# cipherflow-fhe/lattisense

Measured on AMD Instinct MI355X. Metric: ckks_hmult_relin_rescale_throughput, higher is better.
Workload: dtype u64

## Files before the change

include/lattisense_amd.h:

```cpp
#ifndef LATTISENSE_AMD_H
#define LATTISENSE_AMD_H
#include <stddef.h>
#include <stdint.h>

#ifdef __cplusplus
extern "C" {
#endif

typedef struct lsa_context_st* lsa_context;
typedef struct lsa_key_st* lsa_key;

enum { LSA_OK = 0, LSA_ERR_ARG = 1, LSA_ERR_NO_DEVICE = 2, LSA_ERR_HIP = 3, LSA_ERR_INTERNAL = 4 };
enum { LSA_ALGO_BFV = 0, LSA_ALGO_CKKS = 1 };

const char* lsa_last_error(void);
const char* lsa_version(void);
const char* lsa_build_flags(void);

int lsa_context_create(int algo, int n, const uint64_t* q, int nq, const uint64_t* p, int np, uint64_t t,
                       int device, lsa_context* out);
int lsa_context_destroy(lsa_context ctx);
int lsa_context_moduli(lsa_context ctx, uint64_t* out, int capacity, int* count);

int lsa_malloc(lsa_context ctx, void** dptr, size_t bytes);
int lsa_free(lsa_context ctx, void* dptr);
int lsa_memcpy_h2d(lsa_context ctx, void* dst, const void* src, size_t bytes, void* stream);
int lsa_memcpy_d2h(lsa_context ctx, void* dst, const void* src, size_t bytes, void* stream);
int lsa_memcpy_d2d(lsa_context ctx, void* dst, const void* src, size_t bytes, void* stream);
int lsa_stream_create(lsa_context ctx, void** stream);
int lsa_stream_destroy(lsa_context ctx, void* stream);
int lsa_stream_synchronize(lsa_context ctx, void* stream);
int lsa_event_create(lsa_context ctx, void** ev);
int lsa_event_record(lsa_context ctx, void* ev, void* stream);
int lsa_event_elapsed_ms(lsa_context ctx, void* ev_start, void* ev_stop, float* ms);
int lsa_event_destroy(lsa_context ctx, void* ev);

int lsa_key_upload(lsa_context ctx, const uint64_t* compact_host, int key_level, void* stream, lsa_key* out);
int lsa_key_adopt_device(lsa_context ctx, uint64_t* compact_dev, int key_level, void* stream, lsa_key* out);
int lsa_key_destroy(lsa_context ctx, lsa_key key);
size_t lsa_key_bytes(lsa_context ctx, int key_level);

int lsa_ntt(lsa_context ctx, uint64_t* data, int batch, long long batch_stride, int rows, const int* mod_of,
            int period, int inverse, void* stream);

int lsa_poly_addsub(lsa_context ctx, int op, int level, int polys, const uint64_t* a, const uint64_t* b,
                    uint64_t* out, int batch, long long stride_a, long long stride_b, long long stride_out,
                    void* stream);

int lsa_ckks_mult(lsa_context ctx, int level, const uint64_t* a, const uint64_t* b, uint64_t* d3, int batch,
                  long long stride_a, long long stride_b, long long stride_d, void* stream);
int lsa_ckks_relin(lsa_context ctx, int level, const uint64_t* d3, lsa_key rlk, uint64_t* out, int batch,
                   long long stride_d, long long stride_out, void* stream);
int lsa_ckks_rescale(lsa_context ctx, int level, int polys, const uint64_t* in, uint64_t* out, int batch,
                     long long stride_in, long long stride_out, void* stream);
int lsa_ckks_rotate(lsa_context ctx, int level, const uint64_t* in, uint64_t galois_element, lsa_key glk,
                    uint64_t* out, int batch, long long stride_in, long long stride_out, void* stream);
int lsa_drop_level(lsa_context ctx, int level, int polys, const uint64_t* in, uint64_t* out, int batch,
                   long long stride_in, long long stride_out, void* stream);
int lsa_ckks_mult_relin_rescale(lsa_context ctx, int level, const uint64_t* a, const uint64_t* b, lsa_key rlk,
                                uint64_t* out, int batch, long long stride_a, long long stride_b,
                                long long stride_out, void* stream);
int lsa_ckks_mult_sum(lsa_context ctx, int level, int n, const uint64_t* const* as, const long long* sas, const int* a_rpp,
                      const uint64_t* const* bs, const long long* sbs, const int* b_rpp, const uint64_t* addend,
                      long long s_addend, uint64_t* d3, int batch, long long sd, void* stream);
int lsa_ckks_dot(lsa_context ctx, int level, int n, const uint64_t* const* as, const long long* sas, const int* a_rpp,
                 const uint64_t* const* bs, const long long* sbs, const int* b_rpp, const uint64_t* addend,
                 long long s_addend, lsa_key rlk, uint64_t* out, int batch, long long sout, int rescale, void* stream);

int lsa_ckks_encode(lsa_context ctx, int level, int log_slots, const double* values, double scale, uint64_t* out_dev, long long sout,
                    int batch, void* stream);
int lsa_ckks_mult_plain(lsa_context ctx, int level, const uint64_t* ct, long long sct, const uint64_t* pt, long long spt, uint64_t* out,
                        long long sout, int batch, int rescale, void* stream);
int lsa_ckks_addsub_plain(lsa_context ctx, int op, int level, const uint64_t* ct, long long sct, const uint64_t* pt, long long spt,
                          uint64_t* out, long long sout, int batch, void* stream);
int lsa_ckks_mac_plain(lsa_context ctx, int level, int n, const uint64_t* const* cts, const long long* scts, const uint64_t* const* pts,
                       const long long* spts, const uint64_t* addend, long long s_addend, uint64_t* out, long long sout, int batch,
                       int rescale, void* stream);
int lsa_ckks_mult_const(lsa_context ctx, int level, const uint64_t* ct, long long sct, double re, double im, double const_scale,
                        uint64_t* out, long long sout, int batch, int rescale, void* stream);
int lsa_ckks_add_const(lsa_context ctx, int level, const uint64_t* ct, long long sct, double re, double im, double ct_scale,
                       uint64_t* out, long long sout, int batch, void* stream);
int lsa_ckks_affine_const(lsa_context ctx, int level, const uint64_t* ct, long long sct, double re, double im, double const_scale,
                          double add_re, double add_im, double ct_scale, uint64_t* out, long long sout, int batch, int rescale,
                          void* stream);

int lsa_bfv_mult(lsa_context ctx, int level, const uint64_t* a, const uint64_t* b, uint64_t* d3, int batch,
                 long long stride_a, long long stride_b, long long stride_d, void* stream);
int lsa_bfv_relin(lsa_context ctx, int level, const uint64_t* d3, lsa_key rlk, uint64_t* out, int batch,
                  long long stride_d, long long stride_out, void* stream);
int lsa_bfv_rotate(lsa_context ctx, int level, const uint64_t* in, uint64_t galois_element, lsa_key glk,
                   uint64_t* out, int batch, long long stride_in, long long stride_out, void* stream);
int lsa_bfv_mult_plain_mul(lsa_context ctx, int level, const uint64_t* ct, const uint64_t* pt, uint64_t* out, int batch,
                           long long sct, long long spt, long long sout, void* stream);
int lsa_bfv_mac_plain_mul(lsa_context ctx, int level, int n, const uint64_t* const* cts, const long long* scts,
                          const uint64_t* const* pts, const long long* spts, const uint64_t* partial, long long spartial,
                          uint64_t* out, int batch, long long sout, void* stream);
int lsa_bfv_rotate_mac_plain_mul(lsa_context ctx, int level, const uint64_t* in, int n, const uint64_t* galois_elements,
                                 const lsa_key* glk, const uint64_t* const* pts, const long long* spts, const uint64_t* partial,
                                 long long spartial, uint64_t* out, int batch, long long sin, long long sout, void* stream);
int lsa_bfv_rescale(lsa_context ctx, int level, int polys, const uint64_t* in, uint64_t* out, int batch,
                    long long stride_in, long long stride_out, void* stream);
int lsa_bfv_mult_relin(lsa_context ctx, int level, const uint64_t* a, const uint64_t* b, lsa_key rlk,
                       uint64_t* out, int batch, long long stride_a, long long stride_b, long long stride_out,
                       void* stream);
int lsa_bfv_mult_sum(lsa_context ctx, int level, int n, const uint64_t* const* as, const long long* sas, const uint64_t* const* bs,
                     const long long* sbs, const uint64_t* addend, long long s_addend, uint64_t* d3, int batch, long long sd,
                     void* stream);
int lsa_bfv_dot(lsa_context ctx, int level, int n, const uint64_t* const* as, const long long* sas, const uint64_t* const* bs,
                const long long* sbs, const uint64_t* addend, long long s_addend, lsa_key rlk, uint64_t* out, int batch,
                long long sout, void* stream);
int lsa_bfv_dot_plan(int n_ring, const uint64_t* q, int nq, int level, int terms, int* max_terms, int* n_groups, int* aux_limbs);

int lsa_set_bfv_dot_chunk(lsa_context ctx, int pairs);
int lsa_set_tile_batch(lsa_context ctx, int tile_batch);
int lsa_set_fp64_ntt(lsa_context ctx, int enable);
int lsa_set_dual_stream(lsa_context ctx, int enable);
int lsa_set_fuse_tails(lsa_context ctx, int enable);
int lsa_set_modup_lift(lsa_context ctx, int enable);
int lsa_set_ks_tail_in_mac(lsa_context ctx, int mode);
int lsa_set_ntt_chunk_mib(lsa_context ctx, int mib);
int lsa_ckks_rotate_many(lsa_context ctx, int level, const uint64_t* in, int n_rot, const uint64_t* galois_elements,
                         const lsa_key* glk, uint64_t* const* outs, int batch, long long sin, long long sout, void* stream);
int lsa_bfv_rotate_many(lsa_context ctx, int level, const uint64_t* in, int n_rot, const uint64_t* galois_elements,
                        const lsa_key* glk, uint64_t* const* outs, int batch, long long sin, long long sout, void* stream);

typedef struct lsa_bootstrap_st* lsa_bootstrap;
int lsa_bootstrap_create(lsa_context ctx, int cts_depth, int stc_depth, int k, int double_angle, double message_ratio,
                         double in_scale, double out_scale, int log_slots, void* stream, lsa_bootstrap* out);
int lsa_bootstrap_create_ex(lsa_context ctx, int cts_depth, int stc_depth, int k, int double_angle, double message_ratio,
                            double in_scale, double out_scale, int log_slots, int sine_deg, int arcsine_deg, void* stream,
                            lsa_bootstrap* out);
int lsa_bootstrap_evalmod_constants(lsa_bootstrap b, int* n_cheb, double* cheb, int* n_asin, double* asin_coef);
void lsa_bootstrap_destroy(lsa_bootstrap b);
int lsa_bootstrap_info(lsa_bootstrap b, int* out_level, double* out_scale, int* n_galois, int* n_matrices, int* n_cts,
                       int* sparse);
int lsa_bootstrap_galois_elements(lsa_bootstrap b, uint64_t* out, int capacity);
int lsa_bootstrap_chebyshev(lsa_bootstrap b, double* out32);
int lsa_bootstrap_matrix_info(lsa_bootstrap b, int index, int* level, int* n1, int* n_diagonals, int* diagonals, int capacity);
int lsa_bootstrap_plaintext(lsa_bootstrap b, int matrix, int diag_pos, uint64_t* host_out);
int lsa_bootstrap_plaintext_rows(lsa_bootstrap b, int matrix, int* rows);
int lsa_bootstrap_plaintext_ext(lsa_bootstrap b, int matrix, int diag_pos, uint64_t* host_out, long long capacity_words);
int lsa_ckks_bootstrap(lsa_context ctx, lsa_bootstrap b, const uint64_t* in, uint64_t* out, int batch, long long sin, long long sout,
                       lsa_key rlk, int n_glk, const uint64_t* glk_elements, const lsa_key* glk, lsa_key swk_dts, lsa_key swk_std,
                       void* stream);

typedef struct lsa_linear_transform_st* lsa_linear_transform;
int lsa_lt_create(lsa_context ctx, int level, int log_slots, int n_diag, const int* diag_index, const double* values,
                  double pt_scale, double bsgs_ratio, int double_hoist, void* stream, lsa_linear_transform* out);
void lsa_lt_destroy(lsa_linear_transform lt);
int lsa_lt_info(lsa_linear_transform lt, int* level, int* period, int* n_diag, int* n1, int* rows, int* n_galois,
                int* double_hoist, double* pt_scale);
int lsa_lt_diagonals(lsa_linear_transform lt, int* index_out, int capacity);
int lsa_lt_galois_elements(lsa_linear_transform lt, uint64_t* out, int capacity);
int lsa_lt_plaintext(lsa_linear_transform lt, int diag_pos, uint64_t* host_out, long long capacity_words);
int lsa_ckks_linear_transform(lsa_context ctx, lsa_linear_transform lt, const uint64_t* in, uint64_t* out, int batch,
                              long long sin, long long sout, int rescale, int n_glk, const uint64_t* glk_elements,
                              const lsa_key* glk, void* stream);
int lsa_lt_plan_rotations(int period, int n_diag, const int* diag_index, double bsgs_ratio, int* n1, int* rotations,
                          int capacity, int* count);

typedef struct lsa_slot_sum_st* lsa_slot_sum;
int lsa_slot_sum_plan(int n_ring, long long step, int count, int radix, int* n_steps, int* n_keyswitch, int* n_moddown,
                      int* rotations, int capacity, int* n_rot);
int lsa_slot_sum_create(lsa_context ctx, int level, long long step, int count, int radix, lsa_slot_sum* out);
void lsa_slot_sum_destroy(lsa_slot_sum plan);
int lsa_slot_sum_info(lsa_slot_sum plan, int* level, int* count, int* radix, int* n_steps, int* n_keyswitch, int* n_moddown,
                      int* n_galois);
int lsa_slot_sum_galois_elements(lsa_slot_sum plan, uint64_t* out, int capacity);
int lsa_slot_sum_set_multi_mac(lsa_slot_sum plan, int enable);
int lsa_ckks_slot_sum(lsa_context ctx, lsa_slot_sum plan, const uint64_t* in, uint64_t* out, int batch, long long sin,
                      long long sout, int n_keys, const uint64_t* galois_elements, const lsa_key* keys, void* stream);

typedef struct lsa_bfv_slot_sum_st* lsa_bfv_slot_sum_handle;
int lsa_bfv_slot_sum_plan(int n_ring, long long step, int count, int radix, int rows, int* n_steps, int* n_keyswitch, int* n_moddown,
                          uint64_t* galois_elements, int capacity, int* n_galois);
int lsa_bfv_slot_sum_create(lsa_context ctx, int level, long long step, int count, int radix, int rows, lsa_bfv_slot_sum_handle* out);
void lsa_bfv_slot_sum_destroy(lsa_bfv_slot_sum_handle plan);
int lsa_bfv_slot_sum_info(lsa_bfv_slot_sum_handle plan, int* level, int* count, int* radix, int* rows, int* n_steps, int* n_keyswitch,
                          int* n_moddown, int* n_galois, int* gather);
int lsa_bfv_slot_sum_galois_elements(lsa_bfv_slot_sum_handle plan, uint64_t* out, int capacity);
int lsa_bfv_slot_sum_set_gather(lsa_bfv_slot_sum_handle plan, int enable);
int lsa_bfv_slot_sum(lsa_context ctx, lsa_bfv_slot_sum_handle plan, const uint64_t* in, uint64_t* out, int batch, long long sin,
                     long long sout, int n_keys, const uint64_t* galois_elements, const lsa_key* keys, void* stream);

int lsa_bfv_encode(lsa_context ctx, int level, int form, const uint64_t* values, uint64_t* out_dev, long long sout, int batch,
                   void* stream);

int lsa_bfv_addsub_plain(lsa_context ctx, int op, int level, const uint64_t* ct, long long sct, const uint64_t* pt, long long spt,
                         uint64_t* out, long long sout, int batch, void* stream);
int lsa_bfv_plain_lift(lsa_context ctx, int level, int form, const uint64_t* pt, long long spt, uint64_t* out, long long sout,
                       int batch, void* stream);
int lsa_bfv_mult_plain(lsa_context ctx, int level, const uint64_t* ct, long long sct, const uint64_t* pt, long long spt,
                       uint64_t* out, long long sout, int batch, void* stream);

typedef struct lsa_bfv_lt_st* lsa_bfv_lt;
int lsa_bfv_lt_create(lsa_context ctx, int level, int period, int n_diag, const int* diag_index, const uint64_t* values,
                      double bsgs_ratio, void* stream, lsa_bfv_lt* out);
void lsa_bfv_lt_destroy(lsa_bfv_lt lt);
int lsa_bfv_lt_info(lsa_bfv_lt lt, int* level, int* period, int* n_diag, int* n1, int* n_baby, int* n_giant, int* rows,
                    int* n_galois, int* n_moddown);
int lsa_bfv_lt_diagonals(lsa_bfv_lt lt, int* index_out, int capacity);
int lsa_bfv_lt_galois_elements(lsa_bfv_lt lt, uint64_t* out, int capacity);
int lsa_bfv_lt_plaintext(lsa_bfv_lt lt, int diag_pos, uint64_t* host_out, long long capacity_words);
int lsa_bfv_linear_transform(lsa_context ctx, lsa_bfv_lt lt, const uint64_t* in, uint64_t* out, int batch, long long sin,
                             long long sout, int n_keys, const uint64_t* galois_elements, const lsa_key* keys, void* stream);

typedef struct lsa_polynomial_st* lsa_polynomial;
int lsa_poly_plan(int basis, int n_coef, const double* coef, int log_baby, int level_in, int with_interval, int* depth,
                  int* log_baby_out, int* n_mult, int* n_leaves, int* n_leaf_launches);
int lsa_poly_create(lsa_context ctx, int basis, int n_coef, const double* coef, double a, double b, int level_in, double scale_in,
                    double scale_out, int log_baby, lsa_polynomial* out);
void lsa_poly_destroy(lsa_polynomial p);
int lsa_poly_info(lsa_polynomial p, int* level_in, int* level_out, double* scale_out, int* depth, int* log_baby, int* n_mult,
                  int* n_leaves, int* n_leaf_launches, int* n_constants);
int lsa_poly_constants(lsa_polynomial p, long long* out, int capacity);
int lsa_ckks_poly_eval(lsa_context ctx, lsa_polynomial p, const uint64_t* in, uint64_t* out, int batch, long long sin,
                       long long sout, lsa_key rlk, void* stream);

typedef struct lsa_bfv_polynomial_st* lsa_bfv_polynomial;
int lsa_bfv_poly_plan(uint64_t t, int n_coef, const uint64_t* coef, int log_baby, int* log_baby_out, int* depth, int* n_mult,
                      int* n_leaves, int* n_leaf_launches, int* n_pairs);
int lsa_bfv_poly_create(lsa_context ctx, int level, int n_coef, const uint64_t* coef, int log_baby, void* stream,
                        lsa_bfv_polynomial* out);
void lsa_bfv_poly_destroy(lsa_bfv_polynomial p);
int lsa_bfv_poly_info(lsa_bfv_polynomial p, int* level, int* n_coef, int* log_baby, int* depth, int* n_mult, int* n_leaves,
                      int* n_leaf_launches, int* n_pairs);
int lsa_bfv_poly_eval(lsa_context ctx, lsa_bfv_polynomial p, const uint64_t* in, uint64_t* out, int batch, long long sin,
                      long long sout, lsa_key rlk, void* stream);
int lsa_bfv_affine_const(lsa_context ctx, int level, const uint64_t* ct, long long sct, uint64_t k, uint64_t c, uint64_t* out,
                         long long sout, int batch, void* stream);

int lsa_debug_set_ntt_stamps(lsa_context ctx, void* device_buffer);
int lsa_debug_baseconv_plans(lsa_context ctx, int capacity, int* count, int* ns, int* nd, int* split);
int lsa_debug_key_switch_fused(lsa_context ctx, int level, lsa_key key, int* fused);
int lsa_profile_begin(lsa_context ctx, int stride);
int lsa_profile_end(lsa_context ctx);
int lsa_profile_read(lsa_context ctx, int kind, double* total_ms, double* total_bytes, long long* sampled,
                     long long* launched);
int lsa_profile_read_primary(lsa_context ctx, int kind, double* total_bytes_primary);
int lsa_probe_copy(lsa_context ctx, uint64_t* dst, const uint64_t* src, size_t n_u64, void* stream);
int lsa_probe_mulhi(lsa_context ctx, uint64_t* buf, size_t n_u64, int iters, void* stream);

#ifdef __cplusplus
}
#endif
#endif
```

lattisense_amd/_native.py:

```python
import ctypes
import importlib.util
import os

_HERE = os.path.dirname(os.path.abspath(__file__))
LIB_PATH = os.environ.get("LSA_NATIVE_LIB") or os.path.join(_HERE, "liblattisense_amd.so")

_lib = None

c_u64p = ctypes.POINTER(ctypes.c_uint64)
c_ll = ctypes.c_longlong
c_vp = ctypes.c_void_p
c_int = ctypes.c_int


class LsaError(RuntimeError):
    def __init__(self, code, msg):
        super().__init__("lattisense_amd error %d: %s" % (code, msg))
        self.code = code


def _preload_hip_runtime():
    spec = importlib.util.find_spec("torch")
    if spec is not None and spec.origin:
        p = os.path.join(os.path.dirname(spec.origin), "lib", "libamdhip64.so")
        if os.path.exists(p):
            ctypes.CDLL(p, mode=ctypes.RTLD_GLOBAL)


SIGNATURES = {
    "lsa_last_error": (ctypes.c_char_p, []),
    "lsa_version": (ctypes.c_char_p, []),
    "lsa_build_flags": (ctypes.c_char_p, []),
    "lsa_context_create": (c_int, [c_int, c_int, c_u64p, c_int, c_u64p, c_int, ctypes.c_uint64, c_int,
                                   ctypes.POINTER(c_vp)]),
    "lsa_context_destroy": (c_int, [c_vp]),
    "lsa_context_moduli": (c_int, [c_vp, c_u64p, c_int, ctypes.POINTER(c_int)]),
    "lsa_malloc": (c_int, [c_vp, ctypes.POINTER(c_vp), ctypes.c_size_t]),
    "lsa_free": (c_int, [c_vp, c_vp]),
    "lsa_memcpy_h2d": (c_int, [c_vp, c_vp, c_vp, ctypes.c_size_t, c_vp]),
    "lsa_memcpy_d2h": (c_int, [c_vp, c_vp, c_vp, ctypes.c_size_t, c_vp]),
    "lsa_memcpy_d2d": (c_int, [c_vp, c_vp, c_vp, ctypes.c_size_t, c_vp]),
    "lsa_stream_create": (c_int, [c_vp, ctypes.POINTER(c_vp)]),
    "lsa_stream_destroy": (c_int, [c_vp, c_vp]),
    "lsa_stream_synchronize": (c_int, [c_vp, c_vp]),
    "lsa_event_create": (c_int, [c_vp, ctypes.POINTER(c_vp)]),
    "lsa_event_record": (c_int, [c_vp, c_vp, c_vp]),
    "lsa_event_elapsed_ms": (c_int, [c_vp, c_vp, c_vp, ctypes.POINTER(ctypes.c_float)]),
    "lsa_event_destroy": (c_int, [c_vp, c_vp]),
    "lsa_key_upload": (c_int, [c_vp, c_vp, c_int, c_vp, ctypes.POINTER(c_vp)]),
    "lsa_key_adopt_device": (c_int, [c_vp, c_vp, c_int, c_vp, ctypes.POINTER(c_vp)]),
    "lsa_key_destroy": (c_int, [c_vp, c_vp]),
    "lsa_key_bytes": (ctypes.c_size_t, [c_vp, c_int]),
    "lsa_ntt": (c_int, [c_vp, c_vp, c_int, c_ll, c_int, ctypes.POINTER(c_int), c_int, c_int, c_vp]),
    "lsa_poly_addsub": (c_int, [c_vp, c_int, c_int, c_int, c_vp, c_vp, c_vp, c_int, c_ll, c_ll, c_ll, c_vp]),
    "lsa_ckks_mult": (c_int, [c_vp, c_int, c_vp, c_vp, c_vp, c_int, c_ll, c_ll, c_ll, c_vp]),
    "lsa_ckks_relin": (c_int, [c_vp, c_int, c_vp, c_vp, c_vp, c_int, c_ll, c_ll, c_vp]),
    "lsa_ckks_rescale": (c_int, [c_vp, c_int, c_int, c_vp, c_vp, c_int, c_ll, c_ll, c_vp]),
    "lsa_ckks_rotate": (c_int, [c_vp, c_int, c_vp, ctypes.c_uint64, c_vp, c_vp, c_int, c_ll, c_ll, c_vp]),
    "lsa_drop_level": (c_int, [c_vp, c_int, c_int, c_vp, c_vp, c_int, c_ll, c_ll, c_vp]),
    "lsa_ckks_mult_relin_rescale": (c_int, [c_vp, c_int, c_vp, c_vp, c_vp, c_vp, c_int, c_ll, c_ll, c_ll, c_vp]),
    "lsa_ckks_mult_sum": (c_int, [c_vp, c_int, c_int, ctypes.POINTER(c_vp), ctypes.POINTER(c_ll), ctypes.POINTER(c_int),
                                  ctypes.POINTER(c_vp), ctypes.POINTER(c_ll), ctypes.POINTER(c_int), c_vp, c_ll, c_vp, c_int, c_ll, c_vp]),
    "lsa_ckks_dot": (c_int, [c_vp, c_int, c_int, ctypes.POINTER(c_vp), ctypes.POINTER(c_ll), ctypes.POINTER(c_int),
                             ctypes.POINTER(c_vp), ctypes.POINTER(c_ll), ctypes.POINTER(c_int), c_vp, c_ll, c_vp, c_vp, c_int, c_ll, c_int,
                             c_vp]),
    "lsa_ckks_encode": (c_int, [c_vp, c_int, c_int, ctypes.POINTER(ctypes.c_double), ctypes.c_double, c_vp, c_ll, c_int, c_vp]),
    "lsa_ckks_mult_plain": (c_int, [c_vp, c_int, c_vp, c_ll, c_vp, c_ll, c_vp, c_ll, c_int, c_int, c_vp]),
    "lsa_ckks_addsub_plain": (c_int, [c_vp, c_int, c_int, c_vp, c_ll, c_vp, c_ll, c_vp, c_ll, c_int, c_vp]),
    "lsa_ckks_mac_plain": (c_int, [c_vp, c_int, c_int, ctypes.POINTER(c_vp), ctypes.POINTER(c_ll), ctypes.POINTER(c_vp),
                                   ctypes.POINTER(c_ll), c_vp, c_ll, c_vp, c_ll, c_int, c_int, c_vp]),
    "lsa_ckks_mult_const": (c_int, [c_vp, c_int, c_vp, c_ll, ctypes.c_double, ctypes.c_double, ctypes.c_double, c_vp, c_ll, c_int,
                                    c_int, c_vp]),
    "lsa_ckks_add_const": (c_int, [c_vp, c_int, c_vp, c_ll, ctypes.c_double, ctypes.c_double, ctypes.c_double, c_vp, c_ll, c_int,
                                   c_vp]),
    "lsa_ckks_affine_const": (c_int, [c_vp, c_int, c_vp, c_ll, ctypes.c_double, ctypes.c_double, ctypes.c_double, ctypes.c_double,
                                      ctypes.c_double, ctypes.c_double, c_vp, c_ll, c_int, c_int, c_vp]),
    "lsa_bfv_mult": (c_int, [c_vp, c_int, c_vp, c_vp, c_vp, c_int, c_ll, c_ll, c_ll, c_vp]),
    "lsa_bfv_relin": (c_int, [c_vp, c_int, c_vp, c_vp, c_vp, c_int, c_ll, c_ll, c_vp]),
    "lsa_bfv_rotate": (c_int, [c_vp, c_int, c_vp, ctypes.c_uint64, c_vp, c_vp, c_int, c_ll, c_ll, c_vp]),
    "lsa_bfv_rescale": (c_int, [c_vp, c_int, c_int, c_vp, c_vp, c_int, c_ll, c_ll, c_vp]),
    "lsa_bfv_mult_relin": (c_int, [c_vp, c_int, c_vp, c_vp, c_vp, c_vp, c_int, c_ll, c_ll, c_ll, c_vp]),
    "lsa_bfv_mult_sum": (c_int, [c_vp, c_int, c_int, ctypes.POINTER(c_vp), ctypes.POINTER(c_ll), ctypes.POINTER(c_vp),
                                 ctypes.POINTER(c_ll), c_vp, c_ll, c_vp, c_int, c_ll, c_vp]),
    "lsa_bfv_dot": (c_int, [c_vp, c_int, c_int, ctypes.POINTER(c_vp), ctypes.POINTER(c_ll), ctypes.POINTER(c_vp), ctypes.POINTER(c_ll),
                            c_vp, c_ll, c_vp, c_vp, c_int, c_ll, c_vp]),
    "lsa_bfv_dot_plan": (c_int, [c_int, c_u64p, c_int, c_int, c_int, ctypes.POINTER(c_int), ctypes.POINTER(c_int),
                                 ctypes.POINTER(c_int)]),
    "lsa_set_bfv_dot_chunk": (c_int, [c_vp, c_int]),
    "lsa_set_tile_batch": (c_int, [c_vp, c_int]),
    "lsa_set_fp64_ntt": (c_int, [c_vp, c_int]),
    "lsa_set_dual_stream": (c_int, [c_vp, c_int]),
    "lsa_set_fuse_tails": (c_int, [c_vp, c_int]),
    "lsa_set_modup_lift": (c_int, [c_vp, c_int]),
    "lsa_set_ks_tail_in_mac": (c_int, [c_vp, c_int]),
    "lsa_set_ntt_chunk_mib": (c_int, [c_vp, c_int]),
    "lsa_debug_set_ntt_stamps": (c_int, [c_vp, c_vp]),
    "lsa_debug_baseconv_plans": (c_int, [c_vp, c_int, ctypes.POINTER(c_int), ctypes.POINTER(c_int), ctypes.POINTER(c_int),
                                         ctypes.POINTER(c_int)]),
    "lsa_debug_key_switch_fused": (c_int, [c_vp, c_int, c_vp, ctypes.POINTER(c_int)]),
    "lsa_ckks_rotate_many": (c_int, [c_vp, c_int, c_vp, c_int, c_u64p, ctypes.POINTER(c_vp), ctypes.POINTER(c_vp), c_int,
                                     ctypes.c_longlong, ctypes.c_longlong, c_vp]),
    "lsa_bfv_rotate_many": (c_int, [c_vp, c_int, c_vp, c_int, c_u64p, ctypes.POINTER(c_vp), ctypes.POINTER(c_vp), c_int,
                                    ctypes.c_longlong, ctypes.c_longlong, c_vp]),
    "lsa_bfv_mult_plain_mul": (c_int, [c_vp, c_int, c_vp, c_vp, c_vp, c_int, c_ll, c_ll, c_ll, c_vp]),
    "lsa_bfv_mac_plain_mul": (c_int, [c_vp, c_int, c_int, ctypes.POINTER(c_vp), ctypes.POINTER(c_ll), ctypes.POINTER(c_vp),
                                      ctypes.POINTER(c_ll), c_vp, c_ll, c_vp, c_int, c_ll, c_vp]),
    "lsa_bfv_rotate_mac_plain_mul": (c_int, [c_vp, c_int, c_vp, c_int, c_u64p, ctypes.POINTER(c_vp), ctypes.POINTER(c_vp),
                                             ctypes.POINTER(c_ll), c_vp, c_ll, c_vp, c_int, c_ll, c_ll, c_vp]),
    "lsa_bootstrap_create": (c_int, [c_vp, c_int, c_int, c_int, c_int, ctypes.c_double, ctypes.c_double, ctypes.c_double, c_int,
                                     c_vp, ctypes.POINTER(c_vp)]),
    "lsa_bootstrap_create_ex": (c_int, [c_vp, c_int, c_int, c_int, c_int, ctypes.c_double, ctypes.c_double, ctypes.c_double, c_int,
                                        c_int, c_int, c_vp, ctypes.POINTER(c_vp)]),
    "lsa_bootstrap_evalmod_constants": (c_int, [c_vp, ctypes.POINTER(c_int), ctypes.POINTER(ctypes.c_double), ctypes.POINTER(c_int),
                                                ctypes.POINTER(ctypes.c_double)]),
    "lsa_bootstrap_destroy": (None, [c_vp]),
    "lsa_bootstrap_info": (c_int, [c_vp, ctypes.POINTER(c_int), ctypes.POINTER(ctypes.c_double), ctypes.POINTER(c_int),
                                   ctypes.POINTER(c_int), ctypes.POINTER(c_int), ctypes.POINTER(c_int)]),
    "lsa_bootstrap_galois_elements": (c_int, [c_vp, c_u64p, c_int]),
    "lsa_bootstrap_chebyshev": (c_int, [c_vp, ctypes.POINTER(ctypes.c_double)]),
    "lsa_bootstrap_matrix_info": (c_int, [c_vp, c_int, ctypes.POINTER(c_int), ctypes.POINTER(c_int), ctypes.POINTER(c_int),
                                          ctypes.POINTER(c_int), c_int]),
    "lsa_bootstrap_plaintext": (c_int, [c_vp, c_int, c_int, c_u64p]),
    "lsa_bootstrap_plaintext_rows": (c_int, [c_vp, c_int, ctypes.POINTER(c_int)]),
    "lsa_bootstrap_plaintext_ext": (c_int, [c_vp, c_int, c_int, c_u64p, ctypes.c_longlong]),
    "lsa_ckks_bootstrap": (c_int, [c_vp, c_vp, c_vp, c_vp, c_int, ctypes.c_longlong, ctypes.c_longlong, c_vp, c_int, c_u64p,
                                   ctypes.POINTER(c_vp), c_vp, c_vp, c_vp]),
    "lsa_lt_create": (c_int, [c_vp, c_int, c_int, c_int, ctypes.POINTER(c_int), ctypes.POINTER(ctypes.c_double), ctypes.c_double,
                              ctypes.c_double, c_int, c_vp, ctypes.POINTER(c_vp)]),
    "lsa_lt_destroy": (None, [c_vp]),
    "lsa_lt_info": (c_int, [c_vp, ctypes.POINTER(c_int), ctypes.POINTER(c_int), ctypes.POINTER(c_int), ctypes.POINTER(c_int),
                            ctypes.POINTER(c_int), ctypes.POINTER(c_int), ctypes.POINTER(c_int), ctypes.POINTER(ctypes.c_double)]),
    "lsa_lt_diagonals": (c_int, [c_vp, ctypes.POINTER(c_int), c_int]),
    "lsa_lt_galois_elements": (c_int, [c_vp, c_u64p, c_int]),
    "lsa_lt_plaintext": (c_int, [c_vp, c_int, c_u64p, c_ll]),
    "lsa_ckks_linear_transform": (c_int, [c_vp, c_vp, c_vp, c_vp, c_int, c_ll, c_ll, c_int, c_int, c_u64p, ctypes.POINTER(c_vp),
                                          c_vp]),
    "lsa_slot_sum_plan": (c_int, [c_int, c_ll, c_int, c_int, ctypes.POINTER(c_int), ctypes.POINTER(c_int), ctypes.POINTER(c_int),
                                  ctypes.POINTER(c_int), c_int, ctypes.POINTER(c_int)]),
    "lsa_slot_sum_create": (c_int, [c_vp, c_int, c_ll, c_int, c_int, ctypes.POINTER(c_vp)]),
    "lsa_slot_sum_destroy": (None, [c_vp]),
    "lsa_slot_sum_info": (c_int, [c_vp] + [ctypes.POINTER(c_int)] * 7),
    "lsa_slot_sum_galois_elements": (c_int, [c_vp, c_u64p, c_int]),
    "lsa_slot_sum_set_multi_mac": (c_int, [c_vp, c_int]),
    "lsa_ckks_slot_sum": (c_int, [c_vp, c_vp, c_vp, c_vp, c_int, c_ll, c_ll, c_int, c_u64p, ctypes.POINTER(c_vp), c_vp]),
    "lsa_bfv_slot_sum_plan": (c_int, [c_int, c_ll, c_int, c_int, c_int, ctypes.POINTER(c_int), ctypes.POINTER(c_int), ctypes.POINTER(c_int),
                                      c_u64p, c_int, ctypes.POINTER(c_int)]),
    "lsa_bfv_slot_sum_create": (c_int, [c_vp, c_int, c_ll, c_int, c_int, c_int, ctypes.POINTER(c_vp)]),
    "lsa_bfv_slot_sum_destroy": (None, [c_vp]),
    "lsa_bfv_slot_sum_info": (c_int, [c_vp] + [ctypes.POINTER(c_int)] * 9),
    "lsa_bfv_slot_sum_galois_elements": (c_int, [c_vp, c_u64p, c_int]),
    "lsa_bfv_slot_sum_set_gather": (c_int, [c_vp, c_int]),
    "lsa_bfv_slot_sum": (c_int, [c_vp, c_vp, c_vp, c_vp, c_int, c_ll, c_ll, c_int, c_u64p, ctypes.POINTER(c_vp), c_vp]),
    "lsa_bfv_encode": (c_int, [c_vp, c_int, c_int, c_u64p, c_vp, c_ll, c_int, c_vp]),
    "lsa_bfv_addsub_plain": (c_int, [c_vp, c_int, c_int, c_vp, c_ll, c_vp, c_ll, c_vp, c_ll, c_int, c_vp]),
    "lsa_bfv_plain_lift": (c_int, [c_vp, c_int, c_int, c_vp, c_ll, c_vp, c_ll, c_int, c_vp]),
    "lsa_bfv_mult_plain": (c_int, [c_vp, c_int, c_vp, c_ll, c_vp, c_ll, c_vp, c_ll, c_int, c_vp]),
    "lsa_bfv_lt_create": (c_int, [c_vp, c_int, c_int, c_int, ctypes.POINTER(c_int), c_u64p, ctypes.c_double, c_vp, ctypes.POINTER(c_vp)]),
    "lsa_bfv_lt_destroy": (None, [c_vp]),
    "lsa_bfv_lt_info": (c_int, [c_vp] + [ctypes.POINTER(c_int)] * 9),
    "lsa_bfv_lt_diagonals": (c_int, [c_vp, ctypes.POINTER(c_int), c_int]),
    "lsa_bfv_lt_galois_elements": (c_int, [c_vp, c_u64p, c_int]),
    "lsa_bfv_lt_plaintext": (c_int, [c_vp, c_int, c_u64p, c_ll]),
    "lsa_bfv_linear_transform": (c_int, [c_vp, c_vp, c_vp, c_vp, c_int, c_ll, c_ll, c_int, c_u64p, ctypes.POINTER(c_vp), c_vp]),
    "lsa_lt_plan_rotations": (c_int, [c_int, c_int, ctypes.POINTER(c_int), ctypes.c_double, ctypes.POINTER(c_int),
                                      ctypes.POINTER(c_int), c_int, ctypes.POINTER(c_int)]),
    "lsa_poly_plan": (c_int, [c_int, c_int, ctypes.POINTER(ctypes.c_double), c_int, c_int, c_int, ctypes.POINTER(c_int),
                              ctypes.POINTER(c_int), ctypes.POINTER(c_int), ctypes.POINTER(c_int), ctypes.POINTER(c_int)]),
    "lsa_poly_create": (c_int, [c_vp, c_int, c_int, ctypes.POINTER(ctypes.c_double), ctypes.c_double, ctypes.c_double, c_int,
                                ctypes.c_double, ctypes.c_double, c_int, ctypes.POINTER(c_vp)]),
    "lsa_poly_destroy": (None, [c_vp]),
    "lsa_poly_info": (c_int, [c_vp, ctypes.POINTER(c_int), ctypes.POINTER(c_int), ctypes.POINTER(ctypes.c_double),
                              ctypes.POINTER(c_int), ctypes.POINTER(c_int), ctypes.POINTER(c_int), ctypes.POINTER(c_int),
                              ctypes.POINTER(c_int), ctypes.POINTER(c_int)]),
    "lsa_poly_constants": (c_int, [c_vp, ctypes.POINTER(c_ll), c_int]),
    "lsa_ckks_poly_eval": (c_int, [c_vp, c_vp, c_vp, c_vp, c_int, c_ll, c_ll, c_vp, c_vp]),
    "lsa_bfv_poly_plan": (c_int, [ctypes.c_uint64, c_int, c_u64p, c_int] + [ctypes.POINTER(c_int)] * 6),
    "lsa_bfv_poly_create": (c_int, [c_vp, c_int, c_int, c_u64p, c_int, c_vp, ctypes.POINTER(c_vp)]),
    "lsa_bfv_poly_destroy": (None, [c_vp]),
    "lsa_bfv_poly_info": (c_int, [c_vp] + [ctypes.POINTER(c_int)] * 8),
    "lsa_bfv_poly_eval": (c_int, [c_vp, c_vp, c_vp, c_vp, c_int, c_ll, c_ll, c_vp, c_vp]),
    "lsa_bfv_affine_const": (c_int, [c_vp, c_int, c_vp, c_ll, ctypes.c_uint64, ctypes.c_uint64, c_vp, c_ll, c_int, c_vp]),
    "lsa_profile_begin": (c_int, [c_vp, c_int]),
    "lsa_profile_end": (c_int, [c_vp]),
    "lsa_profile_read": (c_int, [c_vp, c_int, ctypes.POINTER(ctypes.c_double), ctypes.POINTER(ctypes.c_double),
                                 ctypes.POINTER(c_ll), ctypes.POINTER(c_ll)]),
    "lsa_profile_read_primary": (c_int, [c_vp, c_int, ctypes.POINTER(ctypes.c_double)]),
    "lsa_probe_copy": (c_int, [c_vp, c_vp, c_vp, ctypes.c_size_t, c_vp]),
    "lsa_probe_mulhi": (c_int, [c_vp, c_vp, ctypes.c_size_t, c_int, c_vp]),
}


def lib():
    global _lib
    if _lib is None:
        if not os.path.exists(LIB_PATH):
            raise RuntimeError("liblattisense_amd.so is not built: run `python -m lattisense_amd.build` "
                               "(or __graft_entry__.build()); there is no fallback path")
        _preload_hip_runtime()
        L = ctypes.CDLL(LIB_PATH)
        for name, (res, args) in SIGNATURES.items():
            fn = getattr(L, name)
            fn.restype = res
            fn.argtypes = args
        flags = L.lsa_build_flags().decode()
        if flags and not os.environ.get("LSA_NATIVE_LIB"):
            raise RuntimeError("%s was built with switches [%s]: not the product build; rebuild with "
                               "`python -m lattisense_amd.build --force`" % (LIB_PATH, flags))
        _lib = L
    return _lib


def build_flags():
    return lib().lsa_build_flags().decode()


def check(rc):
    if rc != 0:
        raise LsaError(rc, lib().lsa_last_error().decode())
```

lattisense_amd/csrc/c_api.hip:

```cpp
#include "bfv_encode.h"
#include "bfv_poly.h"
#include "build_flags.h"
#include "linear_transform.h"
#include "poly_eval.h"
#include "lsa_internal.h"

namespace lsa {
const char* kernels_build_flags();
const char* context_build_flags();
}

using namespace lsa;

struct lsa_context_st {
    Context ctx;
    lsa_context_st(int algo, int n, const u64* q, int nq, const u64* p, int np, u64 t, int dev)
        : ctx(algo, n, q, nq, p, np, t, dev) {}
};
struct lsa_key_st {
    Key key;
    double* fp_owned = nullptr;
};

template <typename F>
// ... 291 lines not shown
    return guard([&] { ckks_encode(CP(ctx, "lsa_ckks_encode"), level, log_slots, values, scale, out_dev, sout, batch, S(stream)); });
}
int lsa_ckks_mult_plain(lsa_context ctx, int level, const uint64_t* ct, long long sct, const uint64_t* pt, long long spt, uint64_t* out,
                        long long sout, int batch, int rescale, void* stream) {
    return guard([&] { ckks_mult_plain(CP(ctx, "lsa_ckks_mult_plain"), level, ct, sct, pt, spt, out, sout, batch, rescale != 0, S(stream)); });
}
int lsa_ckks_addsub_plain(lsa_context ctx, int op, int level, const uint64_t* ct, long long sct, const uint64_t* pt, long long spt,
                          uint64_t* out, long long sout, int batch, void* stream) {
    return guard([&] { ckks_addsub_plain(CP(ctx, "lsa_ckks_addsub_plain"), op, level, ct, sct, pt, spt, out, sout, batch, S(stream)); });
}
int lsa_ckks_mac_plain(lsa_context ctx, int level, int n, const uint64_t* const* cts, const long long* scts, const uint64_t* const* pts,
                       const long long* spts, const uint64_t* addend, long long s_addend, uint64_t* out, long long sout, int batch,
                       int rescale, void* stream) {
    return guard([&] {
        ckks_mac_plain(CP(ctx, "lsa_ckks_mac_plain"), level, n, cts, scts, pts, spts, addend, s_addend, out, sout, batch, rescale != 0,
                       S(stream));
    });
}
int lsa_ckks_mult_const(lsa_context ctx, int level, const uint64_t* ct, long long sct, double re, double im, double const_scale,
                        uint64_t* out, long long sout, int batch, int rescale, void* stream) {
    return guard([&] {
        ckks_mult_const(CP(ctx, "lsa_ckks_mult_const"), level, ct, sct, re, im, const_scale, out, sout, batch, rescale != 0, S(stream));
    });
}
int lsa_ckks_add_const(lsa_context ctx, int level, const uint64_t* ct, long long sct, double re, double im, double ct_scale,
                       uint64_t* out, long long sout, int batch, void* stream) {
    return guard([&] { ckks_add_const(CP(ctx, "lsa_ckks_add_const"), level, ct, sct, re, im, ct_scale, out, sout, batch, S(stream)); });
}
int lsa_ckks_affine_const(lsa_context ctx, int level, const uint64_t* ct, long long sct, double re, double im, double const_scale,
                          double add_re, double add_im, double ct_scale, uint64_t* out, long long sout, int batch, int rescale,
                          void* stream) {
    return guard([&] {
        ckks_affine_const(CP(ctx, "lsa_ckks_affine_const"), level, ct, sct, re, im, const_scale, add_re, add_im, ct_scale, out, sout,
                          batch, rescale != 0, S(stream));
    });
}

int lsa_bfv_mult(lsa_context ctx, int level, const uint64_t* a, const uint64_t* b, uint64_t* d3, int batch, long long sa,
                 long long sb, long long sd, void* stream) {
    return guard([&] { bfv_mult(C(ctx), level, a, b, d3, batch, sa, sb, sd, S(stream)); });
}
int lsa_bfv_relin(lsa_context ctx, int level, const uint64_t* d3, lsa_key rlk, uint64_t* out, int batch, long long sd,
                  long long so, void* stream) {
    return guard([&] { bfv_relin(C(ctx), level, d3, K(rlk, "lsa_bfv_relin"), out, batch, sd, so, S(stream)); });
}
int lsa_bfv_rotate(lsa_context ctx, int level, const uint64_t* in, uint64_t g, lsa_key glk, uint64_t* out, int batch,
                   long long si, long long so, void* stream) {
    return guard([&] { bfv_rotate(C(ctx), level, in, g, K(glk, "lsa_bfv_rotate"), out, batch, si, so, S(stream)); });
}
int lsa_bfv_rescale(lsa_context ctx, int level, int polys, const uint64_t* in, uint64_t* out, int batch, long long si,
                    long long so, void* stream) {
    return guard([&] { bfv_rescale(C(ctx), level, polys, in, out, batch, si, so, S(stream)); });
}
int lsa_bfv_mult_relin(lsa_context ctx, int level, const uint64_t* a, const uint64_t* b, lsa_key rlk, uint64_t* out,
                       int batch, long long sa, long long sb, long long so, void* stream) {
    return guard([&] { bfv_mult_relin(C(ctx), level, a, b, K(rlk, "lsa_bfv_mult_relin"), out, batch, sa, sb, so, S(stream)); });
}

int lsa_bfv_mult_sum(lsa_context ctx, int level, int n, const uint64_t* const* as, const long long* sas, const uint64_t* const* bs,
                     const long long* sbs, const uint64_t* addend, long long s_addend, uint64_t* d3, int batch, long long sd,
                     void* stream) {
    return guard([&] {
        const DotTerms t{n, as, sas, nullptr, bs, sbs, nullptr, addend, s_addend};
        bfv_mult_sum(C(ctx), level, t, d3, batch, sd, S(stream));
    });
}
int lsa_bfv_dot(lsa_context ctx, int level, int n, const uint64_t* const* as, const long long* sas, const uint64_t* const* bs,
                const long long* sbs, const uint64_t* addend, long long s_addend, lsa_key rlk, uint64_t* out, int batch, long long sout,
                void* stream) {
    return guard([&] {
        const DotTerms t{n, as, sas, nullptr, bs, sbs, nullptr, addend, s_addend};
        bfv_dot(C(ctx), level, t, rlk ? &rlk->key : nullptr, out, batch, sout, S(stream));
    });
}
int lsa_bfv_dot_plan(int n_ring, const uint64_t* q, int nq, int level, int terms, int* max_terms, int* n_groups, int* aux_limbs) {
    return guard([&] {
        LSA_REQUIRE(n_ring >= 2 && n_ring <= (1 << 20) && (n_ring & (n_ring - 1)) == 0, "bfv_dot: the ring degree must be a power of two");
        LSA_REQUIRE(q != nullptr && nq >= 1, "bfv_dot: null argument");
        LSA_REQUIRE(level >= 0 && level < nq, "bfv_dot: level out of range");
        LSA_REQUIRE(terms >= 1, "bfv_dot: needs at least one term");
        for (int i = 0; i < nq; i++) LSA_REQUIRE(q[i] >= 2 && (q[i] >> 61) == 0, "bfv_dot: a modulus is out of range");
        int logn = 0;
        while ((1 << logn) < n_ring) logn++;
        const BfvDotPlan p = bfv_dot_plan(q, nq, level, logn, terms);
        if (max_terms) *max_terms = p.max_terms;
        if (n_groups) *n_groups = p.n_groups;
        if (aux_limbs) *aux_limbs = p.aux_limbs;
    });
}

int lsa_profile_begin(lsa_context ctx, int stride) {
    return guard([&] {
        Context& c = C(ctx);
        LSA_REQUIRE(stride >= 1, "stride must be >= 1");
        for (auto& sm : c.prof_samples) {
            c.prof_pool.push_back(sm.e0);
            c.prof_pool.push_back(sm.e1);
        }
        c.prof_samples.clear();
        for (auto& n : c.prof_launched) n = 0;
        c.prof_stride = stride;
        c.prof_on = true;
    });
}
int lsa_profile_end(lsa_context ctx) {
    return guard([&] { C(ctx).prof_on = false; });
}
int lsa_profile_read(lsa_context ctx, int kind, double* total_ms, double* total_bytes, long long* sampled,
                     long long* launched) {
    return guard([&] {
        Context& c = C(ctx);
        LSA_REQUIRE(kind >= 0 && kind < LSA_PROF_KINDS, "unknown kernel kind");
        double ms = 0, by = 0;
        long long n = 0;
        for (auto& sm : c.prof_samples) {
            if (sm.kid != kind) continue;
            LSA_HIP(hipEventSynchronize(sm.e1));
            float t = 0;
            LSA_HIP(hipEventElapsedTime(&t, sm.e0, sm.e1));
            ms += t;
            by += sm.bytes;
            n++;
        }
        if (total_ms) *total_ms = ms;
        if (total_bytes) *total_bytes = by;
        if (sampled) *sampled = n;
        if (launched) *launched = c.prof_launched[kind];
    });
}

int lsa_profile_read_primary(lsa_context ctx, int kind, double* total_bytes_primary) {
    return guard([&] {
        Context& c = C(ctx);
        LSA_REQUIRE(kind >= 0 && kind < LSA_PROF_KINDS && total_bytes_primary, "bad argument");
        double by = 0;
        for (auto& sm : c.prof_samples)
            if (sm.kid == kind) by += sm.bytes_primary;
        *total_bytes_primary = by;
    });
}

int lsa_set_fuse_tails(lsa_context ctx, int enable) {
    return guard([&] { C(ctx).fuse_tails = enable ? 1 : 0; });
}
int lsa_set_modup_lift(lsa_context ctx, int enable) {
    return guard([&] { C(ctx).modup_lift = enable ? 1 : 0; });
}
int lsa_set_ks_tail_in_mac(lsa_context ctx, int mode) {
    return guard([&] {
        LSA_REQUIRE(mode >= 0 && mode <= 2, "lsa_set_ks_tail_in_mac: mode is 0, 1 or 2");
        C(ctx).ks_tail_in_mac = mode;
    });
}
int lsa_set_dual_stream(lsa_context ctx, int enable) {
    return guard([&] { C(ctx).dual_stream = enable ? 1 : 0; });
}
int lsa_debug_set_ntt_stamps(lsa_context ctx, void* device_buffer) {
    return guard([&] { C(ctx).ntt_diag = static_cast<unsigned long long*>(device_buffer); });
}
int lsa_debug_baseconv_plans(lsa_context ctx, int capacity, int* count, int* ns, int* nd, int* split) {
    return guard([&] {
        Context& c = C(ctx);
        LSA_REQUIRE(count != nullptr && (capacity == 0 || (ns && nd && split)), "null argument");
        std::lock_guard<std::mutex> lk(c.mu);
        *count = (int)c.bconv.size();
        int i = 0;
        for (auto& kv : c.bconv) {
            if (i >= capacity) break;
            ns[i] = kv.second.ns;
            nd[i] = kv.second.nd;
            split[i] = kv.second.split29 ? 1 : 0;
            i++;
        }
    });
}
int lsa_debug_key_switch_fused(lsa_context ctx, int level, lsa_key key, int* fused) {
    return guard([&] {
        Context& c = C(ctx);
        LSA_REQUIRE(fused != nullptr && level >= 0 && level < c.nq, "bad argument");
        *fused = ks_fuse_mac(c, level, K(key)) ? 1 : 0;
    });
}

int lsa_ckks_rotate_many(lsa_context ctx, int level, const uint64_t* in, int n_rot, const uint64_t* galois_elements,
                         const lsa_key* glk, uint64_t* const* outs, int batch, long long sin, long long sout, void* stream) {
    return guard([&] {
        LSA_REQUIRE(in != nullptr && n_rot >= 0 && (n_rot == 0 || (galois_elements && glk && outs)), "lsa_ckks_rotate_many: null argument");
        std::vector<const Key*> keys(n_rot);
        for (int i = 0; i < n_rot; i++) {
            LSA_REQUIRE(glk[i] != nullptr && outs[i] != nullptr, "lsa_ckks_rotate_many: null key or output");
            keys[i] = &K(glk[i], "lsa_ckks_rotate_many");
        }
        ckks_rotate_many(C(ctx), level, in, n_rot, galois_elements, keys.data(), outs, batch, sin, sout, S(stream));
    });
}
int lsa_bfv_rotate_many(lsa_context ctx, int level, const uint64_t* in, int n_rot, const uint64_t* galois_elements,
                        const lsa_key* glk, uint64_t* const* outs, int batch, long long sin, long long sout, void* stream) {
    return guard([&] {
        LSA_REQUIRE(in != nullptr && n_rot >= 0 && (n_rot == 0 || (galois_elements && glk && outs)), "null argument");
        std::vector<const Key*> keys(n_rot);
        for (int i = 0; i < n_rot; i++) {
            LSA_REQUIRE(glk[i] != nullptr && outs[i] != nullptr, "null key or output");
            keys[i] = &K(glk[i]);
        }
        bfv_rotate_many(C(ctx), level, in, n_rot, galois_elements, keys.data(), outs, batch, sin, sout, S(stream));
    });
}

int lsa_bfv_mult_plain_mul(lsa_context ctx, int level, const uint64_t* ct, const uint64_t* pt, uint64_t* out, int batch,
                           long long sct, long long spt, long long sout, void* stream) {
    return guard([&] {
        LSA_REQUIRE(ct != nullptr && pt != nullptr && out != nullptr, "null argument");
        bfv_mult_plain_mul(C(ctx), level, ct, pt, out, batch, sct, spt, sout, S(stream));
    });
}
int lsa_bfv_mac_plain_mul(lsa_context ctx, int level, int n, const uint64_t* const* cts, const long long* scts,
                          const uint64_t* const* pts, const long long* spts, const uint64_t* partial, long long spartial,
                          uint64_t* out, int batch, long long sout, void* stream) {
    return guard([&] {
        LSA_REQUIRE(n >= 1 && cts && scts && pts && spts && out, "null argument");
        for (int i = 0; i < n; i++) LSA_REQUIRE(cts[i] != nullptr && pts[i] != nullptr, "null ciphertext or plaintext");
        bfv_mac_plain_mul(C(ctx), level, n, cts, scts, pts, spts, partial, spartial, out, batch, sout, S(stream));
    });
}
int lsa_bfv_rotate_mac_plain_mul(lsa_context ctx, int level, const uint64_t* in, int n, const uint64_t* galois_elements,
                                 const lsa_key* glk, const uint64_t* const* pts, const long long* spts, const uint64_t* partial,
                                 long long spartial, uint64_t* out, int batch, long long sin, long long sout, void* stream) {
    return guard([&] {
        LSA_REQUIRE(n >= 1, "bfv_rotate_mac_plain_mul: needs at least one term");
        LSA_REQUIRE(in && galois_elements && glk && pts && spts && out, "null argument");
        std::vector<const Key*> keys(n, nullptr);
        for (int i = 0; i < n; i++) keys[i] = glk[i] ? &K(glk[i]) : nullptr;
        bfv_rotate_mac_plain_mul(C(ctx), level, in, n, galois_elements, keys.data(), pts, spts, partial, spartial, out, batch, sin,
                                 sout, S(stream));
    });
}


struct lsa_bootstrap_st : PlanHandle<Bootstrap> {};
int lsa_bootstrap_create_ex(lsa_context ctx, int cts_depth, int stc_depth, int k, int double_angle, double message_ratio,
                            double in_scale, double out_scale, int log_slots, int sine_deg, int arcsine_deg, void* stream,
                            lsa_bootstrap* out) {
    return guard([&] {
        LSA_REQUIRE(out != nullptr, "null argument");
        LSA_REQUIRE(k >= 1 && double_angle >= 0 && double_angle <= 8 && message_ratio > 0 && in_scale > 0, "bad bootstrap parameters");
        Context& c = C(ctx);
        LSA_REQUIRE(log_slots >= 0 && (log_slots == 0 || (2 << log_slots) <= c.n), "bad slot count");
        make_plan(out, c, bootstrap_create(c, cts_depth, stc_depth, k, double_angle, message_ratio, in_scale, out_scale, log_slots, S(stream),
                                           sine_deg, arcsine_deg), bootstrap_destroy);
    });
}
int lsa_bootstrap_create(lsa_context ctx, int cts_depth, int stc_depth, int k, int double_angle, double message_ratio,
                         double in_scale, double out_scale, int log_slots, void* stream, lsa_bootstrap* out) {
    return lsa_bootstrap_create_ex(ctx, cts_depth, stc_depth, k, double_angle, message_ratio, in_scale, out_scale, log_slots, 30, 0, stream, out);
}
int lsa_bootstrap_evalmod_constants(lsa_bootstrap b, int* n_cheb, double* cheb, int* n_asin, double* asin_coef) {
    return guard([&] {
        const Bootstrap& bt = P(b, "null bootstrap handle");
        const auto& c = bootstrap_chebyshev(bt);
        const auto& a = bootstrap_arcsine(bt);
        if (n_cheb) *n_cheb = (int)c.size();
        if (n_asin) *n_asin = (int)a.size();
        if (cheb) std::copy(c.begin(), c.end(), cheb);
        if (asin_coef) std::copy(a.begin(), a.end(), asin_coef);
    });
}
void lsa_bootstrap_destroy(lsa_bootstrap b) { delete b; }
int lsa_bootstrap_info(lsa_bootstrap b, int* out_level, double* out_scale, int* n_galois, int* n_matrices, int* n_cts,
                       int* sparse) {
    return guard([&] {
        const Bootstrap& bt = P(b, "null bootstrap handle");
        if (out_level) *out_level = bootstrap_out_level(bt);
        if (out_scale) *out_scale = bootstrap_out_scale(bt);
        if (n_galois) *n_galois = (int)bootstrap_galois(bt).size();
        if (n_matrices) *n_matrices = bootstrap_matrices(bt);
        if (n_cts) *n_cts = bootstrap_cts_matrices(bt);
        if (sparse) *sparse = bootstrap_is_sparse(bt) ? 1 : 0;
    });
}
int lsa_bootstrap_galois_elements(lsa_bootstrap b, uint64_t* out, int capacity) {
    return guard([&] {
        LSA_REQUIRE(b != nullptr && out != nullptr, "null argument");
        copy_out(bootstrap_galois(*b->plan), out, capacity, "buffer too small");
    });
}
int lsa_bootstrap_chebyshev(lsa_bootstrap b, double* out32) {
    return guard([&] {
        LSA_REQUIRE(b != nullptr && out32 != nullptr, "null argument");
        const auto& cf = bootstrap_chebyshev(*b->plan);
        LSA_REQUIRE(cf.size() <= 32, "more than 32 Chebyshev coefficients: use lsa_bootstrap_evalmod_constants");
        for (size_t i = 0; i < 32; i++) out32[i] = i < cf.size() ? cf[i] : 0.0;
    });
}
int lsa_bootstrap_matrix_info(lsa_bootstrap b, int index, int* level, int* n1, int* n_diagonals, int* diagonals, int capacity) {
    return guard([&] {
        int lv, n1v;
        const std::vector<int>* ks;
        const std::vector<u64*>* pl;
        bootstrap_matrix(P(b, "null bootstrap handle"), index, &lv, &n1v, &ks, &pl);
        if (level) *level = lv;
        if (n1) *n1 = n1v;
        if (n_diagonals) *n_diagonals = (int)ks->size();
        if (diagonals) copy_out(*ks, diagonals, capacity, "buffer too small");
    });
}
int lsa_bootstrap_plaintext(lsa_bootstrap b, int matrix, int diag_pos, uint64_t* host_out) {
// ... 445 lines not shown
```

lattisense_amd/csrc/context.hip:

```cpp
#include "build_flags.h"
#include "lsa_internal.h"
#include <cstdlib>
#include <cstring>

namespace lsa {

const char* context_build_flags() { return LSA_BUILD_FLAGS_TEXT; }

static thread_local std::string g_last_error;
void set_last_error(const std::string& m) { g_last_error = m; }
const std::string& last_error() { return g_last_error; }

Context::Context(int algo_, int n_, const u64* q, int nq_, const u64* p, int np_, u64 t_, int device_)
    : algo(algo_), n(n_), nq(nq_), np(np_), device(device_), t(t_) {
    LSA_REQUIRE(algo == LSA_ALGO_BFV || algo == LSA_ALGO_CKKS, "unknown algorithm");
    LSA_REQUIRE(n >= 512 && n <= (1 << 17) && (n & (n - 1)) == 0, "ring degree must be a power of two in [2^9, 2^17]");
    LSA_REQUIRE(nq >= 1 && np >= 0 && np <= LSA_BC_NARROW_SRC, "bad modulus chain lengths");
    std::vector<u64> mods(q, q + nq);
    mods.insert(mods.end(), p, p + np);
    nmul = 0;
    int lg = 0;
    while ((1 << lg) < n) lg++;
    if (algo == LSA_ALGO_BFV) {
        LSA_REQUIRE(t > 1, "BFV needs a plaintext modulus");
        nmul = bfv_aux_count(q, nq, lg);
        std::vector<u64> aux = gen_aux_primes(n, nmul, mods);
        mods.insert(mods.end(), aux.begin(), aux.end());
    }
    nmod = (int)mods.size();
    LSA_REQUIRE(nmod < LSA_ROW_SKIP, "too many moduli");
    T.build(n, mods);
    logn = T.logn;
#ifndef LSA_NTT_TAU
#define LSA_NTT_TAU 12
#endif
    plan = make_ntt_plan(logn, LSA_NTT_TAU, sw::ntt_mu_a());
    plan_wide = make_ntt_plan(logn, (logn == 13 || logn == 14) ? logn : LSA_NTT_TAU);
    fp_raw = sw::ntt_fp_raw(fp_raw);
    wide_mode = sw::ntt_wide(wide_mode);
    LSA_REQUIRE(plan.npass == 1 || plan.pass[1].mu <= plan.pass[1].tau, "ring degree too large for the NTT tile size");

    int ndev = 0;
    hipError_t e = hipGetDeviceCount(&ndev);
    if (e != hipSuccess || ndev <= 0)
        throw Error(LSA_ERR_NO_DEVICE, "no HIP device available: this library has no CPU fallback");
    LSA_REQUIRE(device >= 0 && device < ndev, "device index out of range");
    use_device();
    LSA_HIP(hipMalloc((void**)&d_mods, nmod * sizeof(ModDev)));
    LSA_HIP(hipMalloc((void**)&d_scale, (size_t)nmod * 4 * sizeof(u64)));
    LSA_HIP(hipMalloc((void**)&d_scale_d, (size_t)nmod * 2 * sizeof(double)));
    LSA_HIP(hipMemcpy(d_mods, T.mods.data(), nmod * sizeof(ModDev), hipMemcpyHostToDevice));
    LSA_HIP(hipMemcpy(d_scale, T.scale.data(), (size_t)nmod * 4 * sizeof(u64), hipMemcpyHostToDevice));
    auto upload = [&](const NttPlan& pl, u64** psi, u64** psiinv, double** psi_d, double** psiinv_d) {
        const size_t tw_bytes = (size_t)nmod * n * sizeof(u64);
        std::vector<u64> pi(T.psi.size()), pii(T.psiinv.size());
        std::vector<double> pd(T.psi_d.size()), pdi(T.psiinv_d.size());
        for (int m = 0; m < nmod; m++) {
            const size_t o = (size_t)m * n;
            ntt_permute_twiddles(pl, logn, T.psi.data() + 2 * o, pi.data() + 2 * o, 2, false);
            ntt_permute_twiddles(pl, logn, T.psiinv.data() + 2 * o, pii.data() + 2 * o, 2, false);
            ntt_permute_twiddles(pl, logn, T.psi_d.data() + o, pd.data() + o, 1, true);
            ntt_permute_twiddles(pl, logn, T.psiinv_d.data() + o, pdi.data() + o, 1, true);
        }
        LSA_HIP(hipMalloc((void**)psi, 2 * tw_bytes));
        LSA_HIP(hipMalloc((void**)psiinv, 2 * tw_bytes));
        LSA_HIP(hipMalloc((void**)psi_d, tw_bytes));
        LSA_HIP(hipMalloc((void**)psiinv_d, tw_bytes));
        LSA_HIP(hipMemcpy(*psi, pi.data(), 2 * tw_bytes, hipMemcpyHostToDevice));
        LSA_HIP(hipMemcpy(*psiinv, pii.data(), 2 * tw_bytes, hipMemcpyHostToDevice));
        LSA_HIP(hipMemcpy(*psi_d, pd.data(), tw_bytes, hipMemcpyHostToDevice));
        LSA_HIP(hipMemcpy(*psiinv_d, pdi.data(), tw_bytes, hipMemcpyHostToDevice));
    };
    upload(plan, &d_psi, &d_psiinv, &d_psi_d, &d_psiinv_d);
    if (plan_wide.npass < plan.npass) upload(plan_wide, &d_psi_w, &d_psiinv_w, &d_psi_d_w, &d_psiinv_d_w);
    LSA_HIP(hipMemcpy(d_scale_d, T.scale_d.data(), (size_t)nmod * 2 * sizeof(double), hipMemcpyHostToDevice));
}

Context::~Context() {
    (void)hipSetDevice(device);
    (void)hipDeviceSynchronize();
    (void)hipFree(d_mods);
    (void)hipFree(d_psi);
    (void)hipFree(d_psiinv);
    (void)hipFree(d_scale);
    (void)hipFree(d_psi_d);
    (void)hipFree(d_psiinv_d);
    (void)hipFree(d_psi_w);
    (void)hipFree(d_psiinv_w);
    (void)hipFree(d_psi_d_w);
    (void)hipFree(d_psiinv_d_w);
    (void)hipFree(d_scale_d);
    (void)hipFree(ws);
    (void)hipFree(ws2);
    if (aux_stream) {
        (void)hipStreamDestroy(aux_stream);
        (void)hipEventDestroy(ev_fork);
        (void)hipEventDestroy(ev_join);
    }
    for (auto& sm : prof_samples) {
        (void)hipEventDestroy(sm.e0);
        (void)hipEventDestroy(sm.e1);
    }
    for (auto& e : prof_pool) (void)hipEventDestroy(e);
    for (auto& kv : bconv) (void)hipFree(kv.second.dev);
    for (auto& kv : perm_ntt) (void)hipFree(kv.second);
    for (auto& kv : perm_coeff) (void)hipFree(kv.second);
    for (auto& kv : consts) (void)hipFree(kv.second);
}

u64* Context::workspace(size_t words, hipStream_t s) {
    if (words > ws_words) {
        LSA_HIP(hipStreamSynchronize(s));
        if (ws) LSA_HIP(hipFree(ws));
        ws = nullptr;
        ws_words = 0;
        LSA_HIP(hipMalloc((void**)&ws, words * sizeof(u64)));
        ws_words = words;
    }
    return ws;
}

void Context::fork_aux(hipStream_t s) {
    if (!aux_stream) {
        LSA_HIP(hipStreamCreateWithFlags(&aux_stream, hipStreamNonBlocking));
        LSA_HIP(hipEventCreateWithFlags(&ev_fork, hipEventDisableTiming));
        LSA_HIP(hipEventCreateWithFlags(&ev_join, hipEventDisableTiming));
    }
    LSA_HIP(hipEventRecord(ev_fork, s));
    LSA_HIP(hipStreamWaitEvent(aux_stream, ev_fork, 0));
}

void Context::join_aux(hipStream_t s) {
    LSA_HIP(hipEventRecord(ev_join, aux_stream));
    LSA_HIP(hipStreamWaitEvent(s, ev_join, 0));
}

u64* Context::workspace2(size_t words, hipStream_t s) {
    if (words > ws2_words) {
        LSA_HIP(hipStreamSynchronize(s));
        if (ws2) LSA_HIP(hipFree(ws2));
        ws2 = nullptr;
        ws2_words = 0;
        LSA_HIP(hipMalloc((void**)&ws2, words * sizeof(u64)));
        ws2_words = words;
    }
    return ws2;
}

const BaseConvPlan* Context::baseconv(const std::vector<int>& src, const std::vector<int>& dst, bool centered,
                                      bool pinv_scaled, const BaseConvFold* fold) {
    std::string key = centered ? "c" : "u";
    if (pinv_scaled) key += "s";
    if (fold) {
        LSA_REQUIRE(!fold->tag.empty() && (fold->src_pre.empty() || fold->src_pre.size() == src.size()) &&
                        (fold->dst_scale.empty() || fold->dst_scale.size() == dst.size()),
                    "base conversion: folded factors do not match the limb lists");
        key += "f:" + fold->tag;
    }
    for (int x : src) key += "|" + std::to_string(x);
    key += "->";
    for (int x : dst) key += "|" + std::to_string(x);
    std::lock_guard<std::mutex> lk(mu);
    auto it = bconv.find(key);
    if (it != bconv.end()) return &it->second;
    const int ns = (int)src.size(), nd = (int)dst.size();
    LSA_REQUIRE(ns >= 1 && ns <= LSA_BC_MAX_SRC && nd >= 1 && nd <= LSA_BC_MAX_DST, "base conversion too wide");
    auto K = std::make_unique<BaseConvConsts>();
    K->ns = ns;
    K->nd = nd;
    K->centered = centered ? 1 : 0;
    for (int i = 0; i < ns; i++) {
        const u64 qi = T.mod[src[i]];
        K->src_mod[i] = src[i];
        u64 pr = 1 % qi;
        for (int l = 0; l < ns; l++)
            if (l != i) pr = mul_mod_host(pr, T.mod[src[l]] % qi, qi);
        K->shat_inv_m[i] = to_mont_host(inv_mod(pr, qi), qi);
        K->half_src[i] = mul_mod_host(qi - 1, (qi + 1) >> 1, qi);
        if (fold && !fold->src_pre.empty()) {
            const u64 f = fold->src_pre[i] % qi;
            LSA_REQUIRE(f != 0, "base conversion: folded source factor is zero");
            K->shat_inv_m[i] = to_mont_host(mul_mod_host(inv_mod(pr, qi), f, qi), qi);
            K->half_src[i] = mul_mod_host(K->half_src[i], inv_mod(f, qi), qi);
        }
        K->qf[i] = (double)qi;
        K->rf[i] = 1.0 / (double)qi;
    }
    for (int j = 0; j < nd; j++) {
        const u64 pj = T.mod[dst[j]];
        K->dst_mod[j] = dst[j];
        u64 all = 1 % pj;
        for (int l = 0; l < ns; l++) all = mul_mod_host(all, T.mod[src[l]] % pj, pj);
        u64 scale = 1 % pj;
        if (pinv_scaled && j + 1 < nd) {
            u64 pp = 1;
            for (int l = 0; l < np; l++) pp = mul_mod_host(pp, T.mod[p_mod(l)] % pj, pj);
            scale = inv_mod(pp, pj);
        }
        if (fold && !fold->dst_scale.empty()) scale = mul_mod_host(scale, fold->dst_scale[j] % pj, pj);
        for (int i = 0; i < ns; i++) {
            u64 pr = 1 % pj;
            for (int l = 0; l < ns; l++)
                if (l != i) pr = mul_mod_host(pr, T.mod[src[l]] % pj, pj);
            K->shat_m[j][i] = to_mont_host(mul_mod_host(pr, scale, pj), pj);
        }
        for (int v = 0; v <= ns; v++) K->vs[j][v] = mul_mod_host(mul_mod_host((u64)v % pj, all, pj), scale, pj);
        K->half_dst[j] = mul_mod_host(mul_mod_host((all + pj - 1 % pj) % pj, (pj + 1) >> 1, pj), scale, pj);
    }
    bool small = !sw::bc_no_split() && ns <= LSA_BC_NARROW_SRC;
    for (int i = 0; i < ns; i++) small = small && (T.mod[src[i]] >> 58) == 0;
    for (int j = 0; j < nd; j++) small = small && (T.mod[dst[j]] >> 58) == 0;
    K->split29 = small ? 1 : 0;
    for (int j = 0; j < nd; j++)
        for (int i = 0; i < ns; i++) {
            K->shat_lo[j][i] = (u32)(K->shat_m[j][i] & ((1u << 29) - 1));
            K->shat_hi[j][i] = (u32)(K->shat_m[j][i] >> 29);
            K->shat_sum[j][i] = K->shat_lo[j][i] + K->shat_hi[j][i];
        }
    for (int j = 0; j < nd; j++) {
        const u64 pj = T.mod[dst[j]];
        K->corr_a[j] = to_mont_host((pj - K->vs[j][1]) % pj, pj);
        K->corr_b[j] = centered ? to_mont_host((pj - K->half_dst[j]) % pj, pj) : 0;
    }
    use_device();
    BaseConvConsts* d = nullptr;
    LSA_HIP(hipMalloc((void**)&d, sizeof(BaseConvConsts)));
    LSA_HIP(hipMemcpy(d, K.get(), sizeof(BaseConvConsts), hipMemcpyHostToDevice));
    BaseConvPlan pl;
    pl.dev = d;
    pl.ns = ns;
    pl.nd = nd;
    pl.split29 = small;
    bconv[key] = pl;
    return &bconv[key];
}

static unsigned brv_bits(unsigned x, int bits) {
    unsigned r = 0;
    for (int i = 0; i < bits; i++) {
        r = (r << 1) | (x & 1);
        x >>= 1;
    }
    return r;
}

const u32* Context::ntt_perm(u64 g) {
    std::lock_guard<std::mutex> lk(mu);
    auto it = perm_ntt.find(g);
    if (it != perm_ntt.end()) return it->second;
    LSA_REQUIRE((g & 1) == 1 && g < 2 * (u64)n, "Galois element must be odd and < 2N");
    std::vector<u32> h(n);
    const u64 mask = 2 * (u64)n - 1;
    for (int i = 0; i < n; i++) {
        const u64 e = 2 * (u64)brv_bits((unsigned)i, logn) + 1;
        const u64 e2 = (g * e) & mask;
        h[i] = brv_bits((unsigned)((e2 - 1) >> 1), logn);
    }
    use_device();
    u32* d = nullptr;
    LSA_HIP(hipMalloc((void**)&d, n * sizeof(u32)));
    LSA_HIP(hipMemcpy(d, h.data(), n * sizeof(u32), hipMemcpyHostToDevice));
    perm_ntt[g] = d;
    return d;
}

const u32* Context::coeff_perm(u64 g) {
    std::lock_guard<std::mutex> lk(mu);
    auto it = perm_coeff.find(g);
    if (it != perm_coeff.end()) return it->second;
    LSA_REQUIRE((g & 1) == 1 && g < 2 * (u64)n, "Galois element must be odd and < 2N");
    std::vector<u32> h(n);
    const u64 mask = 2 * (u64)n - 1;
    for (int i = 0; i < n; i++) {
        u64 idx = ((u64)i * g) & mask;
        u32 sign = 0;
        if (idx >= (u64)n) {
            idx -= n;
            sign = 1u << 31;
        }
        h[idx] = (u32)i | sign;
    }
    use_device();
    u32* d = nullptr;
    LSA_HIP(hipMalloc((void**)&d, n * sizeof(u32)));
    LSA_HIP(hipMemcpy(d, h.data(), n * sizeof(u32), hipMemcpyHostToDevice));
    perm_coeff[g] = d;
    return d;
}

const u64* Context::pinv_vec(int level) {
    const int L = level + 1;
    std::vector<int> mods(L);
    std::vector<u64> pinv(L);
    for (int i = 0; i < L; i++) {
        mods[i] = i;
        u64 q = T.mod[i], pr = 1;
        for (int l = 0; l < np; l++) pr = mul_mod_host(pr, T.mod[p_mod(l)] % q, q);
        pinv[i] = inv_mod(pr, q);
    }
    return const_vec("pinv" + std::to_string(L), mods, pinv);
}

const u64* Context::pmodq_vec(int level) {
    const int L = level + 1;
    std::vector<int> mods(L);
    std::vector<u64> pm(L);
    for (int j = 0; j < L; j++) {
        mods[j] = j;
        const u64 q = T.mod[j];
        u64 pr = 1;
        for (int l = 0; l < np; l++) pr = mul_mod_host(pr, T.mod[p_mod(l)] % q, q);
        pm[j] = pr;
    }
    return const_vec("pmodq" + std::to_string(L), mods, pm);
}

const u64* Context::pfold_vec(int level) {
    const int L = level + 1;
    std::vector<u64> v(2 * (size_t)L);
    for (int j = 0; j < L; j++) {
        const u64 q = T.mod[j];
        u64 pr = 1;
        for (int l = 0; l < np; l++) pr = mul_mod_host(pr, T.mod[p_mod(l)] % q, q);
        v[j] = to_mont_host(to_mont_host(pr, q), q);
        v[L + j] = pr;
    }
    return raw_vec("pfold" + std::to_string(L), v);
}

const u64* Context::tail_fp_vec(int level) {
    const std::string name = "tailfp" + std::to_string(level);
    {
        std::lock_guard<std::mutex> lk(mu);
        auto it = consts.find(name);
        if (it != consts.end()) return it->second;
    }
    std::vector<u64> v(2 * (size_t)level);
    const u64 ql = T.mod[level];
    for (int j = 0; j < level; j++) {
        const u64 q = T.mod[j];
        u64 pr = 1;
        for (int l = 0; l < np; l++) pr = mul_mod_host(pr, T.mod[p_mod(l)] % q, q);
        const double kd = (double)inv_mod(pr, q), k2d = (double)inv_mod(ql % q, q);
        std::memcpy(&v[j], &kd, sizeof(double));
        std::memcpy(&v[level + j], &k2d, sizeof(double));
    }
    return raw_vec(name, v);
}

const u64* Context::qlinv_vec(int level) {
    std::vector<int> mods(level);
    std::vector<u64> v(level);
    const u64 ql = T.mod[level];
    for (int i = 0; i < level; i++) {
        mods[i] = i;
        v[i] = inv_mod(ql % T.mod[i], T.mod[i]);
    }
    return const_vec("qlinv" + std::to_string(level), mods, v);
}

// ... 28 lines not shown
```

lattisense_amd/csrc/kernels.hip:

```cpp
#include <atomic>
#include <cstdlib>

#include "build_flags.h"
#include "lsa_internal.h"
#include "ntt_r16.h"
#include "plain_ops.h"
#include "poly_lincomb.h"
#include "tensor_sum.h"

namespace lsa {

const char* kernels_build_flags() { return LSA_BUILD_FLAGS_TEXT; }

static constexpr int TPB = 256;

#ifndef LSA_NTT_WAVES
#define LSA_NTT_WAVES 4
#endif

#if defined(LSA_NTT_DIAG_STAMPS)
#define LSA_STAMP(k)                                                                               \
    do {                                                                                           \
        if (a.diag && threadIdx.x == 0 && blockIdx.x < 8192) a.diag[blockIdx.x * 8 + (k)] = __builtin_amdgcn_s_memtime(); \
    } while (0)
// ... 1025 lines not shown
    const int x = ((blockIdx.x % chunks) * TPB + threadIdx.x) * 2;
    const ModDev m = g.mods[g.mod_of[limb]];
    const long long b = blockIdx.y;
    const long long poly = (long long)g.limbs << g.logn;
    const long long off = ((long long)limb << g.logn) + x;
    const u64* pa = g.a + b * g.sa + off;
    const u64* pb = g.b + b * g.sb + off;
    u64* pd = g.d + b * g.sd + off;
    const ulonglong2 a0 = ld2(pa), a1 = ld2(pa + g.pa), b0 = ld2(pb), b1 = ld2(pb + g.pb);
    u64 r[3][2];
    const u64 a0v[2] = {a0.x, a0.y}, a1v[2] = {a1.x, a1.y}, b0v[2] = {b0.x, b0.y}, b1v[2] = {b1.x, b1.y};
#pragma unroll
    for (int e = 0; e < 2; e++) {
        const u64 b0m = mont_mul_lazy(b0v[e], m.r2, m.q, m.qinv);
        const u64 b1m = mont_mul_lazy(b1v[e], m.r2, m.q, m.qinv);
        r[0][e] = mont_mul(a0v[e], b0m, m.q, m.qinv);
        r[2][e] = mont_mul(a1v[e], b1m, m.q, m.qinv);
        r[1][e] = add_mod(mont_mul(a0v[e], b1m, m.q, m.qinv), mont_mul(a1v[e], b0m, m.q, m.qinv), m.q);
    }
    st2(pd, r[0][0], r[0][1]);
    st2(pd + poly, r[1][0], r[1][1]);
    st2(pd + 2 * poly, r[2][0], r[2][1]);
}

void launch_tensor(Context& c, const u64* a, const u64* b, u64* d, int batch, long long sa, long long sb, long long sd,
                   int limbs, const RowMap& rm, hipStream_t s, int a_rpp, int b_rpp) {
    if (batch <= 0) return;
    TensorArgs g{};
    LSA_REQUIRE((a_rpp == 0 || a_rpp >= limbs) && (b_rpp == 0 || b_rpp >= limbs), "tensor: rows per polynomial below the limb count");
    g.pa = (long long)(a_rpp ? a_rpp : limbs) << c.logn;
    g.pb = (long long)(b_rpp ? b_rpp : limbs) << c.logn;
    g.a = a;
    g.b = b;
    g.d = d;
    g.sa = sa;
    g.sb = sb;
    g.sd = sd;
    g.mods = c.d_mods;
    g.limbs = limbs;
    g.logn = c.logn;
    LSA_REQUIRE(rm.period == limbs && limbs <= LSA_MAX_PERIOD, "tensor: row map must cover the limbs");
    int period;
    fill_rowmap(g.mod_of, period, rm, c.nmod);
    ProfScope ps(c, PROF_TENSOR, 7.0 * 8 * c.n * limbs * batch, s);
    hipLaunchKernelGGL(k_tensor, ew_grid(c, limbs, batch), dim3(TPB), 0, s, g);
    LSA_HIP(hipGetLastError());
}

struct TensorSumArgs {
    const u64* a[LSA_DOT_MAX_TERMS];
    const u64* b[LSA_DOT_MAX_TERMS];
    long long sa[LSA_DOT_MAX_TERMS], sb[LSA_DOT_MAX_TERMS];
    long long pa[LSA_DOT_MAX_TERMS], pb[LSA_DOT_MAX_TERMS];
    const u64* addend;
    u64* d;
    long long s_addend, sd;
    const ModDev* mods;
    int terms, limbs, logn;
    unsigned char mod_of[LSA_MAX_PERIOD];
};

template <bool ACC>
__global__ __launch_bounds__(TPB) void k_tensor_sum(TensorSumArgs g) {
    const int chunks = (1 << g.logn) / (2 * TPB);
    const int limb = blockIdx.x / chunks;
    const int x = ((blockIdx.x % chunks) * TPB + threadIdx.x) * 2;
    const ModDev m = g.mods[g.mod_of[limb]];
    const long long b = blockIdx.y;
    const long long poly = (long long)g.limbs << g.logn;
    const long long off = ((long long)limb << g.logn) + x;
    u64* pd = g.d + b * g.sd + off;
    TsAcc t0, t1;
    ts_init(t0);
    ts_init(t1);
    if (ACC) {
        const ulonglong2 v0 = ld2(pd), v1 = ld2(pd + poly), v2 = ld2(pd + 2 * poly);
        ts_seed(t0.l0, v0.x);
        ts_seed(t1.l0, v0.y);
        ts_seed(t0.l1, v1.x);
        ts_seed(t1.l1, v1.y);
        ts_seed(t0.l2, v2.x);
        ts_seed(t1.l2, v2.y);
    }
    if (g.addend) {
        const u64* pe = g.addend + b * g.s_addend + off;
        const ulonglong2 v0 = ld2(pe), v1 = ld2(pe + poly);
        ts_seed(t0.l0, v0.x);
        ts_seed(t1.l0, v0.y);
        ts_seed(t0.l1, v1.x);
        ts_seed(t1.l1, v1.y);
    }
    for (int i = 0; i < g.terms; i++) {
        const u64* pa = g.a[i] + b * g.sa[i] + off;
        const u64* pb = g.b[i] + b * g.sb[i] + off;
        const ulonglong2 a0 = ld2(pa), a1 = ld2(pa + g.pa[i]), b0 = ld2(pb), b1 = ld2(pb + g.pb[i]);
        ts_term(t0, i, a0.x, a1.x, b0.x, b1.x, m);
        ts_term(t1, i, a0.y, a1.y, b0.y, b1.y, m);
    }
    st2(pd, ts_finish(t0.h0, t0.l0, m), ts_finish(t1.h0, t1.l0, m));
    st2(pd + poly, ts_finish(t0.h1, t0.l1, m), ts_finish(t1.h1, t1.l1, m));
    st2(pd + 2 * poly, ts_finish(t0.h2, t0.l2, m), ts_finish(t1.h2, t1.l2, m));
}

void launch_tensor_sum(Context& c, int terms, const u64* const* a, const long long* sa, const int* a_rpp, const u64* const* b,
                       const long long* sb, const int* b_rpp, const u64* addend, long long s_addend, bool accumulate, u64* d,
                       long long sd, int batch, int limbs, const RowMap& rm, hipStream_t s) {
    if (batch <= 0) return;
    LSA_REQUIRE(terms >= 1 && terms <= LSA_DOT_MAX_TERMS, "dot: too many terms for one launch");
    LSA_REQUIRE(rm.period == limbs && limbs <= LSA_MAX_PERIOD, "dot: row map must cover the limbs");
    LSA_REQUIRE(sd >= 3LL * limbs * c.n, "dot: output stride below three polynomials");
    TensorSumArgs g{};
    for (int i = 0; i < terms; i++) {
        const int ra = a_rpp && a_rpp[i] ? a_rpp[i] : limbs, rb = b_rpp && b_rpp[i] ? b_rpp[i] : limbs;
        LSA_REQUIRE(a[i] && b[i], "dot: null operand");
        LSA_REQUIRE(ra >= limbs && rb >= limbs, "dot: rows per polynomial below the limb count");
        LSA_REQUIRE((sa[i] == 0 || sa[i] >= 2LL * ra * c.n) && (sb[i] == 0 || sb[i] >= 2LL * rb * c.n), "dot: batch stride below one ciphertext");
        g.a[i] = a[i];
        g.b[i] = b[i];
        g.sa[i] = sa[i];
        g.sb[i] = sb[i];
        g.pa[i] = (long long)ra << c.logn;
        g.pb[i] = (long long)rb << c.logn;
    }
    LSA_REQUIRE(!addend || s_addend == 0 || s_addend >= 2LL * limbs * c.n, "dot: addend stride below one ciphertext");
    g.addend = addend;
    g.s_addend = s_addend;
    g.d = d;
    g.sd = sd;
    g.mods = c.d_mods;
    g.terms = terms;
    g.limbs = limbs;
    g.logn = c.logn;
    int period;
    fill_rowmap(g.mod_of, period, rm, c.nmod);
    for (int i = 0; i < limbs; i++) LSA_REQUIRE(g.mod_of[i] != LSA_ROW_SKIP, "dot: every limb needs a modulus");
    ProfScope ps(c, PROF_TENSOR, 8.0 * c.n * limbs * batch * (4 * terms + 3 + (addend ? 2 : 0) + (accumulate ? 3 : 0)), s);
    if (accumulate) hipLaunchKernelGGL((k_tensor_sum<true>), ew_grid(c, limbs, batch), dim3(TPB), 0, s, g);
    else hipLaunchKernelGGL((k_tensor_sum<false>), ew_grid(c, limbs, batch), dim3(TPB), 0, s, g);
    LSA_HIP(hipGetLastError());
}

struct BaseConvArgs {
    const BaseConvConsts* k;
    const ModDev* mods;
    const u64* src;
    u64* dst;
    long long ssrc, sdst;
    int logn;
    BaseConvRows rows;
    const u64* sub;
    long long ssub;
    int sub_row[LSA_BC_MAX_SRC];
};

#define LSA_CONST_AS __attribute__((address_space(4)))
__device__ __forceinline__ ModDev ld_mod(const LSA_CONST_AS ModDev* t, int i) {
    ModDev m;
    m.q = t[i].q;
    m.qinv = t[i].qinv;
    m.r2 = t[i].r2;
    m.r1 = t[i].r1;
    return m;
}
template <int NSMAX, bool EXACT, int TGT, bool SPLIT = false>
__global__ __launch_bounds__(TPB) void k_baseconv(BaseConvArgs g) {
    const LSA_CONST_AS BaseConvConsts& K = *(const LSA_CONST_AS BaseConvConsts*)g.k;
    const LSA_CONST_AS ModDev* const mods_c = (const LSA_CONST_AS ModDev*)g.mods;
    const int x = (blockIdx.x * TPB + threadIdx.x) * 2;
    const long long b = blockIdx.y;
    const u64* src = g.src + b * g.ssrc + x;
    u64* dst = g.dst + b * g.sdst + x;
    const int ns = EXACT ? NSMAX : K.ns, nd = K.nd;
    ulonglong2 xin[NSMAX];
#pragma unroll
    for (int i = 0; i < NSMAX; i++)
        if (EXACT || i < ns) xin[i] = ld2(src + ((long long)g.rows.src_row[i] << g.logn));
    if (g.sub) {
        const u64* sub = g.sub + b * g.ssub + x;
#pragma unroll
        for (int i = 0; i < NSMAX; i++)
            if (EXACT || i < ns) {
                const u64 q = mods_c[K.src_mod[i]].q;
                const ulonglong2 w = ld2(sub + ((long long)g.sub_row[i] << g.logn));
                xin[i].x = sub_mod(xin[i].x, w.x, q);
                xin[i].y = sub_mod(xin[i].y, w.y, q);
            }
    }
    u64 y[NSMAX][2];
    double vf0 = 0.0, vf1 = 0.0;
#pragma unroll
    for (int i = 0; i < NSMAX; i++) {
        if (EXACT || i < ns) {
            const ModDev m = ld_mod(mods_c, K.src_mod[i]);
            ulonglong2 v = xin[i];
            if (K.centered) {
                v.x = add_mod(v.x, K.half_src[i], m.q);
                v.y = add_mod(v.y, K.half_src[i], m.q);
            }
            y[i][0] = mont_mul(v.x, K.shat_inv_m[i], m.q, m.qinv);
            y[i][1] = mont_mul(v.y, K.shat_inv_m[i], m.q, m.qinv);
            const double qf = K.qf[i], rf = K.rf[i];
            const double a0 = (double)y[i][0], a1 = (double)y[i][1];
            const double e0 = a0 * rf, e1 = a1 * rf;
            vf0 += __builtin_fma(__builtin_fma(-e0, qf, a0), rf, e0);
            vf1 += __builtin_fma(__builtin_fma(-e1, qf, a1), rf, e1);
        }
    }
    const int v0 = (int)(u64)vf0, v1 = (int)(u64)vf1;
    const int j0 = blockIdx.z * TGT;
    u32 ylo[SPLIT ? NSMAX : 1][2], yhi[SPLIT ? NSMAX : 1][2], ysum[SPLIT ? NSMAX : 1][2];
    if (SPLIT) {
#pragma unroll
        for (int i = 0; i < NSMAX; i++)
#pragma unroll
            for (int e = 0; e < 2; e++) {
                ylo[i][e] = (u32)y[i][e] & ((1u << 29) - 1);
                yhi[i][e] = (u32)(y[i][e] >> 29);
                ysum[i][e] = ylo[i][e] + yhi[i][e];
            }
    }
#pragma unroll
    for (int jj = 0; jj < TGT; jj++) {
        const int j = min(j0 + jj, nd - 1);
        const ModDev m = ld_mod(mods_c, K.dst_mod[j]);
        u64 h0 = 0, l0 = 0, h1 = 0, l1 = 0, r0 = 0, r1 = 0;
#if defined(LSA_BC_DIAG_NO_MATH)
        if (SPLIT) {
            st2(dst + ((long long)g.rows.dst_row[j] << g.logn), xin[jj % NSMAX].x + v0, xin[jj % NSMAX].y + v1);
            continue;
        }
#endif
        if (SPLIT) {
            constexpr bool KARA = NSMAX <= 8;
            u64 c0[2] = {0, 0}, c1[2] = {0, 0}, c2[2] = {0, 0};
#pragma unroll
            for (int i = 0; i < NSMAX; i++) {
                if (EXACT || i < ns) {
                    const u32 w0 = K.shat_lo[j][i], w1 = K.shat_hi[j][i], ws = K.shat_sum[j][i];
#pragma unroll
                    for (int e = 0; e < 2; e++) {
                        c0[e] += (u64)ylo[i][e] * w0;
                        c2[e] += (u64)yhi[i][e] * w1;
                        if (KARA) {
                            c1[e] += (u64)ysum[i][e] * ws;
                        } else {
                            c1[e] += (u64)ylo[i][e] * w1;
                            c1[e] += (u64)yhi[i][e] * w0;
                        }
                    }
                }
            }
            u64 hs[2], ls[2];
            const u64 cr[2] = {(u64)(u32)v0 * K.corr_a[j] + K.corr_b[j], (u64)(u32)v1 * K.corr_a[j] + K.corr_b[j]};
#pragma unroll
            for (int e = 0; e < 2; e++) {
                const u64 mid = KARA ? c1[e] - c0[e] - c2[e] : c1[e];
#if defined(LSA_BC_CARRY_COMPARES)
                const u64 a = c0[e] + (mid << 29);
                const u64 b = a + (c2[e] << 58);
                const u64 d = b + cr[e];
                ls[e] = d;
                hs[e] = (mid >> 35) + (c2[e] >> 6) + (a < c0[e] ? 1 : 0) + (b < a ? 1 : 0) + (d < b ? 1 : 0);
#else
                const unsigned __int128 sum = (unsigned __int128)c0[e] + ((unsigned __int128)mid << 29) + ((unsigned __int128)c2[e] << 58) + cr[e];
                ls[e] = (u64)sum;
                hs[e] = (u64)(sum >> 64);
#endif
            }
            r0 = csub(mont_redc_lazy(hs[0], ls[0], m.q, m.qinv), m.q);
            r1 = csub(mont_redc_lazy(hs[1], ls[1], m.q, m.qinv), m.q);
#if defined(LSA_BC_DIAG_NO_STORE)
            if (r0 == 0x123456789abcdefull) st2(dst + ((long long)g.rows.dst_row[j] << g.logn), r0, r1);
#else
            st2(dst + ((long long)g.rows.dst_row[j] << g.logn), r0, r1);
#endif
            continue;
        } else {
#pragma unroll
        for (int i = 0; i < NSMAX; i++) {
            if (EXACT || i < ns) {
                const u64 w = K.shat_m[j][i];
                mac128(h0, l0, y[i][0], w);
                mac128(h1, l1, y[i][1], w);
                if ((i & 7) == 7) {
                    r0 = add_mod(r0, csub(mont_redc_lazy(h0, l0, m.q, m.qinv), m.q), m.q);
                    r1 = add_mod(r1, csub(mont_redc_lazy(h1, l1, m.q, m.qinv), m.q), m.q);
                    h0 = l0 = h1 = l1 = 0;
                }
            }
        }
        r0 = add_mod(r0, csub(mont_redc_lazy(h0, l0, m.q, m.qinv), m.q), m.q);
        r1 = add_mod(r1, csub(mont_redc_lazy(h1, l1, m.q, m.qinv), m.q), m.q);
        }
        r0 = sub_mod(r0, K.vs[j][v0], m.q);
        r1 = sub_mod(r1, K.vs[j][v1], m.q);
        if (K.centered) {
            r0 = sub_mod(r0, K.half_dst[j], m.q);
            r1 = sub_mod(r1, K.half_dst[j], m.q);
        }
        st2(dst + ((long long)g.rows.dst_row[j] << g.logn), r0, r1);
    }
}

template <int NSMAX, int TGT>
static void launch_baseconv_nt(int ns, int nd, bool split, dim3 grid, hipStream_t s, const BaseConvArgs& g) {
    grid.z = (unsigned)((nd + TGT - 1) / TGT);
    if (split) {
        if (ns == NSMAX) hipLaunchKernelGGL((k_baseconv<NSMAX, true, TGT, true>), grid, dim3(TPB), 0, s, g);
        else hipLaunchKernelGGL((k_baseconv<NSMAX, false, TGT, true>), grid, dim3(TPB), 0, s, g);
        return;
    }
    if (ns == NSMAX) hipLaunchKernelGGL((k_baseconv<NSMAX, true, TGT>), grid, dim3(TPB), 0, s, g);
    else hipLaunchKernelGGL((k_baseconv<NSMAX, false, TGT>), grid, dim3(TPB), 0, s, g);
}
static int baseconv_targets_per_block(int nd) {
    const int cand[3] = {4, 7, 13};
    int best = 4;
    double best_cost = 1e30;
    for (int T : cand) {
        const double cost = (double)((nd + T - 1) / T) * (2.5 + T);
        if (cost < best_cost) {
            best_cost = cost;
            best = T;
        }
    }
    return best;
}
template <int NSMAX>
static void launch_baseconv_ns(int ns, int nd, bool split, dim3 grid, hipStream_t s, const BaseConvArgs& g) {
    const int best = baseconv_targets_per_block(nd);
    if (best == 4) launch_baseconv_nt<NSMAX, 4>(ns, nd, split, grid, s, g);
    else if (best == 7) launch_baseconv_nt<NSMAX, 7>(ns, nd, split, grid, s, g);
    else launch_baseconv_nt<NSMAX, 13>(ns, nd, split, grid, s, g);
}

template <int NSMAX, bool EXACT, int TGT>
__global__ __launch_bounds__(TPB) void k_baseconv_wide(BaseConvArgs g) {
    const LSA_CONST_AS BaseConvConsts& K = *(const LSA_CONST_AS BaseConvConsts*)g.k;
    const LSA_CONST_AS ModDev* const mods_c = (const LSA_CONST_AS ModDev*)g.mods;
    const int x = blockIdx.x * TPB + threadIdx.x;
    const long long b = blockIdx.y;
    const u64* src = g.src + b * g.ssrc + x;
    u64* dst = g.dst + b * g.sdst + x;
    const int ns = EXACT ? NSMAX : K.ns, nd = K.nd;
    u64 y[NSMAX];
#pragma unroll
    for (int i = 0; i < NSMAX; i++)
        if (EXACT || i < ns) y[i] = src[(long long)g.rows.src_row[i] << g.logn];
    if (g.sub) {
        const u64* sub = g.sub + b * g.ssub + x;
#pragma unroll
        for (int i = 0; i < NSMAX; i++)
            if (EXACT || i < ns) y[i] = sub_mod(y[i], sub[(long long)g.sub_row[i] << g.logn], mods_c[K.src_mod[i]].q);
    }
    double vf = 0.0;
#pragma unroll
    for (int i = 0; i < NSMAX; i++) {
        if (EXACT || i < ns) {
            const ModDev m = ld_mod(mods_c, K.src_mod[i]);
            u64 v = y[i];
            if (K.centered) v = add_mod(v, K.half_src[i], m.q);
            y[i] = mont_mul(v, K.shat_inv_m[i], m.q, m.qinv);
            const double qf = K.qf[i], rf = K.rf[i];
            const double a = (double)y[i];
            const double e = a * rf;
            vf += __builtin_fma(__builtin_fma(-e, qf, a), rf, e);
        }
    }
    const int v = (int)(u64)vf;
    const int j0 = blockIdx.z * TGT;
#pragma unroll
    for (int jj = 0; jj < TGT; jj++) {
        const int j = min(j0 + jj, nd - 1);
        const ModDev m = ld_mod(mods_c, K.dst_mod[j]);
        u64 h = 0, l = 0, r = 0;
#pragma unroll
        for (int i = 0; i < NSMAX; i++) {
            if (EXACT || i < ns) {
                mac128(h, l, y[i], K.shat_m[j][i]);
                if ((i & 7) == 7) {
                    r = add_mod(r, csub(mont_redc_lazy(h, l, m.q, m.qinv), m.q), m.q);
                    h = l = 0;
                }
            }
        }
        r = add_mod(r, csub(mont_redc_lazy(h, l, m.q, m.qinv), m.q), m.q);
        r = sub_mod(r, K.vs[j][v], m.q);
        if (K.centered) r = sub_mod(r, K.half_dst[j], m.q);
        dst[(long long)g.rows.dst_row[j] << g.logn] = r;
    }
}

template <int NSMAX, int TGT>
static void launch_baseconv_wide_nt(int ns, int nd, dim3 grid, hipStream_t s, const BaseConvArgs& g) {
    grid.z = (unsigned)((nd + TGT - 1) / TGT);
    if (ns == NSMAX) hipLaunchKernelGGL((k_baseconv_wide<NSMAX, true, TGT>), grid, dim3(TPB), 0, s, g);
    else hipLaunchKernelGGL((k_baseconv_wide<NSMAX, false, TGT>), grid, dim3(TPB), 0, s, g);
}
template <int NSMAX>
static void launch_baseconv_wide_ns(int ns, int nd, dim3 grid, hipStream_t s, const BaseConvArgs& g) {
    const int best = baseconv_targets_per_block(nd);
    if (best == 4) launch_baseconv_wide_nt<NSMAX, 4>(ns, nd, grid, s, g);
    else if (best == 7) launch_baseconv_wide_nt<NSMAX, 7>(ns, nd, grid, s, g);
    else launch_baseconv_wide_nt<NSMAX, 13>(ns, nd, grid, s, g);
}

void launch_baseconv(Context& c, const BaseConvPlan* k, const BaseConvRows& rows, const u64* src, u64* dst, int batch,
                     long long ssrc, long long sdst, hipStream_t s, const u64* sub, long long ssub, const int* sub_row) {
    if (batch <= 0) return;
    BaseConvArgs g{};
    g.sub = sub;
    g.ssub = ssub;
    LSA_REQUIRE(!sub || sub_row, "base conversion: subtrahend rows missing");
    if (sub)
        for (int i = 0; i < k->ns; i++) g.sub_row[i] = sub_row[i];
    g.k = k->dev;
    g.mods = c.d_mods;
    g.src = src;
    g.dst = dst;
    g.ssrc = ssrc;
    g.sdst = sdst;
    g.logn = c.logn;
    g.rows = rows;
    ProfScope ps(c, PROF_BASECONV, 8.0 * c.n * batch * (double)(k->ns * (sub ? 2 : 1) + k->nd), s);
    const int ns = k->ns, nd = k->nd;
    if (ns > LSA_BC_NARROW_SRC) {
        const dim3 grid((unsigned)(c.n / TPB), (unsigned)batch, 1);
        if (ns <= 24) launch_baseconv_wide_ns<24>(ns, nd, grid, s, g);
        else launch_baseconv_wide_ns<LSA_BC_MAX_SRC>(ns, nd, grid, s, g);
        LSA_HIP(hipGetLastError());
        return;
    }
    const dim3 grid((unsigned)(c.n / (2 * TPB)), (unsigned)batch, 1);
    if (ns <= 1) launch_baseconv_ns<1>(ns, nd, k->split29, grid, s, g);
    else if (ns <= 2) launch_baseconv_ns<2>(ns, nd, k->split29, grid, s, g);
    else if (ns <= 3) launch_baseconv_ns<3>(ns, nd, k->split29, grid, s, g);
    else if (ns <= 4) launch_baseconv_ns<4>(ns, nd, k->split29, grid, s, g);
    else if (ns <= 5) launch_baseconv_ns<5>(ns, nd, k->split29, grid, s, g);
    else if (ns <= 8) launch_baseconv_ns<8>(ns, nd, k->split29, grid, s, g);
    else if (ns <= 12) launch_baseconv_ns<12>(ns, nd, k->split29, grid, s, g);
    else launch_baseconv_ns<LSA_BC_NARROW_SRC>(ns, nd, k->split29, grid, s, g);
    LSA_HIP(hipGetLastError());
}

struct KsMacArgs {
    const u64* cx;
    const u64* ext;
    const u64* key;
    u64* acc;
    long long scx, sext, sacc;
    const ModDev* mods;
    int logn, L, np, nq, beta, kcomp, klvl, batch, bpt;
    int n_tl;
    unsigned char tl_list[64];
    const unsigned* scatter;
    const u64* base;
    const u64* pm;
    long long sbase;
    const u64* fa;
    const u64* fb;
    long long sfa, sfb, pfa, pfb;
    const u64* pf;
};

template <int KB, bool EXT = false, bool FOLD = false, bool EXT_ACC = false>
__global__ __launch_bounds__(TPB) void k_ks_mac(KsMacArgs g) {
    const int chunks = (1 << g.logn) / (2 * TPB);
    const int tl = g.n_tl ? g.tl_list[blockIdx.x / chunks] : blockIdx.x / chunks;
    const int x = ((blockIdx.x % chunks) * TPB + threadIdx.x) * 2;
    const int T = g.L + g.np;
    const int mi = tl < g.L ? tl : g.nq + (tl - g.L);
    const int kj = tl < g.L ? tl : g.klvl + 1 + (tl - g.L);
    const ModDev m = g.mods[mi];
    const long long N = 1LL << g.logn;
    const int own_d = tl < g.L ? tl / g.np : -1;
    ulonglong2 k0[KB > 0 ? KB : 1], k1[KB > 0 ? KB : 1];
    constexpr bool in_regs = KB > 0;
    if constexpr (in_regs) {
#pragma unroll
        for (int d = 0; d < KB; d++) {
            if (d < g.beta) {
                const u64* pk = g.key + ((long long)(d * 2) * g.kcomp + kj) * N + x;
                k0[d] = ld2(pk);
                k1[d] = ld2(pk + (long long)g.kcomp * N);
            }
        }
    }
    const int b_begin = blockIdx.y * g.bpt;
    const int b_end = min(g.batch, b_begin + g.bpt);
    ulonglong2 en[KB > 0 ? KB : 1];
    ulonglong2 fn[FOLD ? 4 : 1];
    auto fetch = [&](long long b) {
        if constexpr (in_regs) {
#pragma unroll
            for (int d = 0; d < KB; d++)
                if (d < g.beta && !(FOLD && d == own_d))
                    en[d] = ld2(d == own_d ? g.cx + b * g.scx + tl * N + x : g.ext + b * g.sext + ((long long)d * T + tl) * N + x);
        }
        if constexpr (FOLD) {
            if (own_d >= 0) {
                const u64* pa = g.fa + b * g.sfa + tl * N + x;
                const u64* pb = g.fb + b * g.sfb + tl * N + x;
                fn[0] = ld2(pa);
                fn[1] = ld2(pa + g.pfa);
                fn[2] = ld2(pb);
                fn[3] = ld2(pb + g.pfb);
            }
        }
    };
    auto own_d2 = [&](const ulonglong2& a1, const ulonglong2& b1) {
        return ulonglong2{mont_mul(a1.x, mont_mul_lazy(b1.x, m.r2, m.q, m.qinv), m.q, m.qinv),
                          mont_mul(a1.y, mont_mul_lazy(b1.y, m.r2, m.q, m.qinv), m.q, m.qinv)};
    };
    if (b_begin < b_end) fetch(b_begin);
    for (long long b = b_begin; b < b_end; b++) {
        u64 h00 = 0, l00 = 0, h01 = 0, l01 = 0, h10 = 0, l10 = 0, h11 = 0, l11 = 0;
        u64 r00 = 0, r01 = 0, r10 = 0, r11 = 0;
        ulonglong2 fc[FOLD ? 4 : 1];
        if constexpr (FOLD) {
            if constexpr (in_regs) {
#pragma unroll
                for (int i = 0; i < 4; i++) fc[i] = fn[i];
            } else if (own_d >= 0) {
                const u64* pa = g.fa + b * g.sfa + tl * N + x;
                const u64* pb = g.fb + b * g.sfb + tl * N + x;
                fc[0] = ld2(pa);
                fc[1] = ld2(pa + g.pfa);
                fc[2] = ld2(pb);
                fc[3] = ld2(pb + g.pfb);
            }
        }
        if constexpr (in_regs) {
            ulonglong2 ec[KB > 0 ? KB : 1];
#pragma unroll
            for (int d = 0; d < KB; d++) ec[d] = en[d];
            if (b + 1 < b_end) fetch(b + 1);
            if constexpr (FOLD) {
                if (own_d >= 0) {
#pragma unroll
                    for (int d = 0; d < KB; d++)
                        if (d == own_d) ec[d] = own_d2(fc[1], fc[3]);
                }
            }
#pragma unroll
            for (int d = 0; d < KB; d++) {
                if (d < g.beta) {
                    const ulonglong2 e = ec[d];
#if defined(LSA_KS_DIAG_NO_MATH)
                    l00 += e.x ^ k0[d].x; l01 += e.y ^ k0[d].y; l10 += e.x ^ k1[d].x; l11 += e.y ^ k1[d].y;
#else
                    mac128(h00, l00, e.x, k0[d].x);
                    mac128(h01, l01, e.y, k0[d].y);
                    mac128(h10, l10, e.x, k1[d].x);
                    mac128(h11, l11, e.y, k1[d].y);
#endif
                }
            }
        } else {
            for (int d = 0; d < g.beta; d++) {
                const u64* pe = d == own_d ? g.cx + b * g.scx + tl * N + x : g.ext + b * g.sext + ((long long)d * T + tl) * N + x;
                const ulonglong2 e = FOLD && d == own_d ? own_d2(fc[1], fc[3]) : ld2(pe);
                const u64* pk = g.key + ((long long)(d * 2) * g.kcomp + kj) * N + x;
                const ulonglong2 kk0 = ld2(pk), kk1 = ld2(pk + (long long)g.kcomp * N);
                mac128(h00, l00, e.x, kk0.x);
                mac128(h01, l01, e.y, kk0.y);
                mac128(h10, l10, e.x, kk1.x);
                mac128(h11, l11, e.y, kk1.y);
                if ((d & 7) == 7) {
                    r00 = add_mod(r00, csub(mont_redc_lazy(h00, l00, m.q, m.qinv), m.q), m.q);
                    r01 = add_mod(r01, csub(mont_redc_lazy(h01, l01, m.q, m.qinv), m.q), m.q);
                    r10 = add_mod(r10, csub(mont_redc_lazy(h10, l10, m.q, m.qinv), m.q), m.q);
                    r11 = add_mod(r11, csub(mont_redc_lazy(h11, l11, m.q, m.qinv), m.q), m.q);
                    h00 = l00 = h01 = l01 = h10 = l10 = h11 = l11 = 0;
                }
            }
        }
#if defined(LSA_KS_DIAG_NO_MATH)
        r00 = l00; r01 = l01; r10 = l10; r11 = l11;
#else
        r00 = add_mod(r00, csub(mont_redc_lazy(h00, l00, m.q, m.qinv), m.q), m.q);
        r01 = add_mod(r01, csub(mont_redc_lazy(h01, l01, m.q, m.qinv), m.q), m.q);
        r10 = add_mod(r10, csub(mont_redc_lazy(h10, l10, m.q, m.qinv), m.q), m.q);
        r11 = add_mod(r11, csub(mont_redc_lazy(h11, l11, m.q, m.qinv), m.q), m.q);
#endif
        if constexpr (FOLD) {
            if (own_d >= 0) {
                const u64 pm = g.pf[tl];
                const u64 p0x = mont_mul(fc[2].x, pm, m.q, m.qinv), p0y = mont_mul(fc[2].y, pm, m.q, m.qinv);
                const u64 p1x = mont_mul(fc[3].x, pm, m.q, m.qinv), p1y = mont_mul(fc[3].y, pm, m.q, m.qinv);
                r00 = add_mod(r00, mont_mul(fc[0].x, p0x, m.q, m.qinv), m.q);
                r01 = add_mod(r01, mont_mul(fc[0].y, p0y, m.q, m.qinv), m.q);
                r10 = add_mod(r10, add_mod(mont_mul(fc[0].x, p1x, m.q, m.qinv), mont_mul(fc[1].x, p0x, m.q, m.qinv), m.q), m.q);
                r11 = add_mod(r11, add_mod(mont_mul(fc[0].y, p1y, m.q, m.qinv), mont_mul(fc[1].y, p0y, m.q, m.qinv), m.q), m.q);
            }
// ... 848 lines not shown
```

lattisense_amd/csrc/key_switch.hip:

```cpp
#include "key_switch.h"

namespace lsa {

RowMap rm_seq(int count, int first) {
    RowMap r;
    LSA_REQUIRE(count >= 1 && count <= LSA_MAX_PERIOD, "row map too long");
    r.period = count;
    for (int i = 0; i < count; i++) r.mod_of[i] = (unsigned char)(first + i);
    return r;
}

static void ks_moddown_head(Context& c, int level, u64* acc, long long s_acc, u64* conv, const KsOut& o, int nb, hipStream_t s) {
    LSA_REQUIRE(!o.scatter || (c.fuse_tails && o.form == KsOut::NTT), "scattered ModDown store: fused tails, NTT-domain output");
    LSA_REQUIRE(!o.rmac || o.scatter, "rotate-and-MAC tail: needs the rotation's index map");
    LSA_REQUIRE(!o.coeff_gather || o.form == KsOut::COEFF, "gathered ModDown tail: coefficient-domain output");
    LSA_REQUIRE(!o.slot_tail || (o.form == KsOut::COEFF && !o.coeff_gather && o.base && o.base_polys == 2 && o.base_rpp == level + 1),
                "slot-sum ModDown tail: coefficient-domain output on a whole ciphertext");
    LSA_REQUIRE(o.form != KsOut::RESCALE || (c.fuse_tails && level >= 1 && ((o.base && o.base_polys == 2) || (!o.base && o.base_polys == 0))),
                "merged ModDown+rescale: unsupported shape");
    const bool coeff_out = o.form == KsOut::COEFF, rs = o.form == KsOut::RESCALE;
    const long long N = c.n;
    const int L = level + 1, np = c.np, T = L + np;
    const long long s_conv = 2LL * L * N;
    {
        RowMap rm;
        rm.period = 2 * T;
        for (int h = 0; h < 2; h++)
            for (int tl = 0; tl < T; tl++)
                rm.mod_of[h * T + tl] = tl >= L ? (unsigned char)c.p_mod(tl - L)
                                                : (coeff_out ? (unsigned char)tl
                                                             : (rs && tl == level ? (unsigned char)level : LSA_ROW_SKIP));
        launch_ntt(c, acc, acc, nb, s_acc, 2 * T, rm, true, s);
    }
    {
        std::vector<int> src, dst;
        BaseConvRows rows{};
        for (int i = 0; i < np; i++) {
            rows.src_row[i] = L + i;
            src.push_back(c.p_mod(i));
        }
        for (int j = 0; j < L; j++) {
            rows.dst_row[j] = j;
            dst.push_back(j);
        }
        const BaseConvPlan* k = c.baseconv(src, dst, true, rs);
        for (int h = 0; h < 2; h++)
            launch_baseconv(c, k, rows, acc + (size_t)h * T * N, conv + (size_t)h * L * N, nb, s_acc, s_conv, s);
    }
}

static NttFusion ks_rescale_head(Context& c, int level, u64* acc, long long s_acc, u64* conv, const KsOut& o, int nb, hipStream_t s,
                                 RowMap& rmo);

static void ks_moddown(Context& c, int level, u64* acc, long long s_acc, u64* conv, const KsOut& o, int nb, hipStream_t s) {
    const bool coeff_out = o.form == KsOut::COEFF, rs = o.form == KsOut::RESCALE;
    const long long N = c.n;
    const int L = level + 1, T = L + c.np;
    const long long s_conv = 2LL * L * N;
    ks_moddown_head(c, level, acc, s_acc, conv, o, nb, s);
    if (coeff_out) {
        if (o.slot_tail)
            launch_bfv_slot_tail(c, level, *o.slot_tail, acc, s_acc, T, conv, s_conv, o.base, o.sbase, o.p, o.sp, nb, s);
        else if (o.coeff_gather)
            launch_moddown_final_perm(c, level, o.coeff_gather, acc, s_acc, T, conv, s_conv, o.base, o.sbase, o.base_rpp,
                                      o.base_polys, o.p, o.sp, nb, s);
        else
            launch_moddown_final(c, level, acc, s_acc, T, conv, s_conv, o.base, o.sbase, o.base_rpp, o.base_polys, o.p, o.sp, nb, s);
        return;
    }
    if (rs) {
        RowMap rmo;
        const NttFusion fb = ks_rescale_head(c, level, acc, s_acc, conv, o, nb, s, rmo);
        launch_ntt(c, conv, conv, nb, s_conv, s_conv, 2 * L, rmo, false, s, &fb);
    } else if (c.fuse_tails) {
        NttFusion fz;
        fz.epi = 1;
        fz.limbs = L;
        fz.a = acc;
        fz.a_stride = s_acc;
        fz.a_rpp = T;
        fz.base = o.base;
        fz.base_stride = o.sbase;
        fz.base_rpp = o.base_rpp;
        fz.base_polys = o.base_polys;
        fz.k = c.pinv_vec(level);
        fz.out = o.p;
        fz.out_stride = o.sp;
        fz.out_rpp = L;
        fz.scatter = o.scatter;
        if (o.rmac) {
            fz.epi = 4;
            fz.pt = o.rmac->pt;
            fz.pt_stride = o.rmac->spt;
            fz.accumulate = o.rmac->accumulate;
        }
        launch_ntt(c, conv, conv, nb, s_conv, s_conv, 2 * L, rm_seq(L), false, s, &fz);
    } else {
        launch_ntt(c, conv, conv, nb, s_conv, 2 * L, rm_seq(L), false, s);
        launch_moddown_final(c, level, acc, s_acc, T, conv, s_conv, o.base, o.sbase, o.base_rpp, o.base_polys, o.p, o.sp, nb, s);
    }
}

static NttFusion ks_rescale_head(Context& c, int level, u64* acc, long long s_acc, u64* conv, const KsOut& o, int nb, hipStream_t s,
                                 RowMap& rmo) {
    const long long N = c.n;
    const int L = level + 1, T = L + c.np;
    const long long s_conv = 2LL * L * N;
    const int l = level;
    if (o.base) {
        u64* base_rw = const_cast<u64*>(o.base);
        RowMap rb;
        rb.period = 1;
        rb.mod_of[0] = (unsigned char)l;
        rb.row0 = l;
        rb.row_step = o.base_rpp;
        launch_ntt(c, base_rw, base_rw, nb, o.sbase, o.sbase, 2, rb, true, s);
    }
    const unsigned char lm[1] = {(unsigned char)l};
    launch_sub_mul_general(c, 2, 1, lm, c.pinv_vec(level) + l, acc + (long long)l * N, s_acc, T, conv + (long long)l * N,
                           s_conv, L, o.base ? o.base + (long long)l * N : nullptr, o.sbase, o.base_rpp, o.base_polys,
                           o.p + (long long)l * N, o.sp, L, nb, s);
    rmo.period = 2 * L;
    for (int h = 0; h < 2; h++)
        for (int j = 0; j < L; j++) rmo.mod_of[h * L + j] = j == l ? LSA_ROW_SKIP : (unsigned char)j;
    NttFusion fb;
    fb.pro = 2;
    fb.epi = 2;
    fb.limbs = L;
    fb.ql_mod = l;
    fb.last = o.p + (long long)l * N;
    fb.last_stride = o.sp;
    fb.last_rpp = L;
    fb.a = acc;
    fb.a_stride = s_acc;
    fb.a_rpp = T;
    fb.base = o.base;
    fb.base_stride = o.sbase;
    fb.base_rpp = o.base_rpp;
    fb.base_polys = o.base_polys;
    fb.k = c.pinv_vec(level);
    fb.k2 = c.qlinv_vec(level);
    fb.out = o.rs.out;
    fb.out_stride = o.rs.sout;
    fb.out_rpp = level;
    return fb;
}

bool ks_fuse_mac(const Context& c, int level, const Key& key) {
    const int L = level + 1, T = L + c.np, beta = ceil_div(L, c.np);
    if (!ks_fused_enabled(c) || !ks_fused_engines(c) || (c.fp64_ntt && !key.fp) || beta * T > LSA_MAX_PERIOD || T > 64) return false;
    for (int tl = 0; tl < T; tl++)
        if (ks_fused_limb(c, L, tl)) return true;
    return false;
}

size_t KsTile::rows(const Context& c, int level, KsSource::Form form) {
    LSA_REQUIRE(c.np >= 1, "key switching needs at least one special prime");
    const int L = level + 1, T = L + c.np, beta = ceil_div(L, c.np);
    return (form == KsSource::COEFF ? (size_t)L : 0) + (size_t)L + (size_t)beta * T + 2 * (size_t)T + 2 * (size_t)L;
}

KsTile::KsTile(Context& c_, int level_, int nb_, u64* ws, hipStream_t s_, const Key* single_key, KsSource::Form form, int tb)
    : c(c_), level(level_), nb(nb_), s(s_), key(single_key) {
    LSA_REQUIRE(c.np >= 1, "key switching needs at least one special prime");
    LSA_REQUIRE(level >= 0 && level < c.nq, "level out of range");
    const long long N = c.n;
    L = level + 1;
    T = L + c.np;
    beta = ceil_div(L, c.np);
    fused = key && ks_fuse_mac(c, level, *key);
    s_cxi = (long long)L * N;
    s_ext = (long long)beta * T * N;
    s_acc = 2LL * T * N;
    s_conv = 2LL * L * N;
    cxn = form == KsSource::COEFF ? ws : nullptr;
    cxi = cxn ? ws + (size_t)(tb ? tb : nb) * s_cxi : ws;
    ext = cxi + (size_t)nb * s_cxi;
    acc = ext + (size_t)nb * s_ext;
    conv = acc + (size_t)nb * s_acc;
}

void KsTile::decompose(const KsSource& source) {
    LSA_REQUIRE((source.form == KsSource::COEFF) == (cxn != nullptr), "key switch: the tile was laid out for another form of source");
    src = source;
    const long long N = c.n;
    const int np = c.np;
    if (src.form == KsSource::COEFF) {
        launch_ntt(c, src.coef, cxn, nb, src.s_coef, s_cxi, L, rm_seq(L), false, s);
        src.ntt = cxn;
        src.s_ntt = s_cxi;
    } else if (src.form == KsSource::PRODUCT) {
        src.ntt = cxi;
        src.s_ntt = s_cxi;
    }
    const u64* cx_coef = src.coef;
    if (src.prod) {
        LSA_REQUIRE(!cx_coef, "key switch: a product source has no coefficient-domain copy");
        const TensorFold* prod = src.prod;
        NttFusion fz;
        fz.pro = 3;
        fz.limbs = L;
        fz.a = prod->a + prod->pa;
        fz.a_stride = prod->sa;
        fz.a_rpp = (int)(prod->pa >> c.logn);
        fz.b = prod->b + prod->pb;
        fz.b_stride = prod->sb;
        fz.b_rpp = (int)(prod->pb >> c.logn);
        launch_ntt(c, cxi, cxi, nb, s_cxi, s_cxi, L, rm_seq(L), true, s, &fz);
    } else if (!cx_coef) {
        launch_ntt(c, src.ntt, cxi, nb, src.s_ntt, s_cxi, L, rm_seq(L), true, s);
    }
    const u64* conv_src = cx_coef ? cx_coef : cxi;
    const long long s_src = cx_coef ? src.s_coef : s_cxi;
    const bool lift_on = c.modup_lift != 0;
    auto lifted = [&](int d) { return lift_on && std::min(d * np + np, L) - d * np == 1 && (c.T.mods[d * np].q >> 53) == 0; };
    bool any_lift = false, any_conv = false;
    for (int d = 0; d < beta; d++) {
        if (lifted(d)) {
            any_lift = true;
            continue;
        }
        any_conv = true;
        const int d0 = d * np, d1 = std::min(d0 + np, L);
        std::vector<int> from, dst;
        BaseConvRows rows{};
        for (int i = d0; i < d1; i++) {
            rows.src_row[i - d0] = i;
            from.push_back(i);
        }
        for (int tl = 0; tl < T; tl++) {
            if (tl >= d0 && tl < d1) continue;
            rows.dst_row[dst.size()] = d * T + tl;
            dst.push_back(c.qp_mod(L, tl));
        }
        launch_baseconv(c, c.baseconv(from, dst, false), rows, conv_src, ext, nb, s_src, s_ext, s);
    }
    auto own = [&](int d, int tl) { return tl >= d * np && tl < std::min((d + 1) * np, L); };
    NttFusion lf;
    lf.pro = 4;
    lf.limbs = T;
    lf.last = conv_src;
    lf.last_stride = s_src;
    lf.last_rpp = np;
    lf.ql_mod = 0;
    if (beta * T <= LSA_MAX_PERIOD) {
        RowMap rm, rl;
        rm.period = rl.period = beta * T;
        for (int d = 0; d < beta; d++)
            for (int tl = 0; tl < T; tl++) {
                const unsigned char m = own(d, tl) ? LSA_ROW_SKIP : (unsigned char)c.qp_mod(L, tl);
                rm.mod_of[d * T + tl] = lifted(d) ? LSA_ROW_SKIP : m;
                rl.mod_of[d * T + tl] = lifted(d) ? m : LSA_ROW_SKIP;
            }
        if (any_conv) launch_ntt(c, ext, ext, nb, s_ext, s_ext, beta * T, rm, false, s, nullptr, fused ? 1 : 3);
        if (any_lift) launch_ntt(c, ext, ext, nb, s_ext, s_ext, beta * T, rl, false, s, &lf, fused ? 1 : 3);
        if (!fused) return;
        bool any = false;
        for (int i = 0; i < beta * T; i++) {
            const bool in_mac = ks_fused_limb(c, L, i % T) && !(tail && i % T == level);
            rm.mod_of[i] = own(i / T, i % T) || in_mac ? LSA_ROW_SKIP : (unsigned char)c.qp_mod(L, i % T);
            any |= rm.mod_of[i] != LSA_ROW_SKIP;
        }
        if (any) launch_ntt(c, ext, ext, nb, s_ext, s_ext, beta * T, rm, false, s, nullptr, 2);
        return;
    }
    for (int d = 0; d < beta; d++) {
        RowMap rm;
        rm.period = T;
        for (int tl = 0; tl < T; tl++) rm.mod_of[tl] = own(d, tl) ? LSA_ROW_SKIP : (unsigned char)c.qp_mod(L, tl);
        lf.last = conv_src + (size_t)d * np * N;
        lf.ql_mod = d * np;
        launch_ntt(c, ext + (size_t)d * T * N, ext + (size_t)d * T * N, nb, s_ext, s_ext, T, rm, false, s, lifted(d) ? &lf : nullptr);
    }
}

void KsTile::mac(const Key& k) {
    LSA_REQUIRE(src.ntt, "key MAC: decompose() has not run on this tile");
    const TensorFold* fold = src.prod;
    if (!fused) {
        launch_ks_mac(c, level, src.ntt, src.s_ntt, ext, s_ext, k, {acc, s_acc}, nb, s, false, fold);
        return;
    }
    LSA_REQUIRE(&k == key && !tail, "fused key MAC: the tile was planned for another key or for mac_rescale()");
    LSA_REQUIRE(launch_ntt_ksmac(c, level, src.ntt, src.s_ntt, ext, s_ext, k, acc, s_acc, nb, s, fold), "fused key MAC: shape not covered");
    launch_ks_mac(c, level, src.ntt, src.s_ntt, ext, s_ext, k, {acc, s_acc}, nb, s, true, fold);
}

void KsTile::mac_ext(const Key& k, const KsMacDst& dst) {
    LSA_REQUIRE(src.ntt && !fused && dst.scatter, "extended key MAC: a decomposed, unfused tile and the rotation's index map");
    launch_ks_mac(c, level, src.ntt, src.s_ntt, ext, s_ext, k, dst, nb, s);
}

void KsTile::mac_ext_multi(int n_keys, const KsMacMultiKey* keys, long long sout, const u64* base, long long sbase) {
    LSA_REQUIRE(src.ntt && !fused, "extended key MAC: a decomposed, unfused tile");
    launch_ks_mac_multi(c, level, src.ntt, src.s_ntt, ext, s_ext, n_keys, keys, sout, base, sbase, nb, s);
}

void KsTile::moddown_of(u64* ext_acc, long long s_ext_acc, const KsOut& o) { ks_moddown(c, level, ext_acc, s_ext_acc, conv, o, nb, s); }

void KsTile::moddown_ext(Context& c, int level, u64* ext_acc, long long s_ext_acc, u64* conv, const KsOut& o, int nb, hipStream_t s) {
    ks_moddown(c, level, ext_acc, s_ext_acc, conv, o, nb, s);
}

bool KsTile::plan_tail(const KsOut& o) {
    const int mu = c.plan.pass[1].mu;
    tail = fused && c.ks_tail_in_mac != 0 && c.fuse_tails && level >= 1 && o.form == KsOut::RESCALE && !o.base && o.base_polys == 0 &&
           ks_fused_engines(c) == 2 && (mu == 8 || (mu == 7 && c.ks_tail_in_mac == 2));
    if (!tail) return false;
    tail = false;
    for (int j = 0; j < level; j++) tail |= ks_fused_limb(c, L, j);
    return tail;
}

void KsTile::mac_rescale(const Key& k, const KsOut& o) {
    LSA_REQUIRE(src.ntt && fused && tail && &k == key, "tail in the key MAC: a decomposed tile planned for it and for this key");
    LSA_REQUIRE(o.form == KsOut::RESCALE && !o.base && o.base_polys == 0, "tail in the key MAC: a merged rescale without base");
    const TensorFold* fold = src.prod;
    LSA_REQUIRE(launch_ntt_ksmac(c, level, src.ntt, src.s_ntt, ext, s_ext, k, acc, s_acc, nb, s, fold, KS_FUSED_P), "fused key MAC: shape not covered");
    launch_ks_mac(c, level, src.ntt, src.s_ntt, ext, s_ext, k, {acc, s_acc}, nb, s, true, fold, level);
    ks_moddown_head(c, level, acc, s_acc, conv, o, nb, s);
    RowMap rmo;
    const NttFusion fb = ks_rescale_head(c, level, acc, s_acc, conv, o, nb, s, rmo);
    NttFusion fp = fb;
    fp.epi = 0;
    launch_ntt(c, conv, conv, nb, s_conv, s_conv, 2 * L, rmo, false, s, &fp, 1);
    const KsTailOperands kt{conv, s_conv, o.rs.out, o.rs.sout};
    LSA_REQUIRE(launch_ntt_ksmac(c, level, src.ntt, src.s_ntt, ext, s_ext, k, acc, s_acc, nb, s, fold, KS_FUSED_Q_TAIL, &kt),
                "fused key MAC: tail shape not covered");
    for (int i = 0; i < 2 * L; i++)
        if (rmo.mod_of[i] != LSA_ROW_SKIP && c.fp_engine(rmo.mod_of[i])) rmo.mod_of[i] = LSA_ROW_SKIP;
    NttFusion fe = fb;
    fe.pro = 0;
    fe.last = nullptr;
    launch_ntt(c, conv, conv, nb, s_conv, s_conv, 2 * L, rmo, false, s, &fe, 2);
}

void key_switch(Context& c, int level, const KsSource& src, const Key& key, const KsOut& o, int nb, u64* ws, hipStream_t s) {
    KsTile t(c, level, nb, ws, s, &key, src.form);
    const bool tail = t.plan_tail(o);
    t.decompose(src);
    if (tail) {
        t.mac_rescale(key, o);
        return;
    }
    t.mac(key);
    t.moddown(o);
}

const u32* inverse_perm(Context& c, u64 g) {
    const u64 mask = 2 * (u64)c.n - 1;
    u64 inv = g;
    for (int i = 0; i < 6; i++) inv = (inv * (2 - g * inv)) & mask;
    LSA_REQUIRE(((inv * g) & mask) == 1, "Galois element without an inverse");
    return c.ntt_perm(inv);
}
const u32* rotation_scatter(Context& c, u64 g) {
    return sw::rot_scatter() && c.fuse_tails ? inverse_perm(c, g) : nullptr;
}

void rescale(Context& c, int level, int polys, const u64* in, long long sin, u64* out, long long sout, int nb,
             bool ntt_domain, u64* ws, hipStream_t s) {
    LSA_REQUIRE(level >= 1 && level < c.nq, "rescale needs level >= 1");
    const long long N = c.n;
    const int L = level + 1;
    u64* last = ws;
    u64* tmp = last + (size_t)nb * polys * N;
    const long long s_last = (long long)polys * N, s_tmp = (long long)polys * level * N;
    std::vector<int> rows(polys);
    for (int p = 0; p < polys; p++) rows[p] = p * L + level;
    launch_copy_rows(c, in, sin, last, s_last, polys, rows.data(), nb, s);
    if (ntt_domain) {
        RowMap rm;
        rm.period = 1;
        rm.mod_of[0] = (unsigned char)level;
        launch_ntt(c, last, last, nb, s_last, polys, rm, true, s);
    }
    if (ntt_domain && c.fuse_tails) {
        NttFusion fz;
        fz.pro = 1;
        fz.epi = 1;
        fz.limbs = level;
        fz.ql_mod = level;
        fz.last = last;
        fz.last_stride = s_last;
        fz.a = in;
        fz.a_stride = sin;
        fz.a_rpp = L;
        fz.k = c.qlinv_vec(level);
        fz.out = out;
        fz.out_stride = sout;
        fz.out_rpp = level;
        launch_ntt(c, tmp, tmp, nb, s_tmp, s_tmp, polys * level, rm_seq(level), false, s, &fz);
        return;
    }
    launch_rescale_prep(c, level, polys, last, s_last, tmp, s_tmp, nb, s);
    if (ntt_domain) launch_ntt(c, tmp, tmp, nb, s_tmp, polys * level, rm_seq(level), false, s);
    launch_rescale_final(c, level, polys, in, sin, tmp, s_tmp, out, sout, nb, s);
}

int pick_tile(const Context& c, size_t rows_per_ct, int batch) {
    if (c.tile_batch > 0) return std::min(c.tile_batch, batch);
    const size_t bytes_per_ct = rows_per_ct * (size_t)c.n * sizeof(u64);
    size_t tb = (8ull << 30) / std::max<size_t>(bytes_per_ct, 1);
    if (tb < 1) tb = 1;
    const size_t cap = std::min<size_t>(512, std::max<size_t>(64, (64ull << 16) / (size_t)c.n));
    if (tb > cap) tb = cap;
    return (int)std::min<size_t>(tb, (size_t)batch);
}

}
```

lattisense_amd/csrc/lsa_internal.h:

```cpp
#pragma once
#include <hip/hip_runtime.h>
#include <cstdint>
#include <map>
#include <memory>
#include <mutex>
#include <stdexcept>
#include <string>
#include <vector>

#include "../../include/lattisense_amd.h"
#include "galois_keys.h"
#include "ntt_plan.h"
#include "ntt_chunk.h"
#include "plain_ops.h"
#include "slot_sum.h"
#include "switches.h"
#include "tables.h"

namespace lsa {

void set_last_error(const std::string& m);

#define LSA_HIP(expr)                                                                                     \
    do {                                                                                                  \
        hipError_t _e = (expr);                                                                           \
        if (_e != hipSuccess)                                                                             \
            throw lsa::Error(_e == hipErrorNoDevice || _e == hipErrorInvalidDevice ? LSA_ERR_NO_DEVICE    \
                                                                                   : LSA_ERR_HIP,        \
                             std::string(#expr) + ": " + hipGetErrorString(_e));                          \
    } while (0)

#define LSA_REQUIRE(cond, msg)                                   \
    do {                                                         \
        if (!(cond)) throw lsa::Error(LSA_ERR_ARG, (msg));       \
    } while (0)

#define LSA_BC_NARROW_SRC 16
#define LSA_BC_MAX_SRC 32
#define LSA_BC_MAX_DST 64

struct BaseConvConsts {
    int ns, nd, centered;
    int src_mod[LSA_BC_MAX_SRC];
    int dst_mod[LSA_BC_MAX_DST];
    u64 shat_inv_m[LSA_BC_MAX_SRC];
    u64 half_src[LSA_BC_MAX_SRC];
    double qf[LSA_BC_MAX_SRC];
    double rf[LSA_BC_MAX_SRC];
    u64 shat_m[LSA_BC_MAX_DST][LSA_BC_MAX_SRC];
    u64 vs[LSA_BC_MAX_DST][LSA_BC_MAX_SRC + 1];
    u64 half_dst[LSA_BC_MAX_DST];
    int split29;
    u32 shat_lo[LSA_BC_MAX_DST][LSA_BC_MAX_SRC];
    u32 shat_hi[LSA_BC_MAX_DST][LSA_BC_MAX_SRC];
    u32 shat_sum[LSA_BC_MAX_DST][LSA_BC_MAX_SRC];
    u64 corr_a[LSA_BC_MAX_DST], corr_b[LSA_BC_MAX_DST];
};

struct BaseConvPlan {
    BaseConvConsts* dev = nullptr;
    int ns = 0, nd = 0;
    bool split29 = false;
};

enum ProfKind { PROF_NTT = 0, PROF_BASECONV = 1, PROF_KSMAC = 2, PROF_TENSOR = 3, PROF_ELEMWISE = 4, LSA_PROF_KINDS = 5 };

struct Key {
    u64* data = nullptr;
    int level = 0;
    bool owned = true;
    const double* fp = nullptr;
};

using GaloisKeys = GaloisKeySet<Key>;

struct Context {
    int algo, n, logn, nq, np, nmul, nmod, device;
    u64 t;
    HostTables T;
    NttPlan plan;
    NttPlan plan_wide;
    int wide_mode = 2;
    ModDev* d_mods = nullptr;
    u64* d_psi = nullptr;
    u64* d_psiinv = nullptr;
    u64* d_scale = nullptr;
    double* d_psi_d = nullptr;
    double* d_psiinv_d = nullptr;
    u64* d_psi_w = nullptr;
    u64* d_psiinv_w = nullptr;
    double* d_psi_d_w = nullptr;
    double* d_psiinv_d_w = nullptr;
    double* d_scale_d = nullptr;
    int fp64_ntt = 1;
    int tile_batch = 0;
    int fp_raw = 1;
    int modup_lift = 1;
    int fuse_tails = 1;
    int ks_tail_in_mac = 1;
    int dual_stream = 0;
    hipStream_t aux_stream = nullptr;
    hipEvent_t ev_fork = nullptr, ev_join = nullptr;
    void fork_aux(hipStream_t s);
    void join_aux(hipStream_t s);
    unsigned long long* ntt_diag = nullptr;
    int ntt_chunk_mib = 0;
    int bfv_dot_chunk = 0;

    struct ProfSample {
        hipEvent_t e0, e1;
        int kid;
        double bytes;
        double bytes_primary;
    };
    bool prof_on = false;
    int prof_stride = 1;
    long long prof_launched[LSA_PROF_KINDS] = {0};
    std::vector<ProfSample> prof_samples;
    std::vector<hipEvent_t> prof_pool;

    std::mutex mu;
    std::map<std::string, BaseConvPlan> bconv;
    std::map<u64, u32*> perm_ntt;
    std::map<u64, u32*> perm_coeff;
    std::map<std::string, u64*> consts;
    struct CconstSelector {
        int bit = -1, pol = 0;
        std::vector<u64> I;
    } cconst;

    std::shared_ptr<const BfvEncodeTables> bfv_enc;

    u64* ws = nullptr;
    size_t ws_words = 0;

    Context(int algo_, int n_, const u64* q, int nq_, const u64* p, int np_, u64 t_, int device_);
    ~Context();
    void use_device() const { LSA_HIP(hipSetDevice(device)); }
    u64* workspace(size_t words, hipStream_t s);
    u64* ws2 = nullptr;
    size_t ws2_words = 0;
    u64* workspace2(size_t words, hipStream_t s);
    int p_mod(int i) const { return nq + i; }
    int aux_mod(int i) const { return nq + np + i; }
    int qp_mod(int L, int tl) const { return tl < L ? tl : p_mod(tl - L); }
    bool fp_engine(int mod) const { return fp64_ntt && (T.mod[mod] >> LSA_FP64_MAX_BITS) == 0; }
    struct BaseConvFold {
        std::string tag;
        std::vector<u64> src_pre, dst_scale;
    };
    const BaseConvPlan* baseconv(const std::vector<int>& src, const std::vector<int>& dst, bool centered,
                                 bool pinv_scaled = false, const BaseConvFold* fold = nullptr);
    const u64* pinv_vec(int level);
    const u64* pmodq_vec(int level);
    const u64* pfold_vec(int level);
    const u64* qlinv_vec(int level);
    const u64* tail_fp_vec(int level);
    const u32* ntt_perm(u64 g);
    const u32* coeff_perm(u64 g);
    const u64* const_vec(const std::string& name, const std::vector<int>& mods, const std::vector<u64>& plain_vals);
    const u64* raw_vec(const std::string& name, const std::vector<u64>& vals);
};

struct ProfScope {
    Context& c;
    hipStream_t s;
    bool active = false;
    Context::ProfSample smp{};
    ProfScope(Context& c_, int kid, double bytes, hipStream_t s_, double bytes_primary = -1.0) : c(c_), s(s_) {
        if (!c.prof_on) return;
        const long long idx = c.prof_launched[kid]++;
        if (c.prof_stride > 1 && ((unsigned long long)(idx + 1) * 0x9E3779B97F4A7C15ull >> 33) % (unsigned)c.prof_stride != 0) return;
        auto take = [&]() {
            hipEvent_t e;
            if (!c.prof_pool.empty()) {
                e = c.prof_pool.back();
                c.prof_pool.pop_back();
            } else {
                LSA_HIP(hipEventCreate(&e));
            }
            return e;
        };
        smp.e0 = take();
        smp.e1 = take();
        smp.kid = kid;
        smp.bytes = bytes;
        smp.bytes_primary = bytes_primary < 0 ? bytes : bytes_primary;
        LSA_HIP(hipEventRecord(smp.e0, s));
        active = true;
    }
    ~ProfScope() {
        if (!active) return;
        (void)hipEventRecord(smp.e1, s);
        c.prof_samples.push_back(smp);
    }
};

struct RowMap {
    int period;
    unsigned char mod_of[LSA_MAX_PERIOD];
    int row0 = 0, row_step = 1;
};

void launch_ntt(Context& c, const u64* src, u64* dst, int batch, long long batch_stride, int rows, const RowMap& rm,
                bool inverse, hipStream_t s);
struct NttFusion {
    int epi = 0, pro = 0, limbs = 1, base_polys = 0, ql_mod = 0;
    const u64* a = nullptr;
    long long a_stride = 0;
    int a_rpp = 0;
    const u64* base = nullptr;
    long long base_stride = 0;
    int base_rpp = 0;
    const u64* k = nullptr;
    u64* out = nullptr;
    long long out_stride = 0;
    int out_rpp = 0;
    const u64* last = nullptr;
    long long last_stride = 0;
    int last_rpp = 1;
    const u64* k2 = nullptr;
    const u32* scatter = nullptr;
    const u64* pt = nullptr;
    long long pt_stride = 0;
    bool accumulate = false;
    const u64* b = nullptr;
    long long b_stride = 0;
    int b_rpp = 0;
};
void launch_ntt(Context& c, const u64* src, u64* dst, int batch, long long src_stride, long long dst_stride, int rows,
                const RowMap& rm, bool inverse, hipStream_t s, const NttFusion* fz = nullptr, int passes = 3);

enum EwOp { EW_ADD = 0, EW_SUB = 1, EW_NEG = 2, EW_MUL = 3 };
void launch_elementwise(Context& c, EwOp op, const u64* a, const u64* b, u64* out, int batch, long long sa,
                        long long sb, long long so, int rows, const RowMap& rm, hipStream_t s);
void launch_muladd(Context& c, EwOp op, const u64* a, const u64* b, const u64* acc, long long sacc, u64* out, int batch,
                   long long sa, long long sb, long long so, int rows, const RowMap& rm, hipStream_t s);
#define LSA_MAC_MAX_TERMS 16
#define LSA_MACM_MAX 8
void launch_mac_plain(Context& c, int terms, const u64* const* ct, const long long* sct, const u64* const* pt,
                      const long long* spt, const u64* partial, long long spartial, u64* out, long long so, int batch,
                      int polys, int limbs, const RowMap& rm, hipStream_t s);
void launch_mac_plain_multi(Context& c, int nb, const u64* const* ct, const long long* sct, int ng, const u64* const* pt,
                            u64* const* out, long long so, int batch, int polys, int limbs, const RowMap& rm, hipStream_t s,
                            bool accumulate = false);
void launch_poly_lincomb(Context& c, int nsrc, const u64* const* src, const long long* ss, const int* rpp, int n_out,
                         const u64* d_k, const u64* d_a, u64* out, int rows, int batch, hipStream_t s);
void launch_mont_muladd(Context& c, const u64* a, long long sa, const u64* pt, long long spt, const u64* acc, long long sacc,
                        u64* out, long long so, int batch, int polys, int limbs, const RowMap& rm, hipStream_t s);
void launch_lift_ringt(Context& c, int mode, int level, const u64* pt, long long spt, u64* out, long long sout, int batch,
                       hipStream_t s);
void launch_tensor(Context& c, const u64* a, const u64* b, u64* d, int batch, long long sa, long long sb, long long sd,
                   int limbs, const RowMap& rm, hipStream_t s, int a_rpp = 0, int b_rpp = 0);
void launch_tensor_sum(Context& c, int terms, const u64* const* a, const long long* sa, const int* a_rpp, const u64* const* b,
                       const long long* sb, const int* b_rpp, const u64* addend, long long s_addend, bool accumulate, u64* d,
                       long long sd, int batch, int limbs, const RowMap& rm, hipStream_t s);
struct TensorFold {
    const u64* a;
    const u64* b;
    long long sa, sb;
    long long pa, pb;
};
struct BaseConvRows {
    int src_row[LSA_BC_MAX_SRC];
    int dst_row[LSA_BC_MAX_DST];
};
void launch_baseconv(Context& c, const BaseConvPlan* k, const BaseConvRows& rows, const u64* src, u64* dst, int batch,
                     long long ssrc, long long sdst, hipStream_t s, const u64* sub = nullptr, long long ssub = 0,
                     const int* sub_row = nullptr);
struct KsMacDst {
    u64* out;
    long long sout;
    const u32* scatter = nullptr;
    const u64* base = nullptr;
    long long sbase = 0;
    bool accumulate = false;
};
void launch_ks_mac(Context& c, int level, const u64* cx, long long scx, const u64* ext, long long sext, const Key& key,
                   const KsMacDst& dst, int batch, hipStream_t s, bool unfused_only = false, const TensorFold* fold = nullptr,
                   int extra_tl = -1);
void launch_moddown_final(Context& c, int level, const u64* acc, long long sacc, int acc_rows_per_poly, const u64* conv,
                          long long sconv, const u64* base, long long sbase, int base_rows_per_poly, int base_polys,
                          u64* out, long long sout, int batch, hipStream_t s);
#define LSA_PERM_LDS_MAX_LOGN 14
void launch_moddown_final_perm(Context& c, int level, const u32* perm, const u64* acc, long long sacc, int acc_rows_per_poly,
                               const u64* conv, long long sconv, const u64* base, long long sbase, int base_rows_per_poly,
                               int base_polys, u64* out, long long sout, int batch, hipStream_t s);
void launch_sub_mul_general(Context& c, int polys, int limbs, const unsigned char* limb_mod, const u64* kvec,
                            const u64* a, long long sa, int a_rpp, const u64* b, long long sb, int b_rpp,
                            const u64* base, long long sbase, int base_rpp, int base_polys, u64* out, long long so,
                            int out_rpp, int batch, hipStream_t s);
void launch_rescale_prep(Context& c, int level, int polys, const u64* last, long long slast, u64* tmp, long long stmp,
                         int batch, hipStream_t s);
void launch_rescale_final(Context& c, int level, int polys, const u64* in, long long sin, const u64* tmp, long long stmp,
                          u64* out, long long sout, int batch, hipStream_t s);
void launch_permute_ntt(Context& c, const u32* perm, const u64* in, long long sin, u64* out, long long sout, int rows,
                        int batch, hipStream_t s);
void launch_permute_coeff(Context& c, const u32* perm, const u64* in, long long sin, u64* out, long long sout, int rows,
                          const RowMap& rm, int batch, hipStream_t s);
struct KsMacMultiKey {
    const Key* key;
    const u32* scatter;
    u64* out;
};
void launch_ks_mac_multi(Context& c, int level, const u64* cx, long long scx, const u64* ext, long long sext, int n_keys,
                         const KsMacMultiKey* keys, long long sout, const u64* base, long long sbase, int batch, hipStream_t s);
void launch_ext_sum(Context& c, int level, int n_in, const u64* const* in, long long sin, u64* out, long long sout, bool accumulate,
                    int batch, hipStream_t s);
void launch_permute_ext(Context& c, int level, const u32* perm, const u64* acc, long long sacc, const u64* base, long long sbase,
                        int base_polys, u64* out, long long sout, bool accumulate, int batch, hipStream_t s);
void launch_copy_rows(Context& c, const u64* in, long long sin, u64* out, long long sout, int rows, const int* src_row,
                      int batch, hipStream_t s);
void launch_to_mont(Context& c, u64* data, int rows, const RowMap& rm, hipStream_t s);
bool ks_fused_enabled(const Context& c);
struct KeyLayout {
    size_t words = 0;
    bool fp = false;
    size_t alloc_words() const { return fp ? 2 * words : words; }
    double* fp_of(u64* data) const { return fp ? reinterpret_cast<double*>(data + words) : nullptr; }
};
KeyLayout key_layout(const Context& c, int key_level);
void key_prepare(Context& c, Key& key, u64* data, int key_level, double* fp, hipStream_t s);
enum KsFusedLimbs { KS_FUSED_ALL = 0, KS_FUSED_P = 1, KS_FUSED_Q_TAIL = 2 };
struct KsTailOperands {
    const u64* conv;
    long long sconv;
    u64* out;
    long long sout;
};
bool launch_ntt_ksmac(Context& c, int level, const u64* cx, long long scx, u64* ext, long long sext, const Key& key, u64* acc,
                      long long sacc, int batch, hipStream_t s, const TensorFold* fold = nullptr, KsFusedLimbs limbs = KS_FUSED_ALL,
                      const KsTailOperands* tail = nullptr);
int ks_fused_engines(const Context& c);
bool ks_fuse_mac(const Context& c, int level, const Key& key);
bool ks_fused_limb(const Context& c, int L, int tl);
void launch_sub_mul_const(Context& c, const u64* a, long long sa, const u64* b, long long sb, const u64* kvec, u64* out,
                          long long so, int rows, const RowMap& rm, int batch, hipStream_t s);
void launch_mul_const(Context& c, const u64* a, long long sa, const u64* kvec, u64* out, long long so, int rows,
                      const RowMap& rm, int batch, hipStream_t s);
void launch_add_const(Context& c, const u64* a, long long sa, const u64* kvec, u64* out, long long so, int rows,
                      const RowMap& rm, int batch, hipStream_t s, const u64* mvec = nullptr);
void launch_lift_i64(Context& c, const long long* v, long long sv, u64* out, long long so, int limbs, int batch, hipStream_t s);
void launch_cconst(Context& c, bool mul, bool add, const u64* a, long long sa, const CconstLimb* k, int sel_bit, int sel_pol,
                   u64* out, long long so, int limbs, int batch, hipStream_t s);
void launch_probe_copy(u64* dst, const u64* src, size_t n, hipStream_t s);
void launch_probe_mulhi(u64* buf, size_t n, int iters, hipStream_t s);

struct Bootstrap;
Bootstrap* bootstrap_create(Context& c, int cts_depth, int stc_depth, int K, int double_angle, double message_ratio,
                            double in_scale, double out_scale, int log_slots, hipStream_t s, int sine_deg = 30, int arcsine_deg = 0);
const std::vector<double>& bootstrap_arcsine(const Bootstrap& bt);
bool bootstrap_is_sparse(const Bootstrap& bt);
void bootstrap_destroy(Bootstrap* b);
int bootstrap_out_level(const Bootstrap& bt);
double bootstrap_out_scale(const Bootstrap& bt);
const std::vector<u64>& bootstrap_galois(const Bootstrap& bt);
const std::vector<double>& bootstrap_chebyshev(const Bootstrap& bt);
int bootstrap_matrices(const Bootstrap& bt);
int bootstrap_cts_matrices(const Bootstrap& bt);
void bootstrap_matrix(const Bootstrap& bt, int i, int* level, int* n1, const std::vector<int>** ks, const std::vector<u64*>** plains,
                      int* rows = nullptr);
void bootstrap_run(Bootstrap& bt, const u64* in, long long sin, u64* out, long long sout, int batch, const Key& rlk,
                   const GaloisKeys& glk, const Key* swk_dts, const Key* swk_std, hipStream_t s);

const std::string& last_error();
void ckks_mult(Context& c, int level, const u64* a, const u64* b, u64* d3, int batch, long long sa, long long sb, long long sd,
               hipStream_t s);
void ckks_relin(Context& c, int level, const u64* d3, const Key& rlk, u64* out, int batch, long long sd, long long so,
                hipStream_t s);
void ckks_rescale(Context& c, int level, int polys, const u64* in, u64* out, int batch, long long sin, long long sout,
                  hipStream_t s);
void ckks_rotate(Context& c, int level, const u64* in, u64 g, const Key& glk, u64* out, int batch, long long sin,
                 long long sout, hipStream_t s);
void ckks_rotate_many(Context& c, int level, const u64* in, int n_rot, const u64* g, const Key* const* glk, u64* const* outs,
                      int batch, long long sin, long long sout, hipStream_t s);
void ckks_switch_key(Context& c, int level, const u64* in, const Key& swk, u64* out, int batch, long long sin, long long sout,
                     hipStream_t s);
void ckks_mult_relin_rescale(Context& c, int level, const u64* a, const u64* b, const Key& rlk, u64* out, int batch,
                             long long sa, long long sb, long long so, hipStream_t s);
void ckks_mult_relin_rescale_rpp(Context& c, int level, const u64* a, const u64* b, const Key& rlk, u64* out, int batch,
                                 long long sa, long long sb, long long so, hipStream_t s, int a_rpp, int b_rpp);
struct DotTerms {
    int n;
    const u64* const* as;
    const long long* sas;
    const int* a_rpp;
    const u64* const* bs;
    const long long* sbs;
    const int* b_rpp;
    const u64* addend;
    long long s_addend;
};
void ckks_mult_sum(Context& c, int level, const DotTerms& t, u64* d3, int batch, long long sd, hipStream_t s);
void ckks_dot(Context& c, int level, const DotTerms& t, const Key& rlk, u64* out, int batch, long long so, bool rescale,
              hipStream_t s);
void ckks_mult_plain(Context& c, int level, const u64* ct, long long sct, const u64* pt, long long spt, u64* out, long long so,
                     int batch, bool rescale, hipStream_t s);
void ckks_addsub_plain(Context& c, int op, int level, const u64* ct, long long sct, const u64* pt, long long spt, u64* out,
                       long long so, int batch, hipStream_t s);
void ckks_mac_plain(Context& c, int level, int n, const u64* const* cts, const long long* scts, const u64* const* pts,
                    const long long* spts, const u64* addend, long long s_addend, u64* out, long long so, int batch, bool rescale,
                    hipStream_t s);
void ckks_mult_const(Context& c, int level, const u64* ct, long long sct, double re, double im, double const_scale, u64* out,
                     long long so, int batch, bool rescale, hipStream_t s);
void ckks_add_const(Context& c, int level, const u64* ct, long long sct, double re, double im, double ct_scale, u64* out,
                    long long so, int batch, hipStream_t s);
void ckks_affine_const(Context& c, int level, const u64* ct, long long sct, double re, double im, double const_scale, double add_re,
                       double add_im, double ct_scale, u64* out, long long so, int batch, bool rescale, hipStream_t s);
void ckks_lift_ext(Context& c, int level, const u64* in, u64* out, int batch, long long sin, long long sout, hipStream_t s);
void ckks_rotate_many_ext(Context& c, int level, const u64* in, int n_rot, const u64* g, const Key* const* glk, u64* const* outs,
                          int batch, long long sin, long long sout, hipStream_t s, const u64* c1_coef = nullptr, long long s_coef = 0);
void ckks_rotate_ext(Context& c, int level, const u64* in, u64 g, const Key& glk, u64* out, bool accumulate, int batch,
                     long long sin, long long sout, hipStream_t s, bool scatter_mac = false);
void ckks_moddown_ext(Context& c, int level, u64* in, u64* out, int batch, long long sin, long long sout, hipStream_t s,
                      bool coeff_out = false);
struct SlotSum {
    Context& c;
    int level;
    SlotSumPlanHost plan;
    bool multi_mac = false;
    SlotSum(Context& ctx, int level_) : c(ctx), level(level_) {}
};
// ... 77 lines not shown
```

lattisense_amd/csrc/ntt_core.h:

```cpp
#pragma once
#include "modarith.h"

#ifndef LSA_NTT_THREADS
#define LSA_NTT_THREADS 256
#endif
#define LSA_MAX_PERIOD 192
#if defined(LSA_EMULATE)
#include <cstdio>
#include <cstdlib>
#define LSA_EMU_CHECK(c) do { if (!(c)) { std::fprintf(stderr, "ntt replay: range invariant violated: %s (%s:%d)\n", #c, __FILE__, __LINE__); std::abort(); } } while (0)
#else
#define LSA_EMU_CHECK(c) do { } while (0)
#endif
#define LSA_ROW_SKIP 0xFF
#define LSA_FP64_MAX_BITS 47
#ifndef LSA_NTT_MAX_RHO
#define LSA_NTT_MAX_RHO 4
#endif

struct NttPassArgs {
    const u64* src;
    u64* dst;
    long long src_stride;
    long long dst_stride;
// ... 85 lines not shown
#else
    x = p[0];
    y = p[1];
#endif
}
LSA_HD void ntt_load_pair(const u64* p, u64& x, u64& y) {
#if defined(__HIP_DEVICE_COMPILE__)
    const ulonglong2 v = *reinterpret_cast<const ulonglong2*>(p);
    x = v.x;
    y = v.y;
#else
    x = p[0];
    y = p[1];
#endif
}
#if defined(__HIP_DEVICE_COMPILE__)
#define LSA_CONST_PTR(T, p) ((const __attribute__((address_space(4))) T*)(p))
#else
#define LSA_CONST_PTR(T, p) (p)
#endif
LSA_HD void ntt_load_tw_fp(const double* tws, int s, int j, unsigned G, double* w) {
    const unsigned gv = ntt_tw_v_fp(j, G);
#if defined(__HIP_DEVICE_COMPILE__) && !defined(LSA_NTT_TW_NATURAL)
    if (j == 0) {
        w[0] = tws[gv];
        return;
    }
#pragma unroll
    for (int k = 0; k < (1 << j); k += 2) {
        const double2 v = *reinterpret_cast<const double2*>(tws + ntt_tw_u_fp(s, j, k) + gv);
        w[k] = v.x;
        w[k + 1] = v.y;
    }
#else
#pragma unroll
    for (int k = 0; k < (1 << j); k++) w[k] = (tws + ntt_tw_u_fp(s, j, k))[gv];
#endif
}

struct NttBlockCtx {
    long long base_src;
    long long base_dst;
    int tile;
    int mod;
    int fp;
    int b, row;
    const u64* tw_l;
};

LSA_HD NttBlockCtx ntt_decode_block(const NttPassArgs& a, long long bid) {
    NttBlockCtx c;
    int tiles = 1 << (a.logn - a.tau);
    int b = (int)(bid % a.batch);
    long long rt = bid / a.batch;
    int row;
    int ri;
    if (a.row_inner) {
        c.tile = (int)(rt / a.rows);
        ri = (int)(rt % a.rows);
    } else {
        c.tile = (int)(rt % tiles);
        ri = (int)(rt / tiles);
    }
    row = a.compact ? (int)a.row_tbl[ri] : a.row0 + ri * a.row_step;
    c.base_src = (long long)b * a.src_stride + ((long long)row << a.logn);
    c.base_dst = (long long)b * a.dst_stride + ((long long)row << a.logn);
    c.mod = a.mod_of[row % a.period];
    c.b = b;
    c.row = row;
    c.fp = 0;
    c.tw_l = nullptr;
    if (c.mod != LSA_ROW_SKIP) c.fp = a.allow_fp64 && (a.mods[c.mod].q >> LSA_FP64_MAX_BITS) == 0;
    return c;
}

LSA_HD int ntt_global_index(const NttPassArgs& a, int tile, int l) {
    if (a.lambda == 0) return (tile << a.tau) + l;
    const int lo_bits = a.logn - a.s_lo - a.mu;
    const int bph_bits = lo_bits - a.lambda;
    const int hi = tile >> bph_bits, lob = tile & ((1 << bph_bits) - 1);
    const int r = l >> a.lambda, c = l & ((1 << a.lambda) - 1);
    return (hi << (a.logn - a.s_lo)) + (r << lo_bits) + (lob << a.lambda) + c;
}
struct NttTileMap {
    int base, lambda, rshift, cmask;
};
LSA_HD NttTileMap ntt_tile_map(const NttPassArgs& a, int tile) {
    NttTileMap m;
    m.base = ntt_global_index(a, tile, 0);
    m.lambda = a.lambda;
    m.rshift = a.lambda ? a.logn - a.s_lo - a.mu : 0;
    m.cmask = (1 << a.lambda) - 1;
    return m;
}
LSA_HD int ntt_tile_index(const NttTileMap& m, int l) { return m.base + ((l >> m.lambda) << m.rshift) + (l & m.cmask); }

LSA_HD int ntt_hi_index(const NttPassArgs& a, int tile, int l) {
    if (a.lambda == 0) return ((tile << a.tau) + l) >> a.mu;
    int lo_bits = a.logn - a.s_lo - a.mu;
    return tile >> (lo_bits - a.lambda);
}

#if !defined(LSA_NTT_EXACT_BFLY) && !defined(LSA_NTT_NO_LAZY)
LSA_HD bool ntt_int_lazy(u64 q) { return (q >> 57) == 0; }
#else
LSA_HD bool ntt_int_lazy(u64) { return false; }
#endif

LSA_HD double d_from_bits(u64 b) {
#if defined(__HIP_DEVICE_COMPILE__)
    return __longlong_as_double((long long)b);
#else
    double d;
    __builtin_memcpy(&d, &b, 8);
    return d;
#endif
}
LSA_HD u64 d_to_bits(double d) {
#if defined(__HIP_DEVICE_COMPILE__)
    return (u64)__double_as_longlong(d);
#else
    u64 b;
    __builtin_memcpy(&b, &d, 8);
    return b;
#endif
}
LSA_HD double u52_to_double(u64 v) { return d_from_bits(v | 0x4330000000000000ull) - 4503599627370496.0; }
LSA_HD u64 double_to_u52(double r) { return d_to_bits(r + 4503599627370496.0) & 0x000FFFFFFFFFFFFFull; }
LSA_HD double fp_modmul(double v, double w, double q, double qinv) {
    const double h = v * w;
    const double l = __builtin_fma(v, w, -h);
    const double c = __builtin_rint(h * qinv);
    const double d = __builtin_fma(-c, q, h);
    return d + l;
}
LSA_HD double fp_reduce(double x, double q, double qinv) { return __builtin_fma(-__builtin_rint(x * qinv), q, x); }
LSA_HD double fp_merged_tail_product(double x, double sum, double bd, double kd, double k2d, double q, double qinv) {
    return fp_modmul(fp_modmul(sum, kd, q, qinv) - x + bd, k2d, q, qinv);
}
LSA_HD u64 fp_merged_tail(double x, double sum, double bd, double kd, double k2d, double q, double qinv, bool wide) {
    if (wide) {
        x = fp_reduce(x, q, qinv);
        sum = fp_reduce(sum, q, qinv);
    }
    double r = fp_reduce(fp_merged_tail_product(x, sum, bd, kd, k2d, q, qinv), q, qinv);
    if (r < 0) r += q;
    return double_to_u52(r);
}

#define LSA_NTT_STAGE_PAIRS 8
#ifndef LSA_NTT_HEAD_ROUNDS
#define LSA_NTT_HEAD_ROUNDS 2
#endif
struct NttLoadFix {
    bool head, add, fp, near, raw, fp_lift, lift;
    u64 ql, h, hq;
    double hd, qld;
    ModDev mi;
};
template <int NE>
LSA_HD void ntt_lift_block(const NttLoadFix& f, u64* v) {
    if (f.fp_lift && f.near) {
#pragma unroll
        for (int e = 0; e < NE; e++) {
            const double x = u52_to_double(v[e]);
            v[e] = d_to_bits(x >= f.qld ? x - f.qld : x);
        }
    } else if (f.fp_lift) {
#pragma unroll
        for (int e = 0; e < NE; e++) v[e] = d_to_bits(fp_reduce(u52_to_double(v[e]), f.qld, f.hd));
    } else if (f.near) {
#pragma unroll
        for (int e = 0; e < NE; e++) v[e] = csub(v[e], f.mi.q);
    } else {
#pragma unroll
        for (int e = 0; e < NE; e++) v[e] = reduce_u64(v[e], f.mi);
    }
    if (f.fp && !f.fp_lift) {
#pragma unroll
        for (int e = 0; e < NE; e++) v[e] = d_to_bits(u52_to_double(v[e]));
    }
}
LSA_HD u64 ntt_load_fix(const NttLoadFix& f, u64 v, u64 t) {
    if (f.lift) {
        ntt_lift_block<1>(f, &v);
        return v;
    }
    if (f.fp_lift) {
        const double td = u52_to_double(t);
        const double r = td > f.hd ? td - f.qld : td;
        return d_to_bits(f.add ? u52_to_double(v) + r : r);
    }
    if (f.head) {
        const u64 c = add_mod(t, f.h, f.ql);
        const u64 lift = sub_mod(f.near ? csub(c, f.mi.q) : reduce_u64(c, f.mi), f.hq, f.mi.q);
        v = f.add ? add_mod(v, lift, f.mi.q) : lift;
    }
    if (f.fp && !f.raw) v = d_to_bits(u52_to_double(v));
    return v;
}
template <bool FZ, int LIFT = 1>
LSA_HD NttLoadFix ntt_make_load_fix(const NttPassArgs& a, const NttBlockCtx& bc, const u64*& g, const u64*& gl) {
    g = a.src + bc.base_src;
    gl = g;
    NttLoadFix f;
    f.head = FZ && LIFT != 2 && (a.fz_pro == 1 || a.fz_pro == 2) && a.fz_first;
    f.add = f.head && a.fz_pro == 2;
    f.fp = bc.fp != 0;
    f.raw = f.fp && a.fp_raw_in;
    LSA_EMU_CHECK(!(a.fz_pro && a.fz_first && a.fp_raw_in));
    f.mi = a.mods[bc.mod];
    f.ql = f.h = f.hq = 0;
    f.hd = f.qld = 0.0;
    f.near = f.fp_lift = false;
    f.lift = FZ && LIFT != 0 && a.fz_pro == 4 && a.fz_first;
    if (f.lift) {
        const int poly = bc.row / a.fz_limbs;
        g = gl = a.fz_last + (long long)bc.b * a.fz_last_stride + ((long long)poly * a.fz_last_rpp << a.logn);
        f.ql = a.mods[a.fz_ql_mod + poly * a.fz_last_rpp].q;
        f.near = f.ql <= 2 * f.mi.q;
        f.fp_lift = f.fp && (f.ql >> 52) == 0;
        f.qld = (double)f.mi.q;
        f.hd = 1.0 / f.qld;
    }
    if (f.head) {
        gl = a.fz_last + (long long)bc.b * a.fz_last_stride + ((long long)(bc.row / a.fz_limbs) * a.fz_last_rpp << a.logn);
        if (!f.add) g = gl;
        f.ql = a.mods[a.fz_ql_mod].q;
        f.h = (f.ql - 1) >> 1;
        f.hq = reduce_u64(f.h, f.mi);
        f.near = f.ql <= 2 * f.mi.q;
        f.fp_lift = f.fp && (f.ql >> 48) == 0;
        f.hd = (double)f.h;
        f.qld = (double)f.ql;
    }
    return f;
}
struct NttProdFix {
    const u64* pa;
    const u64* pb;
    ModDev mi;
    double qd, qinvd;
    bool fp;
};
LSA_HD NttProdFix ntt_make_prod_fix(const NttPassArgs& a, const NttBlockCtx& bc) {
    const int poly = bc.row / a.fz_limbs, limb = bc.row % a.fz_limbs;
    NttProdFix p;
    p.pa = a.fz_a + (long long)bc.b * a.fz_a_stride + (((long long)poly * a.fz_a_rpp + limb) << a.logn);
    p.pb = a.fz_b + (long long)bc.b * a.fz_b_stride + (((long long)poly * a.fz_b_rpp + limb) << a.logn);
    p.mi = a.mods[bc.mod];
    p.fp = bc.fp != 0;
    p.qd = (double)p.mi.q;
    p.qinvd = 1.0 / p.qd;
    LSA_EMU_CHECK(!a.fp_raw_in);
    return p;
}
LSA_HD u64 ntt_prod_fix(const NttProdFix& p, u64 x, u64 y) {
    LSA_EMU_CHECK(x < p.mi.q && y < p.mi.q);
    if (p.fp) return d_to_bits(fp_reduce(fp_modmul(u52_to_double(x), u52_to_double(y), p.qd, p.qinvd), p.qd, p.qinvd));
    return mont_mul(x, mont_mul_lazy(y, p.mi.r2, p.mi.q, p.mi.qinv), p.mi.q, p.mi.qinv);
}
template <bool FZ, int NT, bool PR = false>
LSA_HD void ntt_phase_load(const NttPassArgs& a, const NttBlockCtx& bc, int tid, u64* lds) {
    const u64* g;
    const u64* gl;
    const int half = 1 << (a.tau - 1);
    if (PR && a.fz_pro == 3 && a.fz_first) {
        const NttProdFix pf = ntt_make_prod_fix(a, bc);
        const NttTileMap tm = ntt_tile_map(a, bc.tile);
        if (half == LSA_NTT_STAGE_PAIRS * NT) {
            constexpr int CH = LSA_NTT_STAGE_PAIRS / LSA_NTT_HEAD_ROUNDS;
#pragma unroll 1
            for (int p0 = 0; p0 < LSA_NTT_STAGE_PAIRS; p0 += CH) {
                u64 sa[2 * CH], sb[2 * CH];
#pragma unroll
                for (int p = 0; p < CH; p++) {
                    const int x = ntt_tile_index(tm, 2 * (tid + (p0 + p) * NT));
                    ntt_load_data_pair(pf.pa + x, sa[2 * p], sa[2 * p + 1]);
                    ntt_load_data_pair(pf.pb + x, sb[2 * p], sb[2 * p + 1]);
                }
#pragma unroll
                for (int p = 0; p < CH; p++) {
                    const int l = 2 * (tid + (p0 + p) * NT);
                    lds[lds_addr(l)] = ntt_prod_fix(pf, sa[2 * p], sb[2 * p]);
                    lds[lds_addr(l + 1)] = ntt_prod_fix(pf, sa[2 * p + 1], sb[2 * p + 1]);
                }
            }
            return;
        }
        for (int i = tid; i < half; i += NT) {
            const int x = ntt_tile_index(tm, 2 * i);
            lds[lds_addr(2 * i)] = ntt_prod_fix(pf, pf.pa[x], pf.pb[x]);
            lds[lds_addr(2 * i + 1)] = ntt_prod_fix(pf, pf.pa[x + 1], pf.pb[x + 1]);
        }
        return;
    }
    const NttLoadFix f = ntt_make_load_fix<FZ>(a, bc, g, gl);
    const NttTileMap tm = ntt_tile_map(a, bc.tile);
    if (half == LSA_NTT_STAGE_PAIRS * NT && !f.add) {
        NttLoadFix f1 = f;
        f1.add = false;
        u64 st[2 * LSA_NTT_STAGE_PAIRS];
#pragma unroll
        for (int p = 0; p < LSA_NTT_STAGE_PAIRS; p++) {
            const int x = ntt_tile_index(tm, 2 * (tid + p * NT));
            ntt_load_data_pair(g + x, st[2 * p], st[2 * p + 1]);
        }
        if (FZ && f.lift) {
            ntt_lift_block<2 * LSA_NTT_STAGE_PAIRS>(f, st);
#pragma unroll
            for (int p = 0; p < LSA_NTT_STAGE_PAIRS; p++) {
                const int l = 2 * (tid + p * NT);
                lds[lds_addr(l)] = st[2 * p];
                lds[lds_addr(l + 1)] = st[2 * p + 1];
            }
            return;
        }
#pragma unroll
        for (int p = 0; p < LSA_NTT_STAGE_PAIRS; p++) {
            const int l = 2 * (tid + p * NT);
            lds[lds_addr(l)] = ntt_load_fix(f1, st[2 * p], st[2 * p]);
            lds[lds_addr(l + 1)] = ntt_load_fix(f1, st[2 * p + 1], st[2 * p + 1]);
        }
        return;
    }
    if (half == LSA_NTT_STAGE_PAIRS * NT) {
        constexpr int CH = LSA_NTT_STAGE_PAIRS / LSA_NTT_HEAD_ROUNDS;
#pragma unroll 1
        for (int p0 = 0; p0 < LSA_NTT_STAGE_PAIRS; p0 += CH) {
            u64 st[2 * CH], sl[2 * CH];
#pragma unroll
            for (int p = 0; p < CH; p++) {
                const int x = ntt_tile_index(tm, 2 * (tid + (p0 + p) * NT));
                ntt_load_data_pair(g + x, st[2 * p], st[2 * p + 1]);
                ntt_load_data_pair(gl + x, sl[2 * p], sl[2 * p + 1]);
            }
            if (f.fp_lift) {
#pragma unroll
                for (int p = 0; p < CH; p++) {
                    const int l = 2 * (tid + (p0 + p) * NT);
#pragma unroll
                    for (int h = 0; h < 2; h++) {
                        const double td = u52_to_double(sl[2 * p + h]);
                        const double r = td > f.hd ? td - f.qld : td;
                        lds[lds_addr(l + h)] = d_to_bits(u52_to_double(st[2 * p + h]) + r);
                    }
                }
            } else {
// ... 618 lines not shown
```

lattisense_amd/device.py:

```python
import ctypes

import numpy as np

from . import _native
from ._native import check, lib

ALGO_BFV, ALGO_CKKS = 0, 1


class DeviceBuffer:
    def __init__(self, ctx, nwords):
        self.ctx = ctx
        self.nwords = int(nwords)
        p = ctypes.c_void_p()
        check(lib().lsa_malloc(ctx.h, ctypes.byref(p), self.nwords * 8))
        self.ptr = p.value

    def free(self):
        if self.ptr:
            check(lib().lsa_free(self.ctx.h, self.ptr))
            self.ptr = None

    def __del__(self):
        try:
            self.free()
        except Exception:
            pass


class DeviceContext:

    def __init__(self, algo, n, q, p, t=0, device=0):
        self.algo, self.n, self.q, self.p, self.t = algo, int(n), list(q), list(p), int(t)
        qa = (ctypes.c_uint64 * len(q))(*q)
        pa = (ctypes.c_uint64 * max(1, len(p)))(*p)
        h = ctypes.c_void_p()
        check(lib().lsa_context_create(algo, self.n, qa, len(q), pa, len(p), self.t, device, ctypes.byref(h)))
        self.h = h
        self.stream = None
        cnt = ctypes.c_int()
        out = (ctypes.c_uint64 * 256)()
        check(lib().lsa_context_moduli(self.h, out, 256, ctypes.byref(cnt)))
        self.moduli = [int(out[i]) for i in range(cnt.value)]

    def close(self):
        if self.h:
            check(lib().lsa_context_destroy(self.h))
            self.h = None

    def __del__(self):
        try:
            self.close()
        except Exception:
            pass

    def alloc(self, nwords):
        return DeviceBuffer(self, nwords)

    def upload(self, arr):
        arr = np.ascontiguousarray(arr, dtype=np.uint64)
        buf = self.alloc(arr.size)
        check(lib().lsa_memcpy_h2d(self.h, buf.ptr, arr.ctypes.data, arr.nbytes, self.stream))
        self.sync()
        return buf

    def download(self, buf, shape):
        out = np.empty(shape, dtype=np.uint64)
        assert out.size <= buf.nwords
        check(lib().lsa_memcpy_d2h(self.h, out.ctypes.data, buf.ptr, out.nbytes, self.stream))
        return out

    def sync(self):
        check(lib().lsa_stream_synchronize(self.h, self.stream))

    def set_tile_batch(self, tb):
        check(lib().lsa_set_tile_batch(self.h, tb))

    def set_ntt_chunk_mib(self, mib):
        check(lib().lsa_set_ntt_chunk_mib(self.h, int(mib)))

    def baseconv_plans(self):
        cnt = ctypes.c_int()
        check(lib().lsa_debug_baseconv_plans(self.h, 0, ctypes.byref(cnt), None, None, None))
        n = cnt.value
        ns, nd, sp = (ctypes.c_int * max(n, 1))(), (ctypes.c_int * max(n, 1))(), (ctypes.c_int * max(n, 1))()
        check(lib().lsa_debug_baseconv_plans(self.h, n, ctypes.byref(cnt), ns, nd, sp))
        return [(ns[i], nd[i], bool(sp[i])) for i in range(min(n, cnt.value))]

    def key_switch_fused(self, level, key):
        out = ctypes.c_int()
        check(lib().lsa_debug_key_switch_fused(self.h, level, key, ctypes.byref(out)))
        return bool(out.value)

    def set_modup_lift(self, enable):
        check(lib().lsa_set_modup_lift(self.h, int(enable)))

    def set_ks_tail_in_mac(self, mode):
        check(lib().lsa_set_ks_tail_in_mac(self.h, int(mode)))

    def set_bfv_dot_chunk(self, pairs):
        check(lib().lsa_set_bfv_dot_chunk(self.h, int(pairs)))

    def set_fp64_ntt(self, enable):
        check(lib().lsa_set_fp64_ntt(self.h, int(enable)))

    def upload_key(self, compact, key_level):
        compact = np.ascontiguousarray(compact, dtype=np.uint64)
        assert compact.nbytes == lib().lsa_key_bytes(self.h, key_level), "key shape does not match its level"
        k = ctypes.c_void_p()
        check(lib().lsa_key_upload(self.h, compact.ctypes.data, key_level, self.stream, ctypes.byref(k)))
        return k

    def adopt_key(self, dev_ptr, key_level):
        k = ctypes.c_void_p()
        check(lib().lsa_key_adopt_device(self.h, dev_ptr, key_level, self.stream, ctypes.byref(k)))
        return k

    def key_bytes(self, key_level):
        return lib().lsa_key_bytes(self.h, key_level)

    def destroy_key(self, k):
        check(lib().lsa_key_destroy(self.h, k))

    def ntt(self, buf, batch, rows, mod_of, inverse=False, batch_stride=None):
        mo = (ctypes.c_int * len(mod_of))(*mod_of)
        bs = rows * self.n if batch_stride is None else batch_stride
        check(lib().lsa_ntt(self.h, buf.ptr, batch, bs, rows, mo, len(mod_of), int(inverse), self.stream))

    def addsub(self, op, level, polys, a, b, batch):
        L = level + 1
        out = self.alloc(batch * polys * L * self.n)
        s = polys * L * self.n
        check(lib().lsa_poly_addsub(self.h, op, level, polys, a.ptr, b.ptr if b is not None else None, out.ptr,
                                    batch, s, s, s, self.stream))
        return out

    def ckks_mult(self, level, a, b, batch):
        L = level + 1
        out = self.alloc(batch * 3 * L * self.n)
        check(lib().lsa_ckks_mult(self.h, level, a.ptr, b.ptr, out.ptr, batch, 2 * L * self.n, 2 * L * self.n,
                                  3 * L * self.n, self.stream))
        return out

    def ckks_relin(self, level, d3, rlk, batch):
        L = level + 1
        out = self.alloc(batch * 2 * L * self.n)
        check(lib().lsa_ckks_relin(self.h, level, d3.ptr, rlk, out.ptr, batch, 3 * L * self.n, 2 * L * self.n,
                                   self.stream))
        return out

    def ckks_rescale(self, level, polys, ct, batch):
        L = level + 1
        out = self.alloc(batch * polys * level * self.n)
        check(lib().lsa_ckks_rescale(self.h, level, polys, ct.ptr, out.ptr, batch, polys * L * self.n,
                                     polys * level * self.n, self.stream))
        return out

    def ckks_rotate_many(self, level, ct, keys, batch):
        L = level + 1
        outs = {g: self.alloc(batch * 2 * L * self.n) for g in keys}
        els = (ctypes.c_uint64 * len(keys))(*keys.keys())
        hk = (ctypes.c_void_p * len(keys))(*[k.value for k in keys.values()])
        po = (ctypes.c_void_p * len(keys))(*[o.ptr for o in outs.values()])
        check(lib().lsa_ckks_rotate_many(self.h, level, ct.ptr, len(keys), els, hk, po, batch, 2 * L * self.n, 2 * L * self.n,
                                         self.stream))
        return outs

    def ckks_rotate(self, level, ct, g, glk, batch):
        L = level + 1
        out = self.alloc(batch * 2 * L * self.n)
        check(lib().lsa_ckks_rotate(self.h, level, ct.ptr, g, glk, out.ptr, batch, 2 * L * self.n, 2 * L * self.n,
                                    self.stream))
        return out

    def drop_level(self, level, polys, ct, batch):
        L = level + 1
        out = self.alloc(batch * polys * level * self.n)
        check(lib().lsa_drop_level(self.h, level, polys, ct.ptr, out.ptr, batch, polys * L * self.n,
                                   polys * level * self.n, self.stream))
        return out

    def ckks_mult_relin_rescale(self, level, a, b, rlk, batch, out=None):
        L = level + 1
        if out is None:
            out = self.alloc(batch * 2 * level * self.n)
        check(lib().lsa_ckks_mult_relin_rescale(self.h, level, a.ptr, b.ptr, rlk, out.ptr, batch, 2 * L * self.n,
                                                2 * L * self.n, 2 * level * self.n, self.stream))
        return out

    def _dot_terms(self, level, a_list, b_list, addend):
        n, w = len(a_list), 2 * (level + 1) * self.n
        assert n == len(b_list), "as many b operands as a operands"
        pa = (ctypes.c_void_p * max(n, 1))(*[a.ptr for a in a_list])
        pb = (ctypes.c_void_p * max(n, 1))(*[b.ptr for b in b_list])
        st = (ctypes.c_longlong * max(n, 1))(*([w] * n))
        return n, pa, st, None, pb, st, None, addend.ptr if addend is not None else None, w

    def ckks_mult_sum(self, level, a_list, b_list, batch, addend=None, out=None):
        L = level + 1
        if out is None:
            out = self.alloc(batch * 3 * L * self.n)
        check(lib().lsa_ckks_mult_sum(self.h, level, *self._dot_terms(level, a_list, b_list, addend), out.ptr, batch,
                                      3 * L * self.n, self.stream))
        return out

    def ckks_dot(self, level, a_list, b_list, rlk, batch, rescale=True, addend=None, out=None):
        rows = level if rescale else level + 1
        if out is None:
            out = self.alloc(batch * 2 * rows * self.n)
        check(lib().lsa_ckks_dot(self.h, level, *self._dot_terms(level, a_list, b_list, addend), rlk, out.ptr, batch,
                                 2 * rows * self.n, int(bool(rescale)), self.stream))
        return out

    def _plain_out(self, level, batch, rescale, out):
        rows = level if rescale else level + 1
        if out is None:
            out = self.alloc(max(batch, 1) * 2 * rows * self.n)
        return out, 2 * rows * self.n

    def ckks_encode(self, level, values, scale, batch=1, out=None):
        v = np.ascontiguousarray(np.asarray(values, dtype=np.complex128).reshape(max(batch, 1), -1))
        period = v.shape[1]
        assert period >= 1 and period & (period - 1) == 0, "2^log_slots values per plaintext"
        w = (level + 1) * self.n
        if out is None:
            out = self.alloc(max(batch, 1) * w)
        check(lib().lsa_ckks_encode(self.h, level, period.bit_length() - 1, v.view(np.float64).ctypes.data_as(ctypes.POINTER(ctypes.c_double)),
                                    float(scale), out.ptr, w, batch, self.stream))
        return out

    def bfv_pt_rows(self, level, form):
        return {0: 1, 1: level + 1, 2: level + 1 + len(self.p)}[form]

    def bfv_encode(self, level, form, values, out=None, sout=None):
        v = np.ascontiguousarray(np.asarray(values, dtype=np.uint64).reshape(-1, self.n))
        batch = v.shape[0]
        w = self.bfv_pt_rows(level, form) * self.n
        sout = w if sout is None else sout
        if out is None:
            out = self.alloc(max(batch, 1) * max(sout, w))
        check(lib().lsa_bfv_encode(self.h, level, form, v.ctypes.data_as(ctypes.POINTER(ctypes.c_uint64)), out.ptr, sout, batch, self.stream))
        return out

    def ckks_mult_plain(self, level, ct, pt, batch, rescale=False, out=None, spt=None):
        out, so = self._plain_out(level, batch, rescale, out)
        L = level + 1
        check(lib().lsa_ckks_mult_plain(self.h, level, ct.ptr, 2 * L * self.n, pt.ptr, L * self.n if spt is None else spt, out.ptr, so,
                                        batch, int(bool(rescale)), self.stream))
        return out

    def ckks_addsub_plain(self, op, level, ct, pt, batch, out=None, spt=None):
# ... 574 lines not shown
```

Baseline: 15920.

## Fold CKKS rescale head into the ModDown base-conversion kernel

Adds a HEAD variant of the base-conversion kernel that first computes the conversion into the dropped limb, runs the rescale (subtract, multiply by P^-1, add base, centre) in registers, and then folds that centred value into the other destination limbs as an extra source term. This removes the separate sub_mul kernel and the NTT prologue fusion for the rescale head, saving a kernel launch and a round trip through memory for the last limb. It is on by default for logN>=16 when fuse_tails is set, and can be forced on or off by a new setter. In exchange the kernel carries an extra accumulation term per target and extra per-thread loads, which raises register pressure.

```diff
diff --git a/include/lattisense_amd.h b/include/lattisense_amd.h
--- a/include/lattisense_amd.h
+++ b/include/lattisense_amd.h
@@ -118,6 +118,7 @@
 int lsa_set_fuse_tails(lsa_context ctx, int enable);
 int lsa_set_modup_lift(lsa_context ctx, int enable);
 int lsa_set_ks_tail_in_mac(lsa_context ctx, int mode);
+int lsa_set_rescale_head_in_conv(lsa_context ctx, int mode);
 int lsa_set_ntt_chunk_mib(lsa_context ctx, int mib);
 int lsa_ckks_rotate_many(lsa_context ctx, int level, const uint64_t* in, int n_rot, const uint64_t* galois_elements,
                          const lsa_key* glk, uint64_t* const* outs, int batch, long long sin, long long sout, void* stream);
diff --git a/lattisense_amd/_native.py b/lattisense_amd/_native.py
--- a/lattisense_amd/_native.py
+++ b/lattisense_amd/_native.py
@@ -93,6 +93,7 @@
     "lsa_set_fuse_tails": (c_int, [c_vp, c_int]),
     "lsa_set_modup_lift": (c_int, [c_vp, c_int]),
     "lsa_set_ks_tail_in_mac": (c_int, [c_vp, c_int]),
+    "lsa_set_rescale_head_in_conv": (c_int, [c_vp, c_int]),
     "lsa_set_ntt_chunk_mib": (c_int, [c_vp, c_int]),
     "lsa_debug_set_ntt_stamps": (c_int, [c_vp, c_vp]),
     "lsa_debug_baseconv_plans": (c_int, [c_vp, c_int, ctypes.POINTER(c_int), ctypes.POINTER(c_int), ctypes.POINTER(c_int),
diff --git a/lattisense_amd/csrc/c_api.hip b/lattisense_amd/csrc/c_api.hip
--- a/lattisense_amd/csrc/c_api.hip
+++ b/lattisense_amd/csrc/c_api.hip
@@ -467,6 +467,12 @@
         C(ctx).ks_tail_in_mac = mode;
     });
 }
+int lsa_set_rescale_head_in_conv(lsa_context ctx, int mode) {
+    return guard([&] {
+        LSA_REQUIRE(mode >= 0 && mode <= 2, "lsa_set_rescale_head_in_conv: mode is 0, 1 or 2");
+        C(ctx).rescale_head_in_conv = mode;
+    });
+}
 int lsa_set_dual_stream(lsa_context ctx, int enable) {
     return guard([&] { C(ctx).dual_stream = enable ? 1 : 0; });
 }
diff --git a/lattisense_amd/csrc/context.hip b/lattisense_amd/csrc/context.hip
--- a/lattisense_amd/csrc/context.hip
+++ b/lattisense_amd/csrc/context.hip
@@ -148,9 +148,11 @@
 }
 
 const BaseConvPlan* Context::baseconv(const std::vector<int>& src, const std::vector<int>& dst, bool centered,
-                                      bool pinv_scaled, const BaseConvFold* fold) {
+                                      bool pinv_scaled, const BaseConvFold* fold, bool rescale_head) {
     std::string key = centered ? "c" : "u";
     if (pinv_scaled) key += "s";
+    if (rescale_head) key += "h";
+    LSA_REQUIRE(!rescale_head || (centered && pinv_scaled && !fold && dst.size() >= 2), "base conversion: the rescale-head flavour is a centred, P^-1-scaled ModDown plan");
     if (fold) {
         LSA_REQUIRE(!fold->tag.empty() && (fold->src_pre.empty() || fold->src_pre.size() == src.size()) &&
                         (fold->dst_scale.empty() || fold->dst_scale.size() == dst.size()),
@@ -206,6 +208,7 @@
         }
         for (int v = 0; v <= ns; v++) K->vs[j][v] = mul_mod_host(mul_mod_host((u64)v % pj, all, pj), scale, pj);
         K->half_dst[j] = mul_mod_host(mul_mod_host((all + pj - 1 % pj) % pj, (pj + 1) >> 1, pj), scale, pj);
+        if (rescale_head && j + 1 < nd) K->half_dst[j] = (K->half_dst[j] + ((T.mod[dst[nd - 1]] - 1) >> 1) % pj) % pj;
     }
     bool small = !sw::bc_no_split() && ns <= LSA_BC_NARROW_SRC;
     for (int i = 0; i < ns; i++) small = small && (T.mod[src[i]] >> 58) == 0;
diff --git a/lattisense_amd/csrc/kernels.hip b/lattisense_amd/csrc/kernels.hip
--- a/lattisense_amd/csrc/kernels.hip
+++ b/lattisense_amd/csrc/kernels.hip
@@ -1201,6 +1201,12 @@
     long long ssub;
     int sub_row[LSA_BC_MAX_SRC];
 };
+struct BaseConvHeadArgs : BaseConvArgs {
+    const u64* head_a;
+    const u64* head_b;
+    const u64* head_pinv;
+    long long s_head_a, s_head_b;
+};
 
 #define LSA_CONST_AS __attribute__((address_space(4)))
 __device__ __forceinline__ ModDev ld_mod(const LSA_CONST_AS ModDev* t, int i) {
@@ -1211,8 +1217,8 @@
     m.r1 = t[i].r1;
     return m;
 }
-template <int NSMAX, bool EXACT, int TGT, bool SPLIT = false>
-__global__ __launch_bounds__(TPB) void k_baseconv(BaseConvArgs g) {
+template <int NSMAX, bool EXACT, int TGT, bool SPLIT = false, bool HEAD = false>
+__global__ __launch_bounds__(TPB) void k_baseconv(std::conditional_t<HEAD, BaseConvHeadArgs, BaseConvArgs> g) {
     const LSA_CONST_AS BaseConvConsts& K = *(const LSA_CONST_AS BaseConvConsts*)g.k;
     const LSA_CONST_AS ModDev* const mods_c = (const LSA_CONST_AS ModDev*)g.mods;
     const int x = (blockIdx.x * TPB + threadIdx.x) * 2;
@@ -1224,6 +1230,25 @@
 #pragma unroll
     for (int i = 0; i < NSMAX; i++)
         if (EXACT || i < ns) xin[i] = ld2(src + ((long long)g.rows.src_row[i] << g.logn));
+    ulonglong2 head_a = {0, 0}, head_b = {0, 0};
+    u64 head_c0 = 0, head_c1 = 0;
+    if constexpr (HEAD) {
+        head_a = ld2(g.head_a + b * g.s_head_a + x);
+        if (g.head_b) head_b = ld2(g.head_b + b * g.s_head_b + x);
+    }
+    auto head_step = [&](const ModDev& m, u64 r0, u64 r1) {
+        if constexpr (HEAD) {
+            const u64 pinv = *(const LSA_CONST_AS u64*)g.head_pinv;
+            u64 t0 = rescale_head_t(head_a.x, r0, pinv, m), t1 = rescale_head_t(head_a.y, r1, pinv, m);
+            if (g.head_b) {
+                t0 = add_mod(t0, head_b.x, m.q);
+                t1 = add_mod(t1, head_b.y, m.q);
+            }
+            const u64 h = (m.q - 1) >> 1;
+            head_c0 = rescale_head_centre(t0, h, m.q);
+            head_c1 = rescale_head_centre(t1, h, m.q);
+        }
+    };
     if (g.sub) {
         const u64* sub = g.sub + b * g.ssub + x;
 #pragma unroll
@@ -1269,8 +1294,8 @@
             }
     }
 #pragma unroll
-    for (int jj = 0; jj < TGT; jj++) {
-        const int j = min(j0 + jj, nd - 1);
+    for (int jj = HEAD ? -1 : 0; jj < TGT; jj++) {
+        const int j = HEAD ? (jj < 0 ? nd - 1 : min(j0 + jj, nd - 2)) : min(j0 + jj, nd - 1);
         const ModDev m = ld_mod(mods_c, K.dst_mod[j]);
         u64 h0 = 0, l0 = 0, h1 = 0, l1 = 0, r0 = 0, r1 = 0;
 #if defined(LSA_BC_DIAG_NO_MATH)
@@ -1280,7 +1305,7 @@
         }
 #endif
         if (SPLIT) {
-            constexpr bool KARA = NSMAX <= 8;
+            constexpr bool KARA = NSMAX + (HEAD ? 1 : 0) <= 8;
             u64 c0[2] = {0, 0}, c1[2] = {0, 0}, c2[2] = {0, 0};
 #pragma unroll
             for (int i = 0; i < NSMAX; i++) {
@@ -1296,6 +1321,22 @@
                             c1[e] += (u64)ylo[i][e] * w1;
                             c1[e] += (u64)yhi[i][e] * w0;
                         }
+                    }
+                }
+            }
+            if (HEAD && jj >= 0) {
+                const u32 w0 = (u32)m.r1 & ((1u << 29) - 1), w1 = (u32)(m.r1 >> 29), ws = w0 + w1;
+                const u64 hc[2] = {head_c0, head_c1};
+#pragma unroll
+                for (int e = 0; e < 2; e++) {
+                    const u32 lo = (u32)hc[e] & ((1u << 29) - 1), hi = (u32)(hc[e] >> 29);
+                    c0[e] += (u64)lo * w0;
+                    c2[e] += (u64)hi * w1;
+                    if (KARA) {
+                        c1[e] += (u64)(lo + hi) * ws;
+                    } else {
+                        c1[e] += (u64)lo * w1;
+                        c1[e] += (u64)hi * w0;
                     }
                 }
             }
@@ -1318,6 +1359,10 @@
             }
             r0 = csub(mont_redc_lazy(hs[0], ls[0], m.q, m.qinv), m.q);
             r1 = csub(mont_redc_lazy(hs[1], ls[1], m.q, m.qinv), m.q);
+            if (HEAD && jj < 0) {
+                head_step(m, r0, r1);
+                continue;
+            }
 #if defined(LSA_BC_DIAG_NO_STORE)
             if (r0 == 0x123456789abcdefull) st2(dst + ((long long)g.rows.dst_row[j] << g.logn), r0, r1);
 #else
@@ -1338,6 +1383,10 @@
                 }
             }
         }
+        if (HEAD && jj >= 0) {
+            mac128(h0, l0, head_c0, m.r1);
+            mac128(h1, l1, head_c1, m.r1);
+        }
         r0 = add_mod(r0, csub(mont_redc_lazy(h0, l0, m.q, m.qinv), m.q), m.q);
         r1 = add_mod(r1, csub(mont_redc_lazy(h1, l1, m.q, m.qinv), m.q), m.q);
         }
@@ -1347,20 +1396,24 @@
             r0 = sub_mod(r0, K.half_dst[j], m.q);
             r1 = sub_mod(r1, K.half_dst[j], m.q);
         }
+        if (HEAD && jj < 0) {
+            head_step(m, r0, r1);
+            continue;
+        }
         st2(dst + ((long long)g.rows.dst_row[j] << g.logn), r0, r1);
     }
 }
 
-template <int NSMAX, int TGT>
-static void launch_baseconv_nt(int ns, int nd, bool split, dim3 grid, hipStream_t s, const BaseConvArgs& g) {
+template <int NSMAX, int TGT, bool HEAD = false, class Args = BaseConvArgs>
+static void launch_baseconv_nt(int ns, int nd, bool split, dim3 grid, hipStream_t s, const Args& g) {
     grid.z = (unsigned)((nd + TGT - 1) / TGT);
     if (split) {
-        if (ns == NSMAX) hipLaunchKernelGGL((k_baseconv<NSMAX, true, TGT, true>), grid, dim3(TPB), 0, s, g);
-        else hipLaunchKernelGGL((k_baseconv<NSMAX, false, TGT, true>), grid, dim3(TPB), 0, s, g);
+        if (ns == NSMAX) hipLaunchKernelGGL((k_baseconv<NSMAX, true, TGT, true, HEAD>), grid, dim3(TPB), 0, s, g);
+        else hipLaunchKernelGGL((k_baseconv<NSMAX, false, TGT, true, HEAD>), grid, dim3(TPB), 0, s, g);
         return;
     }
-    if (ns == NSMAX) hipLaunchKernelGGL((k_baseconv<NSMAX, true, TGT>), grid, dim3(TPB), 0, s, g);
-    else hipLaunchKernelGGL((k_baseconv<NSMAX, false, TGT>), grid, dim3(TPB), 0, s, g);
+    if (ns == NSMAX) hipLaunchKernelGGL((k_baseconv<NSMAX, true, TGT, false, HEAD>), grid, dim3(TPB), 0, s, g);
+    else hipLaunchKernelGGL((k_baseconv<NSMAX, false, TGT, false, HEAD>), grid, dim3(TPB), 0, s, g);
 }
 static int baseconv_targets_per_block(int nd) {
     const int cand[3] = {4, 7, 13};
@@ -1375,12 +1428,12 @@
     }
     return best;
 }
-template <int NSMAX>
-static void launch_baseconv_ns(int ns, int nd, bool split, dim3 grid, hipStream_t s, const BaseConvArgs& g) {
+template <int NSMAX, bool HEAD = false, class Args = BaseConvArgs>
+static void launch_baseconv_ns(int ns, int nd, bool split, dim3 grid, hipStream_t s, const Args& g) {
     const int best = baseconv_targets_per_block(nd);
-    if (best == 4) launch_baseconv_nt<NSMAX, 4>(ns, nd, split, grid, s, g);
-    else if (best == 7) launch_baseconv_nt<NSMAX, 7>(ns, nd, split, grid, s, g);
-    else launch_baseconv_nt<NSMAX, 13>(ns, nd, split, grid, s, g);
+    if (best == 4) launch_baseconv_nt<NSMAX, 4, HEAD>(ns, nd, split, grid, s, g);
+    else if (best == 7) launch_baseconv_nt<NSMAX, 7, HEAD>(ns, nd, split, grid, s, g);
+    else launch_baseconv_nt<NSMAX, 13, HEAD>(ns, nd, split, grid, s, g);
 }
 
 template <int NSMAX, bool EXACT, int TGT>
@@ -1455,9 +1508,10 @@
 }
 
 void launch_baseconv(Context& c, const BaseConvPlan* k, const BaseConvRows& rows, const u64* src, u64* dst, int batch,
-                     long long ssrc, long long sdst, hipStream_t s, const u64* sub, long long ssub, const int* sub_row) {
+                     long long ssrc, long long sdst, hipStream_t s, const u64* sub, long long ssub, const int* sub_row,
+                     const BaseConvHead* head) {
     if (batch <= 0) return;
-    BaseConvArgs g{};
+    BaseConvHeadArgs g{};
     g.sub = sub;
     g.ssub = ssub;
     LSA_REQUIRE(!sub || sub_row, "base conversion: subtrahend rows missing");
@@ -1471,24 +1525,48 @@
     g.sdst = sdst;
     g.logn = c.logn;
     g.rows = rows;
-    ProfScope ps(c, PROF_BASECONV, 8.0 * c.n * batch * (double)(k->ns * (sub ? 2 : 1) + k->nd), s);
     const int ns = k->ns, nd = k->nd;
+    if (head) {
+        LSA_REQUIRE(ns <= LSA_BC_NARROW_SRC && nd >= 2 && !sub && head->a && head->pinv, "base conversion: rescale-head form on an unsupported shape");
+        g.head_a = head->a;
+        g.head_b = head->b;
+        g.head_pinv = head->pinv;
+        g.s_head_a = head->sa;
+        g.s_head_b = head->sb;
+    }
+    ProfScope ps(c, PROF_BASECONV, 8.0 * c.n * batch * (head ? (double)(ns + 1 + (head->b ? 1 : 0) + nd - 1)
+                                                                  : (double)(ns * (sub ? 2 : 1) + nd)), s);
+    if (head) {
+        const dim3 grid((unsigned)(c.n / (2 * TPB)), (unsigned)batch, 1);
+        const int st = nd - 1;
+        if (ns <= 1) launch_baseconv_ns<1, true>(ns, st, k->split29, grid, s, g);
+        else if (ns <= 2) launch_baseconv_ns<2, true>(ns, st, k->split29, grid, s, g);
+        else if (ns <= 3) launch_baseconv_ns<3, true>(ns, st, k->split29, grid, s, g);
+        else if (ns <= 4) launch_baseconv_ns<4, true>(ns, st, k->split29, grid, s, g);
+        else if (ns <= 5) launch_baseconv_ns<5, true>(ns, st, k->split29, grid, s, g);
+        else if (ns <= 8) launch_baseconv_ns<8, true>(ns, st, k->split29, grid, s, g);
+        else if (ns <= 12) launch_baseconv_ns<12, true>(ns, st, k->split29, grid, s, g);
+        else launch_baseconv_ns<LSA_BC_NARROW_SRC, true>(ns, st, k->split29, grid, s, g);
+        LSA_HIP(hipGetLastError());
+        return;
+    }
+    const BaseConvArgs& gp = g;
     if (ns > LSA_BC_NARROW_SRC) {
         const dim3 grid((unsigned)(c.n / TPB), (unsigned)batch, 1);
-        if (ns <= 24) launch_baseconv_wide_ns<24>(ns, nd, grid, s, g);
-        else launch_baseconv_wide_ns<LSA_BC_MAX_SRC>(ns, nd, grid, s, g);
+        if (ns <= 24) launch_baseconv_wide_ns<24>(ns, nd, grid, s, gp);
+        else launch_baseconv_wide_ns<LSA_BC_MAX_SRC>(ns, nd, grid, s, gp);
         LSA_HIP(hipGetLastError());
         return;
     }
     const dim3 grid((unsigned)(c.n / (2 * TPB)), (unsigned)batch, 1);
-    if (ns <= 1) launch_baseconv_ns<1>(ns, nd, k->split29, grid, s, g);
-    else if (ns <= 2) launch_baseconv_ns<2>(ns, nd, k->split29, grid, s, g);
-    else if (ns <= 3) launch_baseconv_ns<3>(ns, nd, k->split29, grid, s, g);
-    else if (ns <= 4) launch_baseconv_ns<4>(ns, nd, k->split29, grid, s, g);
-    else if (ns <= 5) launch_baseconv_ns<5>(ns, nd, k->split29, grid, s, g);
-    else if (ns <= 8) launch_baseconv_ns<8>(ns, nd, k->split29, grid, s, g);
-    else if (ns <= 12) launch_baseconv_ns<12>(ns, nd, k->split29, grid, s, g);
-    else launch_baseconv_ns<LSA_BC_NARROW_SRC>(ns, nd, k->split29, grid, s, g);
+    if (ns <= 1) launch_baseconv_ns<1>(ns, nd, k->split29, grid, s, gp);
+    else if (ns <= 2) launch_baseconv_ns<2>(ns, nd, k->split29, grid, s, gp);
+    else if (ns <= 3) launch_baseconv_ns<3>(ns, nd, k->split29, grid, s, gp);
+    else if (ns <= 4) launch_baseconv_ns<4>(ns, nd, k->split29, grid, s, gp);
+    else if (ns <= 5) launch_baseconv_ns<5>(ns, nd, k->split29, grid, s, gp);
+    else if (ns <= 8) launch_baseconv_ns<8>(ns, nd, k->split29, grid, s, gp);
+    else if (ns <= 12) launch_baseconv_ns<12>(ns, nd, k->split29, grid, s, gp);
+    else launch_baseconv_ns<LSA_BC_NARROW_SRC>(ns, nd, k->split29, grid, s, gp);
     LSA_HIP(hipGetLastError());
 }
 
diff --git a/lattisense_amd/csrc/key_switch.hip b/lattisense_amd/csrc/key_switch.hip
--- a/lattisense_amd/csrc/key_switch.hip
+++ b/lattisense_amd/csrc/key_switch.hip
@@ -8,6 +8,21 @@
     r.period = count;
     for (int i = 0; i < count; i++) r.mod_of[i] = (unsigned char)(first + i);
     return r;
+}
+
+static bool ks_head_in_conv(const Context& c, int level, const KsOut& o) {
+    return o.form == KsOut::RESCALE && c.fuse_tails && level >= 1 && c.np <= LSA_BC_NARROW_SRC &&
+           (c.rescale_head_in_conv == 2 || (c.rescale_head_in_conv == 1 && c.logn >= 16));
+}
+static void ks_base_last_intt(Context& c, int level, const KsOut& o, int nb, hipStream_t s) {
+    if (!o.base) return;
+    u64* base_rw = const_cast<u64*>(o.base);
+    RowMap rb;
+    rb.period = 1;
+    rb.mod_of[0] = (unsigned char)level;
+    rb.row0 = level;
+    rb.row_step = o.base_rpp;
+    launch_ntt(c, base_rw, base_rw, nb, o.sbase, o.sbase, 2, rb, true, s);
 }
 
 static void ks_moddown_head(Context& c, int level, u64* acc, long long s_acc, u64* conv, const KsOut& o, int nb, hipStream_t s) {
@@ -43,7 +58,18 @@
             rows.dst_row[j] = j;
             dst.push_back(j);
         }
-        const BaseConvPlan* k = c.baseconv(src, dst, true, rs);
+        const bool in_conv = ks_head_in_conv(c, level, o);
+        const BaseConvPlan* k = c.baseconv(src, dst, true, rs, nullptr, in_conv);
+        if (in_conv) {
+            ks_base_last_intt(c, level, o, nb, s);
+            for (int h = 0; h < 2; h++) {
+                const BaseConvHead hd{acc + ((size_t)h * T + level) * N, s_acc,
+                                      o.base && h < o.base_polys ? o.base + ((size_t)h * o.base_rpp + level) * N : nullptr, o.sbase,
+                                      c.pinv_vec(level) + level};
+                launch_baseconv(c, k, rows, acc + (size_t)h * T * N, conv + (size_t)h * L * N, nb, s_acc, s_conv, s, nullptr, 0, nullptr, &hd);
+            }
+            return;
+        }
         for (int h = 0; h < 2; h++)
             launch_baseconv(c, k, rows, acc + (size_t)h * T * N, conv + (size_t)h * L * N, nb, s_acc, s_conv, s);
     }
@@ -107,28 +133,23 @@
     const int L = level + 1, T = L + c.np;
     const long long s_conv = 2LL * L * N;
     const int l = level;
-    if (o.base) {
-        u64* base_rw = const_cast<u64*>(o.base);
-        RowMap rb;
-        rb.period = 1;
-        rb.mod_of[0] = (unsigned char)l;
-        rb.row0 = l;
-        rb.row_step = o.base_rpp;
-        launch_ntt(c, base_rw, base_rw, nb, o.sbase, o.sbase, 2, rb, true, s);
-    }
-    const unsigned char lm[1] = {(unsigned char)l};
-    launch_sub_mul_general(c, 2, 1, lm, c.pinv_vec(level) + l, acc + (long long)l * N, s_acc, T, conv + (long long)l * N,
-                           s_conv, L, o.base ? o.base + (long long)l * N : nullptr, o.sbase, o.base_rpp, o.base_polys,
-                           o.p + (long long)l * N, o.sp, L, nb, s);
+    const bool in_conv = ks_head_in_conv(c, level, o);
+    if (!in_conv) {
+        ks_base_last_intt(c, level, o, nb, s);
+        const unsigned char lm[1] = {(unsigned char)l};
+        launch_sub_mul_general(c, 2, 1, lm, c.pinv_vec(level) + l, acc + (long long)l * N, s_acc, T, conv + (long long)l * N,
+                               s_conv, L, o.base ? o.base + (long long)l * N : nullptr, o.sbase, o.base_rpp, o.base_polys,
+                               o.p + (long long)l * N, o.sp, L, nb, s);
+    }
     rmo.period = 2 * L;
     for (int h = 0; h < 2; h++)
         for (int j = 0; j < L; j++) rmo.mod_of[h * L + j] = j == l ? LSA_ROW_SKIP : (unsigned char)j;
     NttFusion fb;
-    fb.pro = 2;
+    fb.pro = in_conv ? 0 : 2;
     fb.epi = 2;
     fb.limbs = L;
     fb.ql_mod = l;
-    fb.last = o.p + (long long)l * N;
+    fb.last = in_conv ? nullptr : o.p + (long long)l * N;
     fb.last_stride = o.sp;
     fb.last_rpp = L;
     fb.a = acc;
@@ -323,7 +344,7 @@
     const NttFusion fb = ks_rescale_head(c, level, acc, s_acc, conv, o, nb, s, rmo);
     NttFusion fp = fb;
     fp.epi = 0;
-    launch_ntt(c, conv, conv, nb, s_conv, s_conv, 2 * L, rmo, false, s, &fp, 1);
+    launch_ntt(c, conv, conv, nb, s_conv, s_conv, 2 * L, rmo, false, s, fb.pro ? &fp : nullptr, 1);
     const KsTailOperands kt{conv, s_conv, o.rs.out, o.rs.sout};
     LSA_REQUIRE(launch_ntt_ksmac(c, level, src.ntt, src.s_ntt, ext, s_ext, k, acc, s_acc, nb, s, fold, KS_FUSED_Q_TAIL, &kt),
                 "fused key MAC: tail shape not covered");
diff --git a/lattisense_amd/csrc/lsa_internal.h b/lattisense_amd/csrc/lsa_internal.h
--- a/lattisense_amd/csrc/lsa_internal.h
+++ b/lattisense_amd/csrc/lsa_internal.h
@@ -98,6 +98,7 @@
     int modup_lift = 1;
     int fuse_tails = 1;
     int ks_tail_in_mac = 1;
+    int rescale_head_in_conv = 1;
     int dual_stream = 0;
     hipStream_t aux_stream = nullptr;
     hipEvent_t ev_fork = nullptr, ev_join = nullptr;
@@ -150,7 +151,7 @@
         std::vector<u64> src_pre, dst_scale;
     };
     const BaseConvPlan* baseconv(const std::vector<int>& src, const std::vector<int>& dst, bool centered,
-                                 bool pinv_scaled = false, const BaseConvFold* fold = nullptr);
+                                 bool pinv_scaled = false, const BaseConvFold* fold = nullptr, bool rescale_head = false);
     const u64* pinv_vec(int level);
     const u64* pmodq_vec(int level);
     const u64* pfold_vec(int level);
@@ -265,9 +266,16 @@
     int src_row[LSA_BC_MAX_SRC];
     int dst_row[LSA_BC_MAX_DST];
 };
+struct BaseConvHead {
+    const u64* a;
+    long long sa;
+    const u64* b;
+    long long sb;
+    const u64* pinv;
+};
 void launch_baseconv(Context& c, const BaseConvPlan* k, const BaseConvRows& rows, const u64* src, u64* dst, int batch,
                      long long ssrc, long long sdst, hipStream_t s, const u64* sub = nullptr, long long ssub = 0,
-                     const int* sub_row = nullptr);
+                     const int* sub_row = nullptr, const BaseConvHead* head = nullptr);
 struct KsMacDst {
     u64* out;
     long long sout;
diff --git a/lattisense_amd/csrc/ntt_core.h b/lattisense_amd/csrc/ntt_core.h
--- a/lattisense_amd/csrc/ntt_core.h
+++ b/lattisense_amd/csrc/ntt_core.h
@@ -261,6 +261,16 @@
 #ifndef LSA_NTT_HEAD_ROUNDS
 #define LSA_NTT_HEAD_ROUNDS 2
 #endif
+LSA_HD u64 rescale_head_t(u64 a_l, u64 conv_l, u64 pinv_m, const ModDev& ml) {
+    return mont_mul(sub_mod(a_l, conv_l, ml.q), pinv_m, ml.q, ml.qinv);
+}
+LSA_HD u64 rescale_head_centre(u64 t, u64 h, u64 ql) { return add_mod(t, h, ql); }
+LSA_HD u64 rescale_head_lift(u64 c, bool near, const ModDev& mj, u64 hq) {
+    return sub_mod(near ? csub(c, mj.q) : reduce_u64(c, mj), hq, mj.q);
+}
+LSA_HD u64 rescale_head_in(u64 conv_j, u64 c, bool near, const ModDev& mj, u64 hq) {
+    return add_mod(conv_j, rescale_head_lift(c, near, mj, hq), mj.q);
+}
 struct NttLoadFix {
     bool head, add, fp, near, raw, fp_lift, lift;
     u64 ql, h, hq;
@@ -301,8 +311,8 @@
         return d_to_bits(f.add ? u52_to_double(v) + r : r);
     }
     if (f.head) {
-        const u64 c = add_mod(t, f.h, f.ql);
-        const u64 lift = sub_mod(f.near ? csub(c, f.mi.q) : reduce_u64(c, f.mi), f.hq, f.mi.q);
+        const u64 c = rescale_head_centre(t, f.h, f.ql);
+        const u64 lift = rescale_head_lift(c, f.near, f.mi, f.hq);
         v = f.add ? add_mod(v, lift, f.mi.q) : lift;
     }
     if (f.fp && !f.raw) v = d_to_bits(u52_to_double(v));
diff --git a/lattisense_amd/device.py b/lattisense_amd/device.py
--- a/lattisense_amd/device.py
+++ b/lattisense_amd/device.py
@@ -97,6 +97,9 @@
 
     def set_ks_tail_in_mac(self, mode):
         check(lib().lsa_set_ks_tail_in_mac(self.h, int(mode)))
+
+    def set_rescale_head_in_conv(self, mode):
+        check(lib().lsa_set_rescale_head_in_conv(self.h, int(mode)))
 
     def set_bfv_dot_chunk(self, pairs):
         check(lib().lsa_set_bfv_dot_chunk(self.h, int(pairs)))
```

Measured after the change: 16400, median of 6. 3.0% higher.
